# althonos/nafcodec

Hardware: NVIDIA B200
Metric: decoded_ascii_GBps (higher is better)
Workload: dtype u8

## Files before the change

nafcodec_b200/csrc/naf_kernels.cu:

```cuda
#include "naf_kernels.cuh"

#include <algorithm>

#include "zstd_core.cuh"

namespace nk {

#define FULL 0xFFFFFFFFu

__device__ __forceinline__ void flag_archive(NafCounts* counts, uint32_t* status, uint32_t bits) {
    atomicOr((unsigned long long*)&counts->status, (unsigned long long)bits);
    atomicOr(status, bits);
}

struct CS { uint32_t c; uint64_t s; };

__device__ __forceinline__ CS block_excl_scan(uint32_t c, uint64_t s, CS* total) {
    __shared__ uint32_t wc[33];
    __shared__ uint64_t ws[33];
    const int lane = threadIdx.x & 31, warp = threadIdx.x >> 5, nwarps = blockDim.x >> 5;
    uint32_t ic = c;
    uint64_t is = s;
    for (int d = 1; d < 32; d <<= 1) {
        uint32_t tc = __shfl_up_sync(FULL, ic, d);
        uint64_t ts = __shfl_up_sync(FULL, is, d);
        if (lane >= d) { ic += tc; is += ts; }
    }
    if (lane == 31) { wc[warp] = ic; ws[warp] = is; }
    __syncthreads();
    if (warp == 0) {
        uint32_t xc = lane < nwarps ? wc[lane] : 0, oc = xc;
        uint64_t xs = lane < nwarps ? ws[lane] : 0, os = xs;
        for (int d = 1; d < 32; d <<= 1) {
            uint32_t tc = __shfl_up_sync(FULL, xc, d);
            uint64_t ts = __shfl_up_sync(FULL, xs, d);
            if (lane >= d) { xc += tc; xs += ts; }
        }
        wc[lane] = xc - oc; ws[lane] = xs - os;
        if (lane == 31) { wc[32] = xc; ws[32] = xs; }
    }
    __syncthreads();
    CS r;
    r.c = ic - c + wc[warp];
    r.s = is - s + ws[warp];
    total->c = wc[32];
    total->s = ws[32];
    __syncthreads();
    return r;
}

__device__ __forceinline__ void toggle_bit(uint32_t* bits, uint32_t* chunk_par, uint64_t pos) {
    atomicXor(&bits[pos >> 5], 1u << (pos & 31));
    atomicXor(&chunk_par[pos / CHUNK_RESIDUES], 1u);
}

struct SliceView { const uint8_t* src; uint64_t size, begin, end; bool present, last; };

__device__ __forceinline__ SliceView slice_view(const uint8_t* arena, const NafDev& A, int task, uint32_t slice) {
    SliceView V;
    V.present = task == 0 ? (A.has & HAS_IDS) != 0 : task == 1 ? (A.has & HAS_COMMENTS) != 0 : task == 2 ? (A.has & HAS_LENGTHS) != 0
                                                                                                          : (A.has & HAS_MASK) && (A.has & HAS_SEQUENCE);
    V.src = arena + (task == 0 ? A.ids_off : task == 1 ? A.com_off : task == 2 ? A.len_off : A.mask_off);
    V.size = !V.present ? 0 : task == 0 ? A.ids_size : task == 1 ? A.com_size : task == 2 ? (A.len_size & ~3ull) : A.mask_size;
    V.begin = (uint64_t)slice * NAF_SLICE;
    V.end = V.begin + NAF_SLICE < V.size ? V.begin + NAF_SLICE : V.size;
    V.last = V.begin < V.size ? V.end == V.size : (slice == 0);
    return V;
}

__device__ __forceinline__ void pair_of16(int task, const uint4& v, uint32_t nvalid, uint32_t& c, uint64_t& s) {
    const uint32_t w[4] = {v.x, v.y, v.z, v.w};
    if (task == 2) { for (uint32_t j = 0; j < nvalid / 4; j++) { c += (w[j] != FULL); s += w[j]; } return; }
    const uint32_t term = task == 3 ? 0xFFu : 0u;
    for (uint32_t j = 0; j < nvalid; j++) {
        const uint32_t b = (w[j >> 2] >> (8 * (j & 3))) & 0xFF;
        c += task == 3 ? (b != term) : (b == term);
        if (task == 3) s += b;
    }
}

__global__ void __launch_bounds__(1024) k_naf_agg(const uint8_t* arena, const NafDev* archives, CS* agg, uint32_t n_slices) {
    const NafDev& A = archives[blockIdx.y];
    const int task = blockIdx.x / n_slices;
    const uint32_t slice = blockIdx.x % n_slices;
    const SliceView V = slice_view(arena, A, task, slice);
    uint32_t c = 0;
    uint64_t s = 0;
    for (uint64_t p0 = V.begin + (uint64_t)threadIdx.x * 16; p0 < V.end; p0 += 1024 * 16) {
        const uint4 v = *(const uint4*)(V.src + p0);
        pair_of16(task, v, V.end - p0 >= 16 ? 16u : (uint32_t)(V.end - p0), c, s);
    }
    CS tot;
    block_excl_scan(c, s, &tot);
    if (threadIdx.x == 0) agg[((size_t)blockIdx.y * 4 + task) * n_slices + slice] = tot;
}

__global__ void __launch_bounds__(1024) k_naf_scan(uint8_t* arena, const NafDev* archives, uint32_t* status, const CS* agg, uint32_t n_slices) {
    const NafDev& A = archives[blockIdx.y];
    const int task = blockIdx.x / n_slices;
    const uint32_t slice = blockIdx.x % n_slices;
    const int tid = threadIdx.x;
    NafCounts* counts = (NafCounts*)(arena + A.counts_off);
    const SliceView V = slice_view(arena, A, task, slice);
    if (V.begin >= V.size && slice != 0) return;
    uint64_t carry_c = 0, carry_s = 0;
    if (slice) {
        const CS* ag = agg + ((size_t)blockIdx.y * 4 + task) * n_slices;
        uint32_t c = 0;
        uint64_t s = 0;
        for (uint32_t j = tid; j < slice; j += 1024) { c += ag[j].c; s += ag[j].s; }
        CS tot;
        block_excl_scan(c, s, &tot);
        carry_c = tot.c; carry_s = tot.s;
    }
    if (task <= 1) {
        if (!V.present) { if (tid == 0) { if (task == 0) counts->n_ids = 0; else counts->n_comments = 0; } return; }
        uint64_t* offs = (uint64_t*)(arena + (task == 0 ? A.id_offsets_off : A.com_offsets_off));
        if (tid == 0 && slice == 0) offs[0] = 0;
        uint64_t carry = carry_c;
        uint32_t hi = 0;
        for (uint64_t base = V.begin; base < V.end; base += 1024 * 16) {
            uint64_t p0 = base + (uint64_t)tid * 16;
            uint4 v = make_uint4(0x01010101u, 0x01010101u, 0x01010101u, 0x01010101u);
            if (p0 < V.end) v = *(const uint4*)(V.src + p0);
            uint32_t w[4] = {v.x, v.y, v.z, v.w};
            uint32_t nvalid = p0 >= V.end ? 0 : (V.end - p0 >= 16 ? 16 : (uint32_t)(V.end - p0));
            uint32_t c = 0;
            for (uint32_t j = 0; j < nvalid; j++) {
                uint32_t b = (w[j >> 2] >> (8 * (j & 3))) & 0xFF;
                c += (b == 0);
                hi |= b;
            }
            CS tot;
            CS ex = block_excl_scan(c, 0, &tot);
            uint64_t k = carry + ex.c;
            if (c) {
                for (uint32_t j = 0; j < nvalid; j++) {
                    uint32_t b = (w[j >> 2] >> (8 * (j & 3))) & 0xFF;
                    if (b == 0) { k++; if (k <= A.n_records) offs[k] = p0 + j + 1; }
                }
            }
            carry += tot.c;
        }
        if (__any_sync(FULL, hi & 0x80)) { if ((tid & 31) == 0) atomicOr((unsigned long long*)&counts->nonascii, 1ull << task); }
        if (tid == 0 && V.last) {
            if (task == 0) counts->n_ids = carry; else counts->n_comments = carry;
            if (carry < A.n_records && V.size > 0 && V.src[V.size - 1] != 0) flag_archive(counts, status, zc::E_NUL);
        }
    } else if (task == 2) {
        uint64_t* rec = (uint64_t*)(arena + A.rec_offsets_off);
        uint64_t* lens = (uint64_t*)(arena + A.lengths_off);
        if (tid == 0 && slice == 0) rec[0] = 0;
        const uint64_t w_begin = V.begin / 4, w_end = V.end / 4;
        for (uint64_t base = w_begin; base < w_end; base += 1024 * 4) {
            uint64_t i0 = base + (uint64_t)tid * 4;
            uint4 v = make_uint4(FULL, FULL, FULL, FULL);
            if (i0 < w_end) v = *(const uint4*)(V.src + i0 * 4);
            uint32_t w[4] = {v.x, v.y, v.z, v.w};
            uint32_t nvalid = i0 >= w_end ? 0 : (w_end - i0 >= 4 ? 4 : (uint32_t)(w_end - i0));
            uint32_t c = 0;
            uint64_t s = 0;
            for (uint32_t j = 0; j < nvalid; j++) { c += (w[j] != FULL); s += w[j]; }
            CS tot;
            CS ex = block_excl_scan(c, s, &tot);
            uint64_t k = carry_c + ex.c, S = carry_s + ex.s;
            for (uint32_t j = 0; j < nvalid; j++) {
                S += w[j];
                if (w[j] != FULL) { k++; if (k <= A.n_records) rec[k] = S; }
            }
            carry_c += tot.c; carry_s += tot.s;
        }
        if (n_slices > 1) {
            if (tid == 0 && V.last) counts->n_lengths = carry_c;
            return;
        }
        __syncthreads();
        uint64_t n_len = carry_c < A.n_records ? carry_c : A.n_records;
        uint64_t total = rec[n_len];
        if (tid == 0) {
            counts->n_lengths = n_len;
            counts->total_residues = total;
            counts->first_bad_record = NO_RECORD;
            if ((A.has & HAS_SEQUENCE) && total > A.seq_residues) flag_archive(counts, status, zc::E_LENGTHS);
            if ((A.has & HAS_QUALITY) && total > A.qual_size) flag_archive(counts, status, zc::E_LENGTHS);
        }
        for (uint64_t k = tid; k < n_len; k += blockDim.x) lens[k] = rec[k + 1] - rec[k];
    } else {
        if (!V.present) { if (tid == 0 && slice == 0) { counts->n_mask_runs = 0; counts->mask_sum = 0; } return; }
        uint64_t* bounds = (uint64_t*)(arena + A.mask_bounds_off);
        uint32_t* bits = (uint32_t*)(arena + A.mask_bits_off);
        uint32_t* cpar = (uint32_t*)(arena + A.chunk_par_off);
        for (uint64_t base = V.begin; base < V.end; base += 1024 * 16) {
            uint64_t p0 = base + (uint64_t)tid * 16;
            uint4 v = make_uint4(0, 0, 0, 0);
            if (p0 < V.end) v = *(const uint4*)(V.src + p0);
            uint32_t w[4] = {v.x, v.y, v.z, v.w};
            uint32_t nvalid = p0 >= V.end ? 0 : (V.end - p0 >= 16 ? 16 : (uint32_t)(V.end - p0));
            uint32_t c = 0;
            uint64_t s = 0;
            for (uint32_t j = 0; j < nvalid; j++) {
                uint32_t b = (w[j >> 2] >> (8 * (j & 3))) & 0xFF;
                c += (b != 0xFF); s += b;
            }
            CS tot;
            CS ex = block_excl_scan(c, s, &tot);
            uint64_t k = carry_c + ex.c, S = carry_s + ex.s;
            for (uint32_t j = 0; j < nvalid; j++) {
                uint32_t b = (w[j >> 2] >> (8 * (j & 3))) & 0xFF;
                S += b;
                if (b != 0xFF) { bounds[k++] = S; if (S <= A.seq_residues) toggle_bit(bits, cpar, S); }
            }
            carry_c += tot.c; carry_s += tot.s;
        }
        if (tid == 0 && V.last) {
            if (V.size > 0 && V.src[V.size - 1] == 0xFF) {
                bounds[carry_c++] = carry_s;
                if (carry_s <= A.seq_residues) toggle_bit(bits, cpar, carry_s);
            }
            counts->n_mask_runs = carry_c;
            counts->mask_sum = carry_s;
        }
    }
}

__global__ void __launch_bounds__(256) k_naf_lengths(uint8_t* arena, const NafDev* archives, uint32_t* status) {
    const NafDev& A = archives[blockIdx.y];
    NafCounts* counts = (NafCounts*)(arena + A.counts_off);
    const uint64_t* rec = (const uint64_t*)(arena + A.rec_offsets_off);
    uint64_t* lens = (uint64_t*)(arena + A.lengths_off);
    const uint64_t raw = (A.has & HAS_LENGTHS) ? counts->n_lengths : 0;
    const uint64_t n_len = raw < A.n_records ? raw : A.n_records;
    const uint64_t r = (uint64_t)blockIdx.x * blockDim.x + threadIdx.x;
    if (r < n_len) lens[r] = rec[r + 1] - rec[r];
    if (r == 0) {
        const uint64_t total = rec[n_len];
        counts->n_lengths = n_len;
        counts->total_residues = total;
        counts->first_bad_record = NO_RECORD;
        if ((A.has & HAS_SEQUENCE) && total > A.seq_residues) flag_archive(counts, status, zc::E_LENGTHS);
        if ((A.has & HAS_QUALITY) && total > A.qual_size) flag_archive(counts, status, zc::E_LENGTHS);
    }
}

__global__ void __launch_bounds__(256) k_mask_fix(uint8_t* arena, const NafDev* archives, uint32_t* status) {
    const NafDev& A = archives[blockIdx.y];
    if (!(A.has & HAS_MASK) || !(A.has & HAS_SEQUENCE)) return;
    NafCounts* counts = (NafCounts*)(arena + A.counts_off);
    const uint64_t r = (uint64_t)blockIdx.x * blockDim.x + threadIdx.x;
    if (r >= counts->n_lengths) return;
    const uint64_t* rec = (const uint64_t*)(arena + A.rec_offsets_off);
    const uint64_t* bounds = (const uint64_t*)(arena + A.mask_bounds_off);
    uint32_t* bits = (uint32_t*)(arena + A.mask_bits_off);
    const uint64_t S = rec[r], E = rec[r + 1];
    if (E == S || E > A.seq_residues) return;
    const uint64_t pos = E - 1, n_runs = counts->n_mask_runs;
    uint64_t lo = 0, hi = n_runs;
    while (lo < hi) {
        uint64_t mid = (lo + hi) >> 1;
        if (bounds[mid] > pos) hi = mid; else lo = mid + 1;
    }
    if (lo == n_runs) { flag_archive(counts, status, zc::E_MASK); return; }
    if (lo & 1) {
        uint64_t a = lo ? bounds[lo - 1] : 0;
        uint32_t* cpar = (uint32_t*)(arena + A.chunk_par_off);
        toggle_bit(bits, cpar, a > S ? a : S);
        toggle_bit(bits, cpar, E);
    }
}

__device__ __forceinline__ uint32_t prmt(uint32_t a, uint32_t b, uint32_t s) {
#if defined(__CUDA_ARCH__)
    uint32_t d;
    asm("prmt.b32 %0, %1, %2, %3;" : "=r"(d) : "r"(a), "r"(b), "r"(s));
    return d;
#else
    return __byte_perm(a, b, s);
#endif
}

__device__ __forceinline__ uint32_t iupac4(uint32_t x16, uint32_t l0) {
    const uint32_t sel = x16 & 0x7777u;
    const uint32_t lo = prmt(l0, 0x42535943u, sel);
    const uint32_t hi = prmt(0x44525741u, 0x4E56484Du, sel);
    const uint32_t m = prmt(0x80808080u, 0u, x16 & 0x8888u);
    return (lo & ~m) | (hi & m);
}

__device__ __forceinline__ uint32_t spread4_x20(uint32_t q) {
    return ((q * 0x00204081u) & 0x01010101u) << 5;
}

__global__ void __launch_bounds__(UNPACK_T) k_unpack(uint8_t* arena, const NafDev* archives) {
    const NafDev& A = archives[blockIdx.y];
    if (!(A.has & HAS_SEQUENCE) || A.seq_type > 1 || blockIdx.x >= A.n_chunks) return;
    __shared__ uint32_t wp[32], wp2[32];
    __shared__ uint32_t wball, cball;
    const NafCounts* counts = (const NafCounts*)(arena + A.counts_off);
    const uint64_t total = counts->total_residues < A.seq_residues ? counts->total_residues : A.seq_residues;
    const uint64_t wi = (uint64_t)blockIdx.x * CHUNK_WORDS + UNPACK_W * threadIdx.x;
    const uint64_t r0 = wi * 32;
    uint32_t mask[UNPACK_W];
#pragma unroll
    for (uint32_t k = 0; k < UNPACK_W; k++) mask[k] = 0;
    if (A.has & HAS_MASK) {
        const uint32_t* bits = (const uint32_t*)(arena + A.mask_bits_off);
        const uint64_t n_words = (A.seq_residues + 32) / 32;
        uint32_t par = 0;
#pragma unroll
        for (uint32_t k = 0; k < UNPACK_W; k++) {
            const uint32_t w = wi + k < n_words ? bits[wi + k] : 0;
            uint32_t m = w;
            m ^= m << 1; m ^= m << 2; m ^= m << 4; m ^= m << 8; m ^= m << 16;
            mask[k] = par ? ~m : m;
            par ^= __popc(w) & 1;
        }
        const int lane = threadIdx.x & 31, warp = threadIdx.x >> 5;
        uint32_t b = __ballot_sync(FULL, par);
        if (lane == 0) wp[warp] = __popc(b) & 1;
        __syncthreads();
        if (warp == 0) { uint32_t bb = __ballot_sync(FULL, lane < (int)(UNPACK_T / 32) ? wp[lane] : 0u); if (lane == 0) wball = bb; }
        __syncthreads();
        const uint32_t* cpar = (const uint32_t*)(arena + A.chunk_par_off);
        uint32_t cp = 0;
        for (uint32_t c = threadIdx.x; c < blockIdx.x; c += blockDim.x) cp ^= cpar[c];
        const uint32_t cb = __ballot_sync(FULL, cp & 1);
        if (lane == 0) wp2[warp] = __popc(cb) & 1;
        __syncthreads();
        if (warp == 0) { uint32_t bb = __ballot_sync(FULL, lane < (int)(UNPACK_T / 32) ? wp2[lane] : 0u); if (lane == 0) cball = bb; }
        __syncthreads();
        const uint32_t carry = (__popc(cball) & 1) ^ (__popc(wball & ((1u << warp) - 1u)) & 1) ^ (__popc(b & ((1u << lane) - 1u)) & 1);
        if (carry) {
#pragma unroll
            for (uint32_t k = 0; k < UNPACK_W; k++) mask[k] = ~mask[k];
        }
    }
    if (r0 >= total) return;
    const uint32_t l0 = A.seq_type == 1 ? 0x4B47552Du : 0x4B47542Du;
    const uint4* src = (const uint4*)(arena + A.seq_off + r0 / 2);
    uint4 pk[UNPACK_W];
#pragma unroll
    for (uint32_t k = 0; k < UNPACK_W; k++) {
        pk[k] = make_uint4(0, 0, 0, 0);
        if (r0 + 32 * k < total) pk[k] = src[k];
    }
    uint4* dst = (uint4*)(arena + A.ascii_off + r0);
#pragma unroll
    for (uint32_t k = 0; k < UNPACK_W; k++) {
        if (r0 + 32 * k >= total) break;
        const uint32_t x[4] = {pk[k].x, pk[k].y, pk[k].z, pk[k].w};
        uint32_t o[8];
#pragma unroll
        for (int j = 0; j < 4; j++) {
            o[2 * j] = iupac4(x[j] & 0xFFFFu, l0) | spread4_x20((mask[k] >> (8 * j)) & 0xFu);
            o[2 * j + 1] = iupac4(x[j] >> 16, l0) | spread4_x20((mask[k] >> (8 * j + 4)) & 0xFu);
        }
        dst[2 * k] = make_uint4(o[0], o[1], o[2], o[3]);
        dst[2 * k + 1] = make_uint4(o[4], o[5], o[6], o[7]);
    }
}

__global__ void __launch_bounds__(CHUNK_WORDS) k_text_mask(uint8_t* arena, const NafDev* archives) {
    const NafDev& A = archives[blockIdx.y];
    if (!(A.has & HAS_SEQUENCE) || !(A.has & HAS_MASK) || A.seq_type <= 1 || blockIdx.x >= A.n_chunks) return;
    const NafCounts* counts = (const NafCounts*)(arena + A.counts_off);
    const uint64_t total = counts->total_residues < A.seq_residues ? counts->total_residues : A.seq_residues;
    const uint64_t wi = (uint64_t)blockIdx.x * CHUNK_WORDS + threadIdx.x;
    const uint32_t* bits = (const uint32_t*)(arena + A.mask_bits_off);
    const uint32_t* par = (const uint32_t*)(arena + A.chunk_par_off);
    const uint64_t n_words = (A.seq_residues + 32) / 32;
    if (wi >= n_words) return;
    uint32_t carry = 0;
    for (uint32_t c = 0; c < blockIdx.x; c++) carry ^= par[c] & 1;
    for (uint64_t j = (uint64_t)blockIdx.x * CHUNK_WORDS; j < wi; j++) carry ^= __popc(bits[j]) & 1;
    uint32_t m = bits[wi];
    m ^= m << 1; m ^= m << 2; m ^= m << 4; m ^= m << 8; m ^= m << 16;
    if (carry) m = ~m;
    uint8_t* s = arena + A.seq_off;
    for (int j = 0; j < 32; j++) {
        uint64_t i = wi * 32 + j;
        if (i >= total) break;
        uint8_t c = s[i];
        if (((m >> j) & 1) && c >= 'A' && c <= 'Z') s[i] = c | 0x20;
    }
}

__global__ void __launch_bounds__(256) k_ascii_check(uint8_t* arena, const NafDev* archives) {
    const NafDev& A = archives[blockIdx.y];
    const int field = blockIdx.z;
    const uint8_t* src;
    uint64_t size;
    if (field == 0) { if (!(A.has & HAS_SEQUENCE) || A.seq_type <= 1) return; src = arena + A.seq_off; size = A.seq_size; }
    else { if (!(A.has & HAS_QUALITY)) return; src = arena + A.qual_off; size = A.qual_size; }
    NafCounts* counts = (NafCounts*)(arena + A.counts_off);
    uint32_t acc = 0;
    const uint64_t n16 = (size + 15) / 16;
    for (uint64_t i = (uint64_t)blockIdx.x * blockDim.x + threadIdx.x; i < n16; i += (uint64_t)gridDim.x * blockDim.x) {
        uint4 v = *(const uint4*)(src + i * 16);
        if (i * 16 + 16 > size) {
            uint32_t w[4] = {v.x, v.y, v.z, v.w};
            for (int j = 0; j < 16; j++) if (i * 16 + j < size) acc |= (w[j >> 2] >> (8 * (j & 3))) & 0xFF;
        } else acc |= v.x | v.y | v.z | v.w;
    }
    if (__any_sync(FULL, acc & 0x80808080u)) { if ((threadIdx.x & 31) == 0) atomicOr((unsigned long long*)&counts->nonascii, 1ull << (2 + field)); }
}

__device__ __forceinline__ bool utf8_ok(const uint8_t* s, uint64_t n) {
    uint64_t i = 0;
    while (i < n) {
        uint32_t b = s[i];
        if (b < 0x80) { i++; continue; }
        uint32_t need, cp;
        if (b >= 0xC2 && b <= 0xDF) { need = 1; cp = b & 0x1F; }
        else if (b >= 0xE0 && b <= 0xEF) { need = 2; cp = b & 0x0F; }
        else if (b >= 0xF0 && b <= 0xF4) { need = 3; cp = b & 0x07; }
        else return false;
        if (n - i <= need) return false;
        for (uint32_t k = 1; k <= need; k++) {
            uint32_t c = s[i + k];
            if ((c & 0xC0) != 0x80) return false;
            cp = (cp << 6) | (c & 0x3F);
        }
        if (need == 2 && (cp < 0x800 || (cp >= 0xD800 && cp <= 0xDFFF))) return false;
        if (need == 3 && (cp < 0x10000 || cp > 0x10FFFF)) return false;
        i += need + 1;
    }
    return true;
}

__global__ void __launch_bounds__(256) k_utf8_validate(uint8_t* arena, const NafDev* archives, uint32_t* status) {
    const NafDev& A = archives[blockIdx.y];
    const int field = blockIdx.z;
    NafCounts* counts = (NafCounts*)(arena + A.counts_off);
    if (!((counts->nonascii >> field) & 1)) return;
    const uint64_t r = (uint64_t)blockIdx.x * blockDim.x + threadIdx.x;
    const uint8_t* s;
    uint64_t b, e;
    if (field <= 1) {
        uint64_t n = field == 0 ? counts->n_ids : counts->n_comments;
        if (n > A.n_records) n = A.n_records;
        if (r >= n) return;
        const uint64_t* offs = (const uint64_t*)(arena + (field == 0 ? A.id_offsets_off : A.com_offsets_off));
        s = arena + (field == 0 ? A.ids_off : A.com_off);
        b = offs[r]; e = offs[r + 1] - 1;
    } else {
        if (r >= counts->n_lengths) return;
        const uint64_t* rec = (const uint64_t*)(arena + A.rec_offsets_off);
        s = arena + (field == 2 ? A.seq_off : A.qual_off);
        b = rec[r]; e = rec[r + 1];
        if (e > (field == 2 ? A.seq_size : A.qual_size)) return;
    }
    if (!utf8_ok(s + b, e - b)) {
        flag_archive(counts, status, zc::E_UTF8);
        atomicMin((unsigned long long*)&counts->first_bad_record, (unsigned long long)r);
    }
}

int launch_naf_stage(uint8_t* arena, const NafDev* archives, uint32_t n_archives, uint64_t max_records, uint64_t max_scan_bytes, void* scan_agg,
                     uint32_t max_chunks, uint64_t max_text_bytes, bool any_mask, bool any_text_mask, uint32_t* status, cudaStream_t st,
                     StageEvents* ev) {
    StageEvents none;
    if (!ev) ev = &none;
    int launches = 0;
    if (n_archives == 0) { for (int i = 0; i < NAF_STAGES; i++) ev->mark(); return 0; }
    const uint32_t n_slices = (uint32_t)std::max<uint64_t>(1, (max_scan_bytes + NAF_SLICE - 1) / NAF_SLICE);
    uint32_t rec_grid = (uint32_t)((max_records + 255) / 256);
    if (n_slices > 1) { NAF_LAUNCH(k_naf_agg, dim3(4 * n_slices, n_archives), 1024, 0, st, arena, archives, (CS*)scan_agg, n_slices); launches++; }
    NAF_LAUNCH(k_naf_scan, dim3(4 * n_slices, n_archives), 1024, 0, st, arena, archives, status, (const CS*)scan_agg, n_slices); launches++;
    if (n_slices > 1) { NAF_LAUNCH(k_naf_lengths, dim3(rec_grid ? rec_grid : 1, n_archives), 256, 0, st, arena, archives, status); launches++; }
    ev->mark();
    if (max_chunks > 0 && any_mask) {
        if (rec_grid) { NAF_LAUNCH(k_mask_fix, dim3(rec_grid, n_archives), 256, 0, st, arena, archives, status); launches++; }
        ev->mark();
        ev->mark();
    } else { ev->mark(); ev->mark(); }
    if (max_chunks > 0) {
        NAF_LAUNCH(k_unpack, dim3(max_chunks, n_archives), UNPACK_T, 0, st, arena, archives); launches++;
        if (any_text_mask) { NAF_LAUNCH(k_text_mask, dim3(max_chunks, n_archives), CHUNK_WORDS, 0, st, arena, archives); launches++; }
    }
    ev->mark();
    if (max_text_bytes > 0) {
        uint32_t g = (uint32_t)((max_text_bytes / 16 + 255) / 256);
        if (g > 148 * 8) g = 148 * 8;
        if (g == 0) g = 1;
        NAF_LAUNCH(k_ascii_check, dim3(g, n_archives, 2), 256, 0, st, arena, archives); launches++;
    }
    if (rec_grid) { NAF_LAUNCH(k_utf8_validate, dim3(rec_grid, n_archives, 4), 256, 0, st, arena, archives, status); launches++; }
    ev->mark();
    return launches;
}

}
```

nafcodec_b200/csrc/naf_kernels.cuh:

```cuda
#pragma once
#include "cuda_compat.h"
#include <stdint.h>

namespace nk {

enum : uint32_t { HAS_IDS = 1, HAS_COMMENTS = 2, HAS_LENGTHS = 4, HAS_MASK = 8, HAS_SEQUENCE = 16, HAS_QUALITY = 32 };

constexpr uint32_t UNPACK_T = 256;
constexpr uint32_t UNPACK_W = 2;
constexpr uint32_t CHUNK_WORDS = UNPACK_W * UNPACK_T;
constexpr uint32_t CHUNK_RESIDUES = CHUNK_WORDS * 32;
constexpr uint64_t NO_RECORD = ~0ull;
constexpr uint32_t NAF_SLICE = 32768;
constexpr uint32_t NAF_AGG_BYTES = 16;

struct NafCounts {
    uint64_t n_ids;
    uint64_t n_comments;
    uint64_t n_lengths;
    uint64_t total_residues;
    uint64_t n_mask_runs;
    uint64_t mask_sum;
    uint64_t first_bad_record;
    uint64_t nonascii;
    uint64_t status;
    uint64_t _pad;
};

struct NafDev {
    uint64_t n_records;
    uint32_t seq_type;
    uint32_t has;
    uint64_t seq_residues;
    uint64_t ids_off, ids_size, com_off, com_size, len_off, len_size, mask_off, mask_size;
    uint64_t seq_off, seq_size, qual_off, qual_size;
    uint64_t counts_off, id_offsets_off, com_offsets_off, lengths_off, rec_offsets_off, ascii_off;
    uint64_t mask_bits_off, mask_bounds_off, chunk_par_off;
    uint32_t n_chunks;
    uint32_t _pad;
};

int launch_naf_stage(uint8_t* arena, const NafDev* archives_dev, uint32_t n_archives, uint64_t max_records, uint64_t max_scan_bytes, void* scan_agg,
                     uint32_t max_chunks, uint64_t max_text_bytes, bool any_mask, bool any_text_mask, uint32_t* status, cudaStream_t stream,
                     StageEvents* ev);
constexpr int NAF_STAGES = 5;

}
```

nafcodec_b200/csrc/naf_load.cuh:

```cuda
#pragma once
#include "cuda_compat.h"
#include <stdint.h>

namespace nk {

__device__ __forceinline__ uint4 load16u(const uint8_t* p) {
    const uint32_t s = (uint32_t)((uintptr_t)p & 15);
    const uint4* q = (const uint4*)(p - s);
    const uint4 lo = q[0];
    if (s == 0) return lo;
    const uint4 hi = q[1];
    const bool s2 = s & 8, s1 = s & 4;
    const uint32_t a0 = s2 ? lo.z : lo.x, a1 = s2 ? lo.w : lo.y, a2 = s2 ? hi.x : lo.z, a3 = s2 ? hi.y : lo.w, a4 = s2 ? hi.z : hi.x, a5 = s2 ? hi.w : hi.y;
    const uint32_t b0 = s1 ? a1 : a0, b1 = s1 ? a2 : a1, b2 = s1 ? a3 : a2, b3 = s1 ? a4 : a3, b4 = s1 ? a5 : a4;
    const uint32_t bs = (s & 3) * 8;
    const uint32_t o[4] = {__funnelshift_r(b0, b1, bs), __funnelshift_r(b1, b2, bs), __funnelshift_r(b2, b3, bs), __funnelshift_r(b3, b4, bs)};
    return make_uint4(o[0], o[1], o[2], o[3]);
}

}
```

nafcodec_b200/csrc/nafgpu_api.cu:

```cuda
#if defined(__SSE2__)
#include <emmintrin.h>
#endif
#include <stdio.h>
#include <stdlib.h>
#include <string.h>

#include <algorithm>
#include <atomic>
#include <chrono>
#include <memory>
#include <mutex>
#include <thread>
#include <string>
#include <vector>

#include "../../include/nafgpu.h"
#include "cuda_compat.h"
#include "frame_walk.h"
#include "naf_export.cuh"
#include "naf_kernels.cuh"
#include "naf_pack.cuh"
#include "naf_text.cuh"
#include "zstd_kernels.cuh"

namespace {

constexpr uint64_t ALIGN = 128;
inline uint64_t align_up(uint64_t v, uint64_t a = ALIGN) { return (v + a - 1) / a * a; }
constexpr int N_STAGES = zk::ZSTD_STAGES + nk::NAF_STAGES;
constexpr size_t FLUSH_BYTES = 256u << 20;

struct DevBuf {
    void* p = nullptr;
    size_t cap = 0;
    bool ensure(size_t n) {
        if (n <= cap) return true;
        if (p) cudaFree(p);
        p = nullptr; cap = 0;
        size_t want = n + n / 8 + 256;
        if (cudaMalloc(&p, want) != cudaSuccess) { p = nullptr; cudaGetLastError(); return false; }
        cap = want;
        return true;
    }
    void release() { if (p) cudaFree(p); p = nullptr; cap = 0; }
    ~DevBuf() { release(); }
};
struct PinBuf {
    void* p = nullptr;
    size_t cap = 0;
    bool ensure(size_t n) {
        if (n <= cap) return true;
        if (p) cudaFreeHost(p);
        p = nullptr; cap = 0;
        size_t want = n + n / 8 + 256;
        if (cudaHostAlloc(&p, want, cudaHostAllocDefault) != cudaSuccess) { p = nullptr; cudaGetLastError(); return false; }
        cap = want;
        return true;
    }
    void release() { if (p) cudaFreeHost(p); p = nullptr; cap = 0; }
    ~PinBuf() { release(); }
};

struct ArchPlan {
    uint64_t n_records = 0;
    bool dec[6] = {false, false, false, false, false, false};
    uint64_t blob_off[6] = {0, 0, 0, 0, 0, 0};
    uint64_t blob_size[6] = {0, 0, 0, 0, 0, 0};
    bool nucleotide = true;
    uint64_t line_length = 0;
    uint32_t sep = ' ';
    uint32_t first_frame = 0, n_frames = 0;
    int host_status = 0;
    std::string host_msg;
};

struct WalkTask {
    uint32_t arch = 0;
    int sec = 0;
    const uint8_t* data = nullptr;
    uint64_t comp_off = 0, comp_size = 0, dst_off = 0, dst_size = 0;
    fw::JobPlan plan;
    int rc = 0;
    std::string err;
    bool live = true;
    size_t bo = 0;
    uint32_t so = 0, slot_off = 0, ho = 0;
    uint64_t lo = 0;
    uint64_t p_begin = 0, p_end = 0;
    bool first = true, last = true, heavy = false;
    fw::RangeState st;
    int carry_huf_task = -1, carry_tbl_task[3] = {-1, -1, -1};
    uint32_t carry_huf_block = 0, carry_huf_slot = 0, carry_tbl_slot[3] = {0, 0, 0};
    uint32_t abs_huf_block = zf::NO_BLOCK, abs_huf_slot = 0, abs_tbl[3] = {zf::NO_SLOT, zf::NO_SLOT, zf::NO_SLOT};
};

struct PrepClock {
    bool on = getenv("NAFGPU_DEBUG_PREP") != nullptr;
    std::chrono::steady_clock::time_point t = std::chrono::steady_clock::now();
    void lap(const char* what) {
        if (!on) return;
        const auto n = std::chrono::steady_clock::now();
        fprintf(stderr, "[prepare] %-28s %8.3f ms\n", what, std::chrono::duration<double, std::milli>(n - t).count());
        t = n;
    }
};

static_assert(sizeof(zf::BlockDesc) % 16 == 0, "store_desc writes 16 bytes at a time");
#if defined(__SSE2__) && !defined(__CUDA_ARCH__)
inline void store_desc(zf::BlockDesc* dst, const zf::BlockDesc& b) {
    if (((uintptr_t)dst & 15) == 0) {
        const __m128i* s = (const __m128i*)&b;
        __m128i* d = (__m128i*)dst;
        for (size_t k = 0; k < sizeof(zf::BlockDesc) / 16; k++) _mm_stream_si128(d + k, _mm_loadu_si128(s + k));
    } else {
        *dst = b;
    }
}
inline void desc_fence() { _mm_sfence(); }
#else
inline void store_desc(zf::BlockDesc* dst, const zf::BlockDesc& b) { *dst = b; }
inline void desc_fence() {}
#endif

static std::atomic<int> g_helpers_busy{0};
struct HelperLease {
    unsigned n = 1;
    HelperLease() {
        const int hw = (int)std::max(1u, std::thread::hardware_concurrency());
        const int cap = std::min(12, std::max(1, hw * 3 / 4));
        const int got = std::max(1, std::min(cap, hw - g_helpers_busy.load(std::memory_order_relaxed)));
        g_helpers_busy.fetch_add(got, std::memory_order_relaxed);
        n = (unsigned)got;
    }
    ~HelperLease() { g_helpers_busy.fetch_sub((int)n, std::memory_order_relaxed); }
    HelperLease(const HelperLease&) = delete;
    HelperLease& operator=(const HelperLease&) = delete;
};

template <class F>
void parallel_for(size_t n, unsigned max_threads, F fn) {
    if (n <= 1 || max_threads <= 1) { for (size_t i = 0; i < n; i++) fn(i); return; }
    const unsigned w = (unsigned)std::min<size_t>(n, max_threads);
    std::atomic<size_t> next{0};
    auto body = [&] { for (;;) { const size_t i = next.fetch_add(1); if (i >= n) return; fn(i); } };
    std::vector<std::thread> th;
    for (unsigned t = 1; t < w; t++) th.emplace_back(body);
    body();
    for (std::thread& t : th) t.join();
}

}

struct nafgpu_ctx {
    int device = 0;
    cudaStream_t st = 0, st2 = 0, st3 = 0;
    cudaEvent_t ev_fork = nullptr, ev_join = nullptr, ev_fork3 = nullptr, ev_join3 = nullptr, ev_fork4 = nullptr, ev_join4 = nullptr, ev_block = nullptr, ev_d2h = nullptr;
    std::string err;
    DevBuf comp, arena, lit, desc, bstate, hufw, fsstate, lzidx, scanagg, debug, tables, table_al, seq32, seq64, misc, flush, text, fin_g, pack_in, pack_out;
    size_t o_frames = 0, o_naf = 0, o_huf = 0, o_chunks = 0, o_gbase = 0, o_tiles = 0, o_big = 0, o_bigseq = 0, o_biglit = 0;
    PinBuf stage, result, misc_host, text_host, text_stage, pack_host;
    fw::JobPlan plan;
    std::vector<WalkTask> tasks;
    size_t n_tasks = 0;
    std::vector<nk::NafDev> arch;
    std::vector<ArchPlan> aplan;
    zk::JobDev J;
    uint64_t z1_size = 0, z2_off = 0, z2_size = 0, arena_size = 0, counts_size = 0;
    uint64_t max_records = 0, max_text = 0, max_mask = 0, max_scan = 0;
    uint32_t max_chunks = 0;
    bool any_mask = false, any_text_mask = false;
    uint32_t coop_ctas = 1, fin_ctas = 1, fin2_ctas = 1;
    size_t misc_words = 0;
    nafgpu_job_stats stats;
    bool prepared = false, ran = false;
    bool win_counts = false;
    PinBuf win;
    uint32_t want = 0;
    bool exp_ready = false;
    std::vector<nafgpu_counts> counts;
    DevBuf exp_desc;
    PinBuf exp_stage;
    uint32_t n_exp_rec = 0, n_exp_span[4] = {0, 0, 0, 0};
    uint64_t o_exp_span[4] = {0, 0, 0, 0}, exp_bytes[4] = {0, 0, 0, 0}, exp_records = 0, exp_residues = 0;
    cudaEvent_t ev_exp_ready = nullptr, ev_exp_done = nullptr;
    cudaEvent_t ev[N_STAGES + 3];
    bool ev_ok = false;
#if !defined(NAFGPU_EMULATE)
    cudaGraphExec_t graph = nullptr;
#endif
};

namespace {

int fail(nafgpu_ctx* c, int code, const std::string& msg) {
    c->err = msg;
    return code;
}

#define CUDA_TRY(c, expr) do { cudaError_t _e = (expr); if (_e != cudaSuccess) { \
    char _b[256]; snprintf(_b, sizeof _b, "%s failed: %s", #expr, cudaGetErrorString(_e)); return fail((c), NAFGPU_ERR_CUDA, _b); } } while (0)

void drop_graph(nafgpu_ctx* c) {
#if !defined(NAFGPU_EMULATE)
    if (c->graph) { cudaGraphExecDestroy(c->graph); c->graph = nullptr; }
#else
    (void)c;
#endif
}

int enqueue_run(nafgpu_ctx* c, StageEvents* ev) {
    cudaStream_t st = c->st;
    CUDA_TRY(c, cudaMemsetAsync(c->misc.p, 0, c->misc_words * 4, st));
    if (c->J.n_seq && !c->J.lz_small) {
        CUDA_TRY(c, cudaMemsetAsync(c->J.seq_done, 0, c->J.n_seq * 4, st));
        CUDA_TRY(c, cudaMemsetAsync(c->J.lz_blocker, 0xFF, c->J.n_seq * 4, st));
    }
    CUDA_TRY(c, cudaMemsetAsync(c->arena.p, 0, c->counts_size, st));
    if (c->z2_size) CUDA_TRY(c, cudaMemsetAsync((uint8_t*)c->arena.p + c->z2_off, 0, c->z2_size, st));
    int launches = zk::launch_zstd_stage(c->J, st, ev ? (cudaStream_t)0 : c->st2, c->ev_fork, c->ev_join, ev, c->st3, c->ev_fork3, c->ev_join3, c->ev_fork4, c->ev_join4);
    launches += nk::launch_naf_stage((uint8_t*)c->arena.p, (const nk::NafDev*)((const uint8_t*)c->desc.p + c->o_naf), (uint32_t)c->arch.size(), c->max_records, c->max_scan, c->scanagg.p,
                                     c->max_chunks, c->max_text, c->any_mask, c->any_text_mask, c->J.status, st, ev);
    c->stats.kernel_launches = (uint32_t)launches;
    CUDA_TRY(c, cudaGetLastError());
    c->ran = true;
    c->win_counts = false;
    c->exp_ready = false;
    return NAFGPU_OK;
}

void read_lz_stats(nafgpu_ctx* c) {
    const uint32_t* m = (const uint32_t*)c->misc_host.p;
    c->stats.lz_handover = m[4]; c->stats.lz_rounds = m[5]; c->stats.lz_unresolved = m[6];
    c->stats.lz_flow = c->misc_words >= 32 ? (m[c->misc_words - 32] | ((c->J.lz_flow_early && m[c->misc_words - 32 + 4] == 0) ? 2u : 0u)) : 0;
    if (c->misc_words >= 24) memcpy(c->stats.lz_pending, m + c->misc_words - 24, 24 * 4);
}

int status_to_code(uint32_t s, std::string& msg) {
    using namespace zc;
    if (s == 0) return NAFGPU_OK;
    char b[96];
    snprintf(b, sizeof b, " (device status 0x%x)", s);
    if (s & (E_FSE_TABLE | E_HUF_TREE | E_HUF_STREAM | E_SEQ_STREAM | E_LITERALS | E_OFFSET | E_NO_TABLE | E_INTERNAL)) {
        msg = std::string("corrupt zstd stream") + b; return NAFGPU_ERR_INVALID_DATA;
    }
    if (s & E_CHECKSUM) { msg = std::string("zstd frame checksum mismatch") + b; return NAFGPU_ERR_INVALID_DATA; }
    if (s & E_SIZE) { msg = std::string("section does not regenerate the size its header states") + b; return NAFGPU_ERR_INVALID_DATA; }
    if (s & E_LENGTHS) { msg = std::string("record lengths exceed the sequence/quality stream") + b; return NAFGPU_ERR_UNEXPECTED_EOF; }
    if (s & E_MASK) { msg = std::string("failed to get mask unit") + b; return NAFGPU_ERR_UNEXPECTED_EOF; }
    if (s & E_NUL) { msg = std::string("id/comment stream is not NUL terminated") + b; return NAFGPU_ERR_INVALID_DATA; }
    if (s & E_UTF8) { msg = std::string("invalid utf-8") + b; return NAFGPU_ERR_UTF8; }
    msg = std::string("unknown device status") + b;
    return NAFGPU_ERR_INVALID_DATA;
}

static std::mutex g_d2h_turn[16];

static cudaError_t wait_stream(nafgpu_ctx* c) {
    if (c->z1_size < (8u << 20) || !c->ev_block) return cudaStreamSynchronize(c->st);
    cudaError_t e = cudaEventRecord(c->ev_block, c->st);
    return e != cudaSuccess ? e : cudaEventSynchronize(c->ev_block);
}

static cudaEvent_t g_last_d2h[16];

static int d2h_results(nafgpu_ctx* c) {
    if (!c->result.ensure(c->z1_size + 64)) return fail(c, NAFGPU_ERR_NOMEM, "pinned host allocation failed");
    c->win_counts = false;
    CUDA_TRY(c, wait_stream(c));
    {
        std::lock_guard<std::mutex> turn(g_d2h_turn[c->device & 15]);
        cudaEvent_t prev = g_last_d2h[c->device & 15];
        if (prev && prev != c->ev_d2h && c->ev_d2h) CUDA_TRY(c, cudaStreamWaitEvent(c->st, prev, 0));
        CUDA_TRY(c, cudaMemcpyAsync(c->misc_host.p, c->misc.p, c->misc_words * 4, cudaMemcpyDeviceToHost, c->st));
        CUDA_TRY(c, cudaMemcpyAsync(c->result.p, c->arena.p, c->z1_size, cudaMemcpyDeviceToHost, c->st));
        if (c->ev_d2h) { CUDA_TRY(c, cudaEventRecord(c->ev_d2h, c->st)); g_last_d2h[c->device & 15] = c->ev_d2h; }
        else { CUDA_TRY(c, wait_stream(c)); return NAFGPU_OK; }
    }
    CUDA_TRY(c, wait_stream(c));
    return NAFGPU_OK;
}

struct Copy { const uint8_t* src; uint64_t dst, size; };

int finish_prepare(nafgpu_ctx* c, const std::vector<Copy>& copies, uint64_t comp_off, uint32_t n, bool copies_enqueued = false) {
    PrepClock clk;
    size_t nb = 0;
    uint64_t walked_bytes = 0;
    for (size_t ti = 0; ti < c->n_tasks; ti++) {
        WalkTask& T = c->tasks[ti];
        if (!T.live) continue;
        fw::JobPlan& G = c->plan;
        const fw::JobPlan& L = T.plan;
        T.bo = nb; T.so = (uint32_t)G.seq_total; T.lo = G.lit_total - 16; T.slot_off = G.n_slots - 3; T.ho = G.n_huf_slots;
        if (G.seq_total + L.seq_total > 0xFFFFFFF0ull || nb + L.blocks.size() > 0xFFFFFFF0ull) return fail(c, NAFGPU_ERR_UNSUPPORTED, "job has too many blocks or sequences: split the batch");
        for (zf::FrameDesc F : L.frames) { F.first_block += (uint32_t)T.bo; F.first_seq += T.so; G.frames.push_back(F); }
        if (!T.first) {
            zf::FrameDesc& F = G.frames.back();
            F.n_blocks += T.st.n_blocks; F.n_seq += T.st.n_seq;
            if (T.last) { F.has_checksum = T.st.has_checksum; F.checksum = T.st.checksum; }
            if (T.carry_huf_task >= 0) { const WalkTask& S = c->tasks[T.carry_huf_task]; T.abs_huf_block = (uint32_t)S.bo + T.carry_huf_block; T.abs_huf_slot = S.ho + T.carry_huf_slot; }
            for (int k = 0; k < 3; k++) {
                if (T.carry_tbl_task[k] == -2) T.abs_tbl[k] = T.carry_tbl_slot[k];
                else if (T.carry_tbl_task[k] >= 0) T.abs_tbl[k] = c->tasks[T.carry_tbl_task[k]].slot_off + T.carry_tbl_slot[k];
            }
        }
        for (zf::HufItem it : L.huf_items) { it.block += (uint32_t)T.bo; G.huf_items.push_back(it); }
        for (uint32_t b : L.big_seq) G.big_seq.push_back(b + (uint32_t)T.bo);
        for (uint32_t b : L.big_lit) G.big_lit.push_back(b + (uint32_t)T.bo);
        G.seq_total += L.seq_total; G.lit_total += L.lit_total - 16; G.n_slots += L.n_slots - 3; G.n_huf_slots += L.n_huf_slots;
        G.n_huf_blocks += L.n_huf_blocks; G.n_seq_blocks += L.n_seq_blocks; G.n_checksums += L.n_checksums;
        G.max_seq_section = std::max(G.max_seq_section, L.max_seq_section);
        G.max_seq_section_big = std::max(G.max_seq_section_big, L.max_seq_section_big); G.n_tiny_seq_blocks += L.n_tiny_seq_blocks;
        nb += L.blocks.size();
        walked_bytes += T.comp_size;
    }
    c->plan.finalize(zk::HUF_SMALL_SYMBOLS);
    const fw::JobPlan& pl = c->plan;
    const size_t nf = pl.frames.size();
    const uint64_t nseq = pl.seq_total;

    c->misc_words = 0;
    const size_t nh = pl.huf_items.size();
    c->o_frames = align_up(nb * sizeof(zf::BlockDesc), 16);
    c->o_naf = c->o_frames + align_up(nf * sizeof(zf::FrameDesc), 16);
    c->o_huf = c->o_naf + align_up((size_t)n * sizeof(nk::NafDev), 16);
    c->o_chunks = c->o_huf + align_up(nh * sizeof(zf::HufItem), 16);
    std::vector<uint32_t> chunk_first(nf + 1, 0);
    for (size_t f = 0; f < nf; f++) {
        const uint64_t nchunks = (pl.frames[f].dst_size + 65535) >> 16;
        if ((uint64_t)chunk_first[f] + nchunks > 0x7FFFFFFFull) return fail(c, NAFGPU_ERR_UNSUPPORTED, "job too large for the chunk table");
        chunk_first[f + 1] = chunk_first[f] + (uint32_t)nchunks;
    }
    const uint32_t total_chunks = chunk_first[nf];
    std::vector<uint64_t> g_base(nf + 1, 0);
    for (size_t f = 0; f < nf; f++) g_base[f + 1] = g_base[f] + ((pl.frames[f].dst_size + 15) & ~(uint64_t)15);
    c->o_gbase = c->o_chunks + align_up((nf + 1) * 4, 16);
    std::vector<zf::FsTile> tiles;
    std::vector<zf::FsBigFrame> bigs;
    uint32_t fs_big = zf::FS_BIG_FRAME, fs_tile = zf::FS_TILE;
    if (const char* e = getenv("NAFGPU_FS_TILE")) { fs_tile = (uint32_t)std::max(1, atoi(e)); fs_big = 2 * fs_tile; }
    for (size_t f = 0; f < nf; f++) {
        const zf::FrameDesc& F = pl.frames[f];
        if (F.n_blocks <= fs_big) continue;
        bigs.push_back({(uint32_t)f, (uint32_t)tiles.size(), (F.n_blocks + fs_tile - 1) / fs_tile, 0u});
        for (uint32_t b = 0; b < F.n_blocks; b += fs_tile) tiles.push_back({(uint32_t)f, F.first_block + b, std::min(fs_tile, F.n_blocks - b), 0u});
    }
    c->o_tiles = c->o_gbase + align_up((nf + 1) * 8, 16);
    c->o_big = c->o_tiles + align_up(tiles.size() * sizeof(zf::FsTile), 16);
    c->o_bigseq = c->o_big + align_up(bigs.size() * sizeof(zf::FsBigFrame), 16);
    c->o_biglit = c->o_bigseq + align_up(pl.big_seq.size() * 4, 16);
    const size_t stage_bytes = c->o_biglit + align_up(pl.big_lit.size() * 4, 16);
    c->misc_words = 1 + 3 + 1 + 1 + 1 + 3 + nf + total_chunks + 8 + 24;
    bool ok = c->comp.ensure(comp_off + 64) && c->arena.ensure(c->arena_size) && c->lit.ensure(pl.lit_total + 64) &&
              c->desc.ensure(stage_bytes + 64) && c->fin_g.ensure((size_t)g_base[nf] * 4 + 256 + (size_t)total_chunks * 8192) &&
              c->bstate.ensure(nb * sizeof(zf::BlockState) + 64) && c->fsstate.ensure(tiles.size() * sizeof(zf::FsTileState) + 64) && c->lzidx.ensure(((size_t)total_chunks * 16 + nf + 16) * 4) &&
              c->scanagg.ensure((size_t)n * 4 * ((c->max_scan + nk::NAF_SLICE - 1) / nk::NAF_SLICE + 1) * nk::NAF_AGG_BYTES + 64) && c->hufw.ensure((size_t)pl.n_huf_slots * 258 + 64) &&
              c->tables.ensure((size_t)pl.n_slots * zf::FSE_SLOT_CELLS * sizeof(zc::SeqCell)) && c->table_al.ensure(pl.n_slots + 64) &&
              c->seq32.ensure(nseq * 5 * 4 + 64) && c->seq64.ensure(nseq * sizeof(zf::SeqRec) + 64) && c->misc.ensure(c->misc_words * 4);
    if (!ok) return fail(c, NAFGPU_ERR_NOMEM, "device allocation failed");
    clk.lap("merge + device buffers");
    if (!c->stage.ensure(stage_bytes + 64) || !c->result.ensure(c->counts_size + 64) || !c->misc_host.ensure(c->misc_words * 4 + 64))
        return fail(c, NAFGPU_ERR_NOMEM, "pinned host allocation failed");

    uint8_t* sp = (uint8_t*)c->stage.p;
    {
        std::vector<uint32_t> frame_off(c->n_tasks, 0);
        { uint32_t fo = 0; for (size_t t = 0; t < c->n_tasks; t++) { frame_off[t] = c->tasks[t].first ? fo : fo - 1; if (c->tasks[t].live) fo += (uint32_t)c->tasks[t].plan.frames.size(); } }
        (void)walked_bytes;
        unsigned threads = 1;
        std::unique_ptr<HelperLease> lease;
        if (nb > 200000) { lease.reset(new HelperLease); threads = lease->n; }
        struct Chunk { size_t task, begin, end; };
        std::vector<Chunk> chunks;
        for (size_t t = 0; t < c->n_tasks; t++) {
            if (!c->tasks[t].live) continue;
            const size_t cnt = c->tasks[t].plan.blocks.size();
            for (size_t b = 0; b < cnt; b += 65536) chunks.push_back({t, b, std::min(cnt, b + 65536)});
        }
        parallel_for(chunks.size(), threads, [&](size_t ci) {
            const Chunk& K = chunks[ci];
            const WalkTask& T = c->tasks[K.task];
            zf::BlockDesc* out = (zf::BlockDesc*)sp + T.bo;
            const zf::BlockDesc* in = T.plan.blocks.data();
            const uint32_t fo = frame_off[K.task];
            for (size_t i = K.begin; i < K.end; i++) {
                zf::BlockDesc b = in[i];
                b.frame += fo;
                if (b.n_seq) b.seq_base += T.so;
                if (b.huf_block == fw::PREV_BLOCK) { b.lit_base += T.lo; b.huf_block = T.abs_huf_block; b.huf_slot = T.abs_huf_slot; }
                else {
                    if (b.lit_type >= zf::LT_HUF && b.btype == zf::BT_COMPRESSED) { b.lit_base += T.lo; b.huf_slot += T.ho; }
                    if (b.huf_block != zf::NO_BLOCK) b.huf_block += (uint32_t)T.bo;
                }
                for (int k = 0; k < 3; k++) {
                    if (b.tbl[k] == fw::PREV_SLOT) b.tbl[k] = T.abs_tbl[k];
                    else if (b.tbl[k] != zf::NO_SLOT && b.tbl[k] >= 3) b.tbl[k] += T.slot_off;
                }
                store_desc(out + i, b);
            }
            desc_fence();
        });
    }
    clk.lap("pinned staging + block copy");
    if (nf) memcpy(sp + c->o_frames, pl.frames.data(), nf * sizeof(zf::FrameDesc));
    if (n) memcpy(sp + c->o_naf, c->arch.data(), (size_t)n * sizeof(nk::NafDev));
    if (nh) memcpy(sp + c->o_huf, pl.huf_items.data(), nh * sizeof(zf::HufItem));
    memcpy(sp + c->o_chunks, chunk_first.data(), (nf + 1) * 4);
    memcpy(sp + c->o_gbase, g_base.data(), (nf + 1) * 8);
    if (!pl.big_seq.empty()) memcpy(sp + c->o_bigseq, pl.big_seq.data(), pl.big_seq.size() * 4);
    if (!pl.big_lit.empty()) memcpy(sp + c->o_biglit, pl.big_lit.data(), pl.big_lit.size() * 4);
    if (!tiles.empty()) { memcpy(sp + c->o_tiles, tiles.data(), tiles.size() * sizeof(zf::FsTile)); memcpy(sp + c->o_big, bigs.data(), bigs.size() * sizeof(zf::FsBigFrame)); }
    if (stage_bytes) CUDA_TRY(c, cudaMemcpyAsync(c->desc.p, sp, stage_bytes, cudaMemcpyHostToDevice, c->st));
    uint64_t h2d = stage_bytes;
    for (const Copy& cp : copies) {
        if (!copies_enqueued) CUDA_TRY(c, cudaMemcpyAsync((uint8_t*)c->comp.p + cp.dst, cp.src, cp.size, cudaMemcpyHostToDevice, c->st));
        h2d += cp.size;
    }

    clk.lap("H2D enqueue");
    zk::JobDev& J = c->J;
    J.comp = (const uint8_t*)c->comp.p; J.out = (uint8_t*)c->arena.p; J.lit = (uint8_t*)c->lit.p;
    J.frames = (const zf::FrameDesc*)((const uint8_t*)c->desc.p + c->o_frames); J.blocks = (const zf::BlockDesc*)c->desc.p;
    J.bstate = (zf::BlockState*)c->bstate.p; J.tables = (zc::SeqCell*)c->tables.p; J.table_al = (uint8_t*)c->table_al.p;
    J.seq_done = (uint32_t*)c->seq32.p;
    J.lz_list[0] = J.seq_done + nseq; J.lz_list[1] = J.seq_done + 2 * nseq; J.lz_list[2] = J.seq_done + 3 * nseq; J.lz_blocker = J.seq_done + 4 * nseq;
    J.seq = (zf::SeqRec*)c->seq64.p;
    J.tiny_blocks = pl.n_tiny_seq_blocks >= 4096u ? 1u : 0u;
    if (const char* e = getenv("NAFGPU_TINY_BLOCKS")) J.tiny_blocks = (uint32_t)atoi(e);
    J.seq_big_list = (const uint32_t*)((const uint8_t*)c->desc.p + c->o_bigseq); J.n_seq_big = (uint32_t)pl.big_seq.size();
    J.lit_big_list = (const uint32_t*)((const uint8_t*)c->desc.p + c->o_biglit); J.n_lit_big = (uint32_t)pl.big_lit.size();
    {
        uint64_t small_max = 2048;
        if (const char* e = getenv("NAFGPU_LZ_SMALL")) small_max = (uint64_t)std::min(8192, std::max(0, atoi(e)));
        J.lz_small = (nseq <= small_max && nf <= 65535 && c->arena_size < (1ull << 32)) ? 1u : 0u;
    }
    J.seq_stage_bytes = std::min<uint32_t>((((J.tiny_blocks ? pl.max_seq_section_big : pl.max_seq_section) + 15u) & ~15u) + 64u, 16u * 1024u);
    uint32_t* misc = (uint32_t*)c->misc.p;
    J.status = misc; J.lz_count = misc + 1; J.lz_handover = misc + 4; J.lz_rounds = misc + 5; J.fin_unresolved = misc + 6; J.fin_count = misc + 7;
    J.frame_bad = misc + 10; J.fin_chunk_flag = misc + 10 + nf; J.lz_pending = misc + 10 + nf + total_chunks + 8;
    J.lz_flow = misc + 10 + nf + total_chunks;
    J.lz_flow_on = nseq > 8192 ? 1u : 0u;
    if (const char* e = getenv("NAFGPU_LZ_FLOW")) J.lz_flow_on = (uint32_t)atoi(e);
    J.flow_ctas = (uint32_t)std::min<uint64_t>((nseq + 255) / 256, 148u * 8u);
    J.lz_flow_early = (nseq > 2048 && nseq <= 65536 && !getenv("NAFGPU_LZ_SMALL")) ? 1u : 0u;
    if (const char* e = getenv("NAFGPU_LZ_FLOW_EARLY")) J.lz_flow_early = (uint32_t)atoi(e);
    J.fin_chunk_first = (const uint32_t*)((const uint8_t*)c->desc.p + c->o_chunks); J.fin_total_chunks = total_chunks;
    J.lz_idx = (uint32_t*)c->lzidx.p;
    J.fin_ctas = c->fin_ctas; J.fin2_ctas = c->fin2_ctas; J.fin_g = (uint32_t*)c->fin_g.p; J.fin_ext = (uint32_t*)c->fin_g.p + g_base[nf] + 64;
    J.fin_g_base = (const uint64_t*)((const uint8_t*)c->desc.p + c->o_gbase);
    J.coop_ctas = c->coop_ctas;
    {
        uint64_t biggest = 0;
        for (const auto& F : c->plan.frames) biggest = std::max<uint64_t>(biggest, F.dst_size);
        (void)biggest;
        const uint64_t waves = ((uint64_t)total_chunks + c->fin_ctas - 1) / std::max<uint32_t>(c->fin_ctas, 1u);
        J.fin_cost_us = (uint32_t)std::min<uint64_t>(300 + waves * 270, 0x7FFFFFFFu);
        if (const char* e = getenv("NAFGPU_FIN_COST_US")) J.fin_cost_us = (uint32_t)atoi(e);
    }
    J.huf_weights = (uint8_t*)c->hufw.p; J.huf_meta = (uint8_t*)c->hufw.p + (size_t)pl.n_huf_slots * 256;
    J.huf_items = (const zf::HufItem*)((const uint8_t*)c->desc.p + c->o_huf); J.n_huf_items = (uint32_t)nh; J.n_huf_big = pl.n_huf_big; J.max_huf_stream = pl.max_huf_stream; J.max_huf_small = pl.max_huf_small;
    J.huf_block_min = 0;
    if (const char* e = getenv("NAFGPU_HUF_BLOCK_MIN")) J.huf_block_min = (uint32_t)std::max(1, atoi(e));
    J.debug = nullptr; J.debug_seq = nullptr;
    if (getenv("NAFGPU_DEBUG_HUF") && nh) {
        if (!c->debug.ensure(nh * 64 + 64)) return fail(c, NAFGPU_ERR_NOMEM, "debug buffer");
        cudaMemsetAsync(c->debug.p, 0, nh * 64 + 64, c->st);
        J.debug = (unsigned long long*)c->debug.p;
        J.debug_seq = J.debug + nh * 8;
    }
    J.fs_tiles = (const zf::FsTile*)((const uint8_t*)c->desc.p + c->o_tiles); J.fs_big = (const zf::FsBigFrame*)((const uint8_t*)c->desc.p + c->o_big);
    J.fs_state = (zf::FsTileState*)c->fsstate.p; J.n_fs_tiles = (uint32_t)tiles.size(); J.n_fs_big = (uint32_t)bigs.size(); J.fs_big_frame = fs_big;
    J.n_frames = (uint32_t)nf; J.n_blocks = (uint32_t)nb; J.n_slots = pl.n_slots; J.n_seq = nseq; J.n_checksums = pl.n_checksums;

    c->stats.n_archives = n; c->stats.n_frames = nf; c->stats.n_blocks = nb; c->stats.n_sequences = nseq;
    c->stats.h2d_bytes = h2d; c->stats.d2h_bytes = c->z1_size + c->misc_words * 4;
    c->stats.n_stages = N_STAGES + 1;
    c->prepared = true;
    return NAFGPU_OK;
}

int archive_status(nafgpu_ctx* c, uint32_t a, std::string& msg) {
    const ArchPlan& P = c->aplan[a];
    if (P.host_status) { msg = P.host_msg; return P.host_status; }
    const uint32_t* frame_bad = (const uint32_t*)c->misc_host.p + 10;
    uint32_t s = 0;
    for (uint32_t f = P.first_frame; f < P.first_frame + P.n_frames; f++) s |= frame_bad[f];
    const nk::NafCounts* C = (const nk::NafCounts*)((const uint8_t*)c->result.p + c->arch[a].counts_off);
    s |= (uint32_t)C->status;
    return status_to_code(s & ~zc::E_UTF8, msg);
}

int read_counts(nafgpu_ctx* c) {
    if (c->win_counts) return NAFGPU_OK;
    CUDA_TRY(c, wait_stream(c));
    CUDA_TRY(c, cudaMemcpyAsync(c->misc_host.p, c->misc.p, c->misc_words * 4, cudaMemcpyDeviceToHost, c->st));
    CUDA_TRY(c, cudaMemcpyAsync(c->result.p, c->arena.p, c->counts_size, cudaMemcpyDeviceToHost, c->st));
    CUDA_TRY(c, cudaStreamSynchronize(c->st));
    read_lz_stats(c);
    c->win_counts = true;
    return NAFGPU_OK;
}

int export_tables(nafgpu_ctx* c) {
    if (c->exp_ready) return NAFGPU_OK;
    { int rc = read_counts(c); if (rc) return rc; }
    const uint32_t n = (uint32_t)c->arch.size();
    c->counts.assign(n, nafgpu_counts());
    std::vector<nk::ExpRec> recs;
    std::vector<nk::ExpSpan> spans[4];
    uint64_t records = 0, residues = 0, bytes[4] = {0, 0, 0, 0};
    for (uint32_t a = 0; a < n; a++) {
        const nk::NafDev& D = c->arch[a];
        const ArchPlan& P = c->aplan[a];
        const nk::NafCounts* C = (const nk::NafCounts*)((const uint8_t*)c->result.p + D.counts_off);
        nafgpu_counts& k = c->counts[a];
        memset(&k, 0, sizeof k);
        k.n_records = P.n_records;
        k.first_bad_record = nk::NO_RECORD;
        std::string msg;
        k.status = archive_status(c, a, msg);
        if (k.status) continue;
        k.n_ids = P.dec[0] ? std::min<uint64_t>(C->n_ids, P.n_records) : 0;
        k.n_comments = P.dec[1] ? std::min<uint64_t>(C->n_comments, P.n_records) : 0;
        k.n_lengths = P.dec[2] ? C->n_lengths : 0;
        k.total_residues = P.dec[2] ? C->total_residues : 0;
        k.id_bytes = P.dec[0] ? D.ids_size : 0;
        k.comment_bytes = P.dec[1] ? D.com_size : 0;
        k.first_bad_record = C->first_bad_record;
        k.record_status = (C->first_bad_record != nk::NO_RECORD) ? NAFGPU_ERR_UTF8 : 0;
        if (k.n_lengths)
            recs.push_back({records, residues, D.rec_offsets_off, {P.dec[4] ? D.ascii_off : nk::NO_FIELD, P.dec[5] ? D.qual_off : nk::NO_FIELD}, 0});
        const uint64_t field_bytes[4] = {k.id_bytes, k.comment_bytes, P.dec[4] ? k.total_residues : 0, P.dec[5] ? k.total_residues : 0};
        const uint64_t field_off[4] = {D.ids_off, D.com_off, D.ascii_off, D.qual_off};
        for (int f = 0; f < 4; f++) {
            if (!field_bytes[f]) continue;
            spans[f].push_back({bytes[f], field_off[f]});
            bytes[f] += field_bytes[f];
        }
        records += k.n_lengths;
        residues += k.total_residues;
    }
    uint64_t off = align_up(recs.size() * sizeof(nk::ExpRec), 16);
    for (int f = 0; f < 4; f++) { c->o_exp_span[f] = off; off += align_up(spans[f].size() * sizeof(nk::ExpSpan), 16); }
    if (!c->exp_desc.ensure(off + 64)) return fail(c, NAFGPU_ERR_NOMEM, "device allocation failed");
    if (!c->exp_stage.ensure(off + 64)) return fail(c, NAFGPU_ERR_NOMEM, "pinned host allocation failed");
    uint8_t* S = (uint8_t*)c->exp_stage.p;
    if (!recs.empty()) memcpy(S, recs.data(), recs.size() * sizeof(nk::ExpRec));
    for (int f = 0; f < 4; f++) if (!spans[f].empty()) memcpy(S + c->o_exp_span[f], spans[f].data(), spans[f].size() * sizeof(nk::ExpSpan));
    if (off) CUDA_TRY(c, cudaMemcpyAsync(c->exp_desc.p, S, off, cudaMemcpyHostToDevice, c->st));
    c->n_exp_rec = (uint32_t)recs.size();
    for (int f = 0; f < 4; f++) { c->n_exp_span[f] = (uint32_t)spans[f].size(); c->exp_bytes[f] = bytes[f]; }
    c->exp_records = records;
    c->exp_residues = residues;
    c->exp_ready = true;
    return NAFGPU_OK;
}

}

extern "C" {

int nafgpu_ctx_create(int device, nafgpu_ctx** out) {
    if (!out) return NAFGPU_ERR_ARGUMENT;
    *out = nullptr;
    int n = 0;
    if (cudaGetDeviceCount(&n) != cudaSuccess || n <= 0) { cudaGetLastError(); return NAFGPU_ERR_NO_DEVICE; }
    if (device < 0 || device >= n) return NAFGPU_ERR_ARGUMENT;
    if (cudaSetDevice(device) != cudaSuccess) return NAFGPU_ERR_CUDA;
    nafgpu_ctx* c = new nafgpu_ctx();
    c->device = device;
    memset(&c->stats, 0, sizeof c->stats);
    memset(&c->J, 0, sizeof c->J);
    if (cudaStreamCreateWithFlags(&c->st, cudaStreamNonBlocking) != cudaSuccess) { delete c; return NAFGPU_ERR_CUDA; }
    if (cudaStreamCreateWithFlags(&c->st2, cudaStreamNonBlocking) != cudaSuccess || cudaStreamCreateWithFlags(&c->st3, cudaStreamNonBlocking) != cudaSuccess) { delete c; return NAFGPU_ERR_CUDA; }
    if (cudaEventCreateWithFlags(&c->ev_fork3, cudaEventDisableTiming) != cudaSuccess || cudaEventCreateWithFlags(&c->ev_join3, cudaEventDisableTiming) != cudaSuccess) { delete c; return NAFGPU_ERR_CUDA; }
    if (cudaEventCreateWithFlags(&c->ev_fork4, cudaEventDisableTiming) != cudaSuccess || cudaEventCreateWithFlags(&c->ev_join4, cudaEventDisableTiming) != cudaSuccess) { delete c; return NAFGPU_ERR_CUDA; }
    if (cudaEventCreateWithFlags(&c->ev_fork, cudaEventDisableTiming) != cudaSuccess || cudaEventCreateWithFlags(&c->ev_join, cudaEventDisableTiming) != cudaSuccess) { delete c; return NAFGPU_ERR_CUDA; }
    if (cudaEventCreateWithFlags(&c->ev_block, cudaEventDisableTiming | cudaEventBlockingSync) != cudaSuccess) { c->ev_block = nullptr; cudaGetLastError(); }
    if (cudaEventCreateWithFlags(&c->ev_d2h, cudaEventDisableTiming) != cudaSuccess) { c->ev_d2h = nullptr; cudaGetLastError(); }
    if (cudaEventCreateWithFlags(&c->ev_exp_ready, cudaEventDisableTiming) != cudaSuccess || cudaEventCreateWithFlags(&c->ev_exp_done, cudaEventDisableTiming) != cudaSuccess) { delete c; return NAFGPU_ERR_CUDA; }
    for (int i = 0; i < N_STAGES + 3; i++) if (cudaEventCreate(&c->ev[i]) != cudaSuccess) { delete c; return NAFGPU_ERR_CUDA; }
    c->ev_ok = true;
    c->coop_ctas = zk::lz_resolve_max_ctas(device);
    zk::lz_finish_ctas(device, &c->fin_ctas, &c->fin2_ctas);
    *out = c;
    return NAFGPU_OK;
}

void nafgpu_ctx_destroy(nafgpu_ctx* c) {
    if (!c) return;
    cudaSetDevice(c->device);
    cudaStreamSynchronize(c->st);
    drop_graph(c);
    DevBuf* d[] = {&c->comp, &c->arena, &c->lit, &c->desc, &c->bstate, &c->hufw, &c->fsstate, &c->lzidx, &c->scanagg, &c->debug, &c->tables, &c->table_al, &c->seq32, &c->seq64, &c->misc, &c->flush, &c->text, &c->fin_g, &c->pack_in, &c->pack_out, &c->exp_desc};
    for (DevBuf* b : d) b->release();
    c->stage.release(); c->result.release(); c->misc_host.release(); c->text_host.release(); c->text_stage.release(); c->pack_host.release(); c->win.release();
    c->exp_stage.release();
    if (c->ev_exp_ready) cudaEventDestroy(c->ev_exp_ready);
// ... 820 lines not shown
```

nafcodec_b200/csrc/zstd_format.h:

```cpp
#pragma once
#include <stdint.h>

namespace zf {

constexpr uint32_t BLOCK_MAX = 128 * 1024;
constexpr uint32_t NO_BLOCK = 0xFFFFFFFFu;
constexpr uint32_t NO_SLOT = 0xFFFFFFFFu;
constexpr int COMP_PAD = 32;

enum BlockType : uint8_t { BT_RAW = 0, BT_RLE = 1, BT_COMPRESSED = 2 };
enum LitType : uint8_t { LT_RAW = 0, LT_RLE = 1, LT_HUF = 2, LT_TREELESS = 3 };
enum SeqMode : uint8_t { SM_PREDEF = 0, SM_RLE = 1, SM_FSE = 2, SM_REPEAT = 3 };

struct FrameDesc {
    uint64_t src_off;
    uint64_t src_size;
    uint64_t dst_off;
    uint64_t dst_size;
    uint32_t first_block;
    uint32_t n_blocks;
    uint32_t first_seq;
    uint32_t n_seq;
    uint64_t window;
    uint32_t has_checksum;
    uint32_t checksum;
};

struct BlockDesc {
    uint64_t src_off;
    uint64_t lit_base;
    uint32_t src_size;
    uint32_t frame;
    uint32_t lit_regen;
    uint32_t lit_csize;
    uint32_t lit_src;
    uint32_t seq_src;
    uint32_t n_seq;
    uint32_t seq_base;
    uint32_t huf_block;
    uint32_t tbl[3];
    uint8_t btype;
    uint8_t lit_type;
    uint8_t n_streams;
    uint8_t modes;
    uint8_t defines;
    uint8_t _pad[3];
    uint32_t known_regen;
    uint32_t huf_slot;
};

constexpr uint32_t TINY_SEQ_MAX = 32, TINY_LIT_MAX = 2048;
#if defined(__CUDACC__)
#define ZF_HD __host__ __device__
#else
#define ZF_HD
#endif
ZF_HD inline bool tiny_seq_block(const BlockDesc& B) { return B.btype == BT_COMPRESSED && B.n_seq != 0 && B.n_seq <= TINY_SEQ_MAX; }
ZF_HD inline bool needs_seq_kernel(const BlockDesc& B) { return B.btype == BT_COMPRESSED && B.n_seq > TINY_SEQ_MAX; }
ZF_HD inline bool tiny_lit_block(const BlockDesc& B) {
    if (B.btype != BT_COMPRESSED) return B.src_size <= TINY_LIT_MAX;
    return B.n_seq <= TINY_SEQ_MAX && B.lit_regen <= TINY_LIT_MAX;
}

struct HufItem {
    uint32_t block;
    uint32_t src_off;
    uint32_t src_size;
    uint32_t dst_off;
    uint32_t n_sym;
    uint32_t seg_symbols;
};

struct SeqRec {
    uint32_t ll, ml;
    uint32_t off;
    uint32_t litpos;
    uint32_t outpos;
    uint32_t block;
    uint64_t match_pos;
};

struct BlockState {
    uint64_t out_off;
    uint32_t regen;
    uint32_t seq_bits_off;
    int32_t rep_src[3];
    uint32_t rep_val[3];
    uint32_t rep_in[3];
    uint32_t _pad;
};

constexpr uint32_t FS_BIG_FRAME = 16384, FS_TILE = 8192;
struct FsTile { uint32_t frame, first_block, n_blocks, _pad; };
struct FsBigFrame { uint32_t frame, first_tile, n_tiles, _pad; };
struct FsTileState {
    uint64_t off_in;
    uint64_t regen;
    uint32_t rep_in[3];
    int32_t ms[3];
    uint32_t mv[3];
    uint32_t bad;
};

constexpr uint32_t OFF_SYMBOLIC = 0x80000000u;

constexpr int FSE_SLOT_CELLS = 512;

}
```

nafcodec_b200/csrc/zstd_kernels.cu:

```cuda
#include "zstd_kernels.cuh"

#include <algorithm>

namespace zk {

using namespace zf;
using zc::BackBits;
using zc::SeqCell;

__device__ __forceinline__ void flag_error(const JobDev& J, uint32_t frame, uint32_t bits) {
    atomicOr(J.status, bits);
    atomicOr(&J.frame_bad[frame], bits);
}

struct SmemBits {
    const uint32_t* sw;
    uint64_t w;
    int qi, rr;
    int x_zero;
    __device__ __forceinline__ void init(const uint32_t* words, int x, int xz) {
        sw = words; x_zero = xz;
        qi = (x >> 5) - 1;
        rr = x - (qi << 5);
        w = ((uint64_t)sw[qi + 1] << 32) | sw[qi];
    }
    __device__ __forceinline__ uint32_t read(int k) {
        if (rr < k) { w = (w << 32) | sw[--qi]; rr += 32; }
        rr -= k;
        return k ? (uint32_t)(w >> rr) & (k >= 32 ? 0xFFFFFFFFu : ((1u << k) - 1u)) : 0u;
    }
    __device__ __forceinline__ int remaining() const { return (qi << 5) + rr - x_zero; }
};

#if defined(__CUDA_ARCH__)
typedef uint32_t saddr_t;
__device__ __forceinline__ saddr_t to_saddr(const void* p) { return (saddr_t)__cvta_generic_to_shared(p); }
__device__ __forceinline__ uint32_t lds32(saddr_t a) { uint32_t v; asm volatile("ld.shared.u32 %0, [%1];" : "=r"(v) : "r"(a)); return v; }
__device__ __forceinline__ uint2 lds64(saddr_t a) { uint2 v; asm volatile("ld.shared.v2.u32 {%0, %1}, [%2];" : "=r"(v.x), "=r"(v.y) : "r"(a)); return v; }
__device__ __forceinline__ uint32_t lds16(saddr_t a) { uint16_t v; asm volatile("ld.shared.u16 %0, [%1];" : "=h"(v) : "r"(a)); return v; }
__device__ __forceinline__ void sts8(saddr_t a, uint32_t v) { asm volatile("st.shared.u8 [%0], %1;" :: "r"(a), "r"(v)); }
__device__ __forceinline__ void sts32(saddr_t a, uint32_t v) { asm volatile("st.shared.u32 [%0], %1;" :: "r"(a), "r"(v)); }
#else
typedef uintptr_t saddr_t;
static inline saddr_t to_saddr(const void* p) { return (saddr_t)p; }
static inline uint32_t lds32(saddr_t a) { return *(const uint32_t*)a; }
static inline uint2 lds64(saddr_t a) { return *(const uint2*)a; }
static inline uint32_t lds16(saddr_t a) { return *(const uint16_t*)a; }
static inline void sts8(saddr_t a, uint32_t v) { *(uint8_t*)a = (uint8_t)v; }
static inline void sts32(saddr_t a, uint32_t v) { *(uint32_t*)a = v; }
#endif

__device__ __forceinline__ uint32_t smem_bits(const uint32_t* sw, int o, uint32_t k) {
    const uint32_t lo = sw[o >> 5], hi = sw[(o >> 5) + 1];
    const uint32_t v = __funnelshift_r(lo, hi, (uint32_t)o);
    return k >= 32 ? v : (v & ((1u << k) - 1u));
}

template <class Emit>
__device__ __forceinline__ bool fse_build_warp(const int16_t* norm, int max_symbol, int al, uint8_t* cell_sym, uint16_t* cnt, uint16_t* cum,
                                               int lane, Emit emit) {
    const int size = 1 << al, mask = size - 1, step = (size >> 1) + (size >> 3) + 3;
    const uint32_t lt = (1u << lane) - 1u;
    int n_low = 0, reg_total = 0;
    for (int s0 = 0; s0 <= max_symbol; s0 += 32) {
        const int s = s0 + lane;
        const int nv = s <= max_symbol ? (int)norm[s] : 0;
        const bool low = nv == -1;
        const uint32_t lb = __ballot_sync(0xFFFFFFFFu, low);
        if (low) cell_sym[size - 1 - (n_low + __popc(lb & lt))] = (uint8_t)s;
        const int c = nv > 0 ? nv : 0;
        int inc = c;
#pragma unroll
        for (int d = 1; d < 32; d <<= 1) { const int t = __shfl_up_sync(0xFFFFFFFFu, inc, d); if (lane >= d) inc += t; }
        if (s <= max_symbol) { cnt[s] = (uint16_t)(low ? 1 : c); cum[s] = (uint16_t)(reg_total + inc - c); }
        reg_total += __shfl_sync(0xFFFFFFFFu, inc, 31);
        n_low += __popc(lb);
    }
    if (lane == 0) cum[max_symbol + 1] = (uint16_t)reg_total;
    __syncwarp();
    if (reg_total + n_low != size) return false;
    const int high = size - n_low;
    int placed = 0;
    for (int j0 = 0; j0 < size; j0 += 32) {
        const int p = ((j0 + lane) * step) & mask;
        const bool valid = p < high;
        const uint32_t vb = __ballot_sync(0xFFFFFFFFu, valid);
        if (valid) {
            const int t = placed + __popc(vb & lt);
            int lo = 0, hi = max_symbol + 1;
            while (hi - lo > 1) { const int mid = (lo + hi) >> 1; if ((int)cum[mid] <= t) lo = mid; else hi = mid; }
            cell_sym[p] = (uint8_t)lo;
        }
        placed += __popc(vb);
    }
    __syncwarp();
    for (int i0 = 0; i0 < size; i0 += 32) {
        const int i = i0 + lane;
        const int s = cell_sym[i];
        const uint32_t same = __match_any_sync(0xFFFFFFFFu, s);
        const int r = __popc(same & lt);
        const uint32_t nx = (uint32_t)cnt[s] + (uint32_t)r;
        __syncwarp();
        if (r == 0) cnt[s] = (uint16_t)(cnt[s] + __popc(same));
        __syncwarp();
        const int nb = al - zc::highbit32(nx);
        emit(i, s, nb, (int)((nx << nb) - (uint32_t)size));
    }
    return true;
}

__device__ __forceinline__ uint32_t fse_read_ncount_staged(const uint32_t* dw, uint32_t byte0, uint32_t src_len, int max_symbol, int max_al,
                                                           int16_t* norm, int* al_out) {
    uint32_t pos = byte0 * 8u;
    const uint32_t limit = pos + src_len * 8u;
    auto peek = [&](uint32_t k) { const uint32_t i = pos >> 5; return __funnelshift_r(dw[i], dw[i + 1], pos) & ((1u << k) - 1u); };
    const int al = (int)peek(4) + 5;
    pos += 4;
    if (al > max_al) return 0;
    int rem = 1 << al, sym = 0;
    while (rem > 0 && sym <= max_symbol) {
        const uint32_t bits = 32u - (uint32_t)__clz(rem + 1);
        uint32_t v = peek(bits);
        const uint32_t low = (1u << (bits - 1)) - 1u, thr = (1u << bits) - 1u - (uint32_t)(rem + 1);
        const bool small = (v & low) < thr;
        pos += bits - (small ? 1u : 0u);
        v = small ? (v & low) : (v > low ? v - thr : v);
        const int pr = (int)v - 1;
        rem -= pr < 0 ? -pr : pr;
        norm[sym++] = (int16_t)pr;
        if (pr == 0) {
            for (;;) {
                const uint32_t r = peek(2);
                pos += 2;
                sym += (int)r;
                if (r != 3) break;
                if (pos > limit) return 0;
            }
            if (sym > max_symbol + 1) return 0;
        }
        if (pos > limit) return 0;
    }
    if (rem != 0 || sym > max_symbol + 1) return 0;
    *al_out = al;
    return ((pos + 7u) >> 3) - byte0;
}

template <int PART>
__global__ void __launch_bounds__(PART == 0 ? 96 : 32) k_build_tables(JobDev J) {
    if (PART == 1) {
        if (blockIdx.x >= J.n_blocks) return;
        const BlockDesc& B = J.blocks[blockIdx.x];
        if (B.btype != BT_COMPRESSED || B.lit_type != LT_HUF) return;
        __shared__ __align__(16) uint8_t tree[192];
        __shared__ __align__(16) uint32_t sb[48];
        __shared__ uint32_t cells[64];
        __shared__ uint8_t cell_sym[64];
        __shared__ __align__(4) uint8_t w[256];
        __shared__ int s_n, s_mode, s_start, s_nbytes, s_al;
        __shared__ int16_t hnorm[16];
        __shared__ uint16_t hcnt[16], hcum[16];
        const int l1 = threadIdx.x;
        const uint32_t tsize = B.lit_csize < 130u ? B.lit_csize : 130u;
        for (uint32_t i = l1; i < 192; i += 32) tree[i] = i < tsize ? J.comp[B.src_off + B.lit_src + i] : 0;
        for (uint32_t i = l1; i < 64; i += 32) ((uint32_t*)w)[i] = 0;
        for (uint32_t i = l1; i < 48; i += 32) sb[i] = 0;
        if (l1 == 0) { s_n = 0; s_mode = -1; }
        __syncwarp();
        const uint32_t h = tsize ? tree[0] : 0u;
        if (l1 == 0 && tsize) {
            if (h >= 128) { if (1u + (h - 127u + 1u) / 2u <= tsize) { s_mode = 0; s_n = (int)h - 127; } }
            else if (h >= 2 && 1u + h <= tsize) {
                int al = 0;
                const uint32_t used = zc::fse_read_ncount(tree + 1, h, 12, zc::MAX_AL_HUF, hnorm, &al);
                if (used != 0 && used < h) { s_mode = 2; s_start = 1 + (int)used; s_nbytes = (int)(h - used); s_al = al; }
            }
        }
        __syncwarp();
        if (s_mode == 2) {
            const bool good = fse_build_warp(hnorm, 12, s_al, cell_sym, hcnt, hcum, l1,
                                             [&](int i, int sy, int nb, int base) { cells[i] = (uint32_t)sy | ((uint32_t)nb << 8) | ((uint32_t)base << 16); });
            __syncwarp();
            if (l1 == 0) s_mode = good ? 1 : -1;
            __syncwarp();
        }
        int n = 0;
        bool good = s_mode >= 0;
        if (s_mode == 0) {
            n = s_n;
            for (int i = l1; i < n; i += 32) { const uint8_t b = tree[1 + (i >> 1)]; w[i] = (i & 1) ? (b & 15) : (b >> 4); }
        } else if (s_mode == 1) {
            for (int i = l1; i < s_nbytes; i += 32) ((uint8_t*)sb)[16 + i] = tree[s_start + i];
            __syncwarp();
            if (l1 == 0) {
                const uint8_t last = ((const uint8_t*)sb)[16 + s_nbytes - 1];
                bool ok = last != 0;
                if (ok) {
                    const int al = s_al;
                    int pos = 8 * (s_nbytes - 1) + zc::highbit32(last);
                    pos -= al; uint32_t s1 = smem_bits(sb, 128 + pos, (uint32_t)al);
                    pos -= al; uint32_t s2 = smem_bits(sb, 128 + pos, (uint32_t)al);
                    ok = pos >= 0;
                    int k = 0;
                    bool ended = false;
                    if (ok) for (int it = 0; it < 127; it++) {
                        const uint32_t c1 = cells[s1], c2 = cells[s2];
                        const int n1 = (int)((c1 >> 8) & 0xFF), n2 = (int)((c2 >> 8) & 0xFF);
                        const int p1 = pos - n1, p2 = p1 - n2;
                        const uint32_t b1 = smem_bits(sb, 128 + p1, (uint32_t)n1);
                        const uint32_t b2 = smem_bits(sb, 128 + (p2 < -96 ? -96 : p2), (uint32_t)n2);
                        w[k] = (uint8_t)c1; w[k + 1] = (uint8_t)c2;
                        s1 = (c1 >> 16) + b1;
                        s2 = (c2 >> 16) + b2;
                        if (p2 < 0) {
                            if (p1 < 0) k += 2;
                            else { w[k + 2] = (uint8_t)cells[s1]; k += 3; }
                            ended = true;
                            break;
                        }
                        k += 2; pos = p2;
                    }
                    ok = ok && ended;
                    s_n = ok ? k : 0;
                }
                if (!ok) s_n = 0;
            }
            __syncwarp();
            n = s_n;
            good = n > 0;
        }
        __syncwarp();
        uint32_t tot = 0, bad = 0;
        for (int i = l1; i < n; i += 32) { const uint32_t x = w[i]; if (x > (uint32_t)zc::HUF_MAX_BITS) bad = 1; else if (x) tot += 1u << (x - 1); }
#pragma unroll
        for (int d = 16; d > 0; d >>= 1) { tot += __shfl_xor_sync(0xFFFFFFFFu, tot, d); bad |= __shfl_xor_sync(0xFFFFFFFFu, bad, d); }
        int ns = 0, mb = 0;
        if (good && !bad && tot != 0) {
            mb = zc::highbit32(tot) + 1;
            const uint32_t left = (1u << mb) - tot;
            if (mb <= zc::HUF_MAX_BITS && (left & (left - 1)) == 0) {
                if (l1 == 0) w[n] = (uint8_t)(zc::highbit32(left) + 1);
                ns = n + 1;
            }
        }
        __syncwarp();
        uint32_t* gw = (uint32_t*)(J.huf_weights + (size_t)B.huf_slot * 256);
        for (int i = l1; i < 64; i += 32) gw[i] = ((const uint32_t*)w)[i];
        if (l1 != 0) return;
        J.huf_meta[(size_t)B.huf_slot * 2] = (uint8_t)(ns ? ns - 1 : 0);
        J.huf_meta[(size_t)B.huf_slot * 2 + 1] = (uint8_t)(ns ? mb : 0);
        if (ns == 0) flag_error(J, B.frame, zc::E_HUF_TREE);
        return;
    }
    __shared__ int16_t norm[3][56];
    __shared__ uint8_t cell_sym[3][512];
    __shared__ uint16_t cnt[3][56];
    __shared__ int al[3];
    __shared__ int mode[3];
    __shared__ int rle_sym[3];
    __shared__ int ok;
    const int lane = threadIdx.x & 31, warp = threadIdx.x >> 5;
    const uint32_t bi = blockIdx.x;
    uint32_t slot[3];
    uint32_t frame = 0;
    if (bi == J.n_blocks) {
        if (threadIdx.x < 3) {
            int k = (int)threadIdx.x;
            for (int s = 0; s <= zc::kind_max_symbol(k); s++) norm[k][s] = zc::predef_norm(k, s);
            al[k] = zc::predef_al(k);
            mode[k] = SM_FSE;
        }
        if (threadIdx.x == 0) ok = 1;
        slot[0] = 0; slot[1] = 1; slot[2] = 2;
    } else {
        const BlockDesc& B = J.blocks[bi];
        if (B.btype != BT_COMPRESSED || B.n_seq == 0) return;
        frame = B.frame;
        slot[0] = B.tbl[0]; slot[1] = B.tbl[1]; slot[2] = B.tbl[2];
        __shared__ __align__(16) uint8_t desc[272];
        const uint32_t dsize = (B.src_size - B.seq_src) < 240u ? (B.src_size - B.seq_src) : 240u;
        for (uint32_t i = threadIdx.x; i < 272; i += blockDim.x) desc[i] = i < dsize ? J.comp[B.src_off + B.seq_src + i] : 0;
        for (uint32_t i = threadIdx.x; i < 3 * 56; i += blockDim.x) (&norm[0][0])[i] = 0;
        __syncthreads();
        if (threadIdx.x == 0) {
            ok = 1;
            const uint8_t* src = desc - B.seq_src;
            uint32_t p = B.seq_src;
            for (int k = 0; k < 3; k++) {
                int m = (B.modes >> (6 - 2 * k)) & 3;
                mode[k] = (B.defines >> k) & 1 ? m : -1;
                if (p - B.seq_src + 80 > 256 && (m == SM_RLE || m == SM_FSE)) src = J.comp + B.src_off;
                if (m == SM_RLE) {
                    if (p >= B.src_size) { ok = 0; break; }
                    rle_sym[k] = src[p++];
                    if (rle_sym[k] > zc::kind_max_symbol(k)) { ok = 0; break; }
                } else if (m == SM_FSE) {
                    int a = 0;
                    const bool in_stage = src != J.comp + B.src_off;
                    uint32_t used = in_stage ? fse_read_ncount_staged((const uint32_t*)desc, p - B.seq_src, B.src_size - p, zc::kind_max_symbol(k), zc::kind_max_al(k), norm[k], &a)
                                             : zc::fse_read_ncount(src + p, B.src_size - p, zc::kind_max_symbol(k), zc::kind_max_al(k), norm[k], &a);
                    if (used == 0 || p + used > B.src_size) { ok = 0; break; }
                    al[k] = a;
                    p += used;
                }
            }
            if (p >= B.src_size) ok = 0;
// ... 1235 lines not shown
__global__ void __launch_bounds__(HB_T, 3) k_huf_decode_block(JobDev J) {
    NAF_DYN_SMEM(unsigned char, smem);
    uint16_t* t1 = (uint16_t*)smem;
    uint8_t* weights = smem + 4096;
    uint16_t* wcnt = (uint16_t*)(smem + 4096 + 256);
    uint32_t* misc = (uint32_t*)(smem + 4096 + 512);
    uint64_t* wmap = (uint64_t*)(smem + 4096 + 256);
    uint32_t* t3 = (uint32_t*)(smem + 4864);
    uint8_t* sout = smem + 4864 + 16384;
    uint16_t* legtab = (uint16_t*)sout;
    uint16_t* qitems = (uint16_t*)(sout + HB_LEG_BYTES);
    uint32_t* scomp = (uint32_t*)(smem + HB_FIXED);
    const int tid = threadIdx.x, lane = tid & 31, warp = tid >> 5;

    const uint32_t item0 = blockIdx.x * 4u;
    const BlockDesc& B = J.blocks[J.huf_items[item0].block];
#if defined(__CUDA_ARCH__)
    const uint32_t mbar = (uint32_t)__cvta_generic_to_shared(&misc[56]);
#endif
    auto stage = [&](uint32_t sidx) {
        const HufItem si = J.huf_items[item0 + sidx];
        const uint8_t* sg = J.comp + B.src_off + si.src_off;
        const uint32_t sa = (uint32_t)((uintptr_t)sg & 15);
        const uint32_t bytes = ((sa + si.src_size + 15u) >> 4) << 4;
#if defined(__CUDA_ARCH__)
        if (tid == 0) {
            asm volatile("mbarrier.arrive.expect_tx.shared::cta.b64 _, [%0], %1;" :: "r"(mbar), "r"(bytes) : "memory");
            asm volatile("cp.async.bulk.shared::cluster.global.mbarrier::complete_tx::bytes [%0], [%1], %2, [%3];"
                         :: "r"((uint32_t)__cvta_generic_to_shared(scomp + 4)), "l"(sg - sa), "r"(bytes), "r"(mbar) : "memory");
        }
#else
        for (uint32_t c = tid; c < (bytes >> 4); c += HB_T) ((uint4*)scomp)[1 + c] = ((const uint4*)(sg - sa))[c];
#endif
    };
#if defined(__CUDA_ARCH__)
    if (tid == 0) {
        asm volatile("mbarrier.init.shared::cta.b64 [%0], %1;" :: "r"(mbar), "r"(1));
        asm volatile("fence.mbarrier_init.release.cluster;" ::: "memory");
    }
    __syncthreads();
#endif
    stage(0);
    for (int i = tid; i < 64; i += HB_T) ((uint32_t*)weights)[i] = ((const uint32_t*)(J.huf_weights + (size_t)B.huf_slot * 256))[i];
    const int nsym = (int)J.huf_meta[(size_t)B.huf_slot * 2] + 1, maxbits = (int)J.huf_meta[(size_t)B.huf_slot * 2 + 1];
    __syncthreads();
    if (maxbits != 0) {
        huf_build_t1<HB_T>(weights, nsym, maxbits, t1, wcnt);
        huf_build_wide<HB_T, true>(t1, maxbits, nullptr, t3, 0u, 1u << HUF_W);
    }
    const bool fixed_len = !__syncthreads_or(tid < 128 && (tid & 15) >= 2 && (tid & 15) <= zc::HUF_MAX_BITS && wcnt[tid] != 0);
    const bool skip = __syncthreads_or(maxbits == 0 || (tid == 0 && J.frame_bad[B.frame] != 0));
    for (uint32_t sidx = 0; sidx < 4u; sidx++) {
    const HufItem it = J.huf_items[item0 + sidx];
    const uint8_t* g = J.comp + B.src_off + it.src_off;
    const uint32_t a = (uint32_t)((uintptr_t)g & 15);
#if defined(__CUDA_ARCH__)
    {
        uint32_t done;
        do {
            asm volatile("{\n\t.reg .pred p;\n\tmbarrier.try_wait.parity.shared::cta.b64 p, [%1], %2;\n\tselp.u32 %0, 1, 0, p;\n\t}"
                         : "=r"(done) : "r"(mbar), "r"(sidx & 1u) : "memory");
        } while (!done);
    }
#endif
    if (skip) break;
    if ((uint32_t)tid < 16 + a) ((uint8_t*)scomp)[tid] = 0;
    __syncthreads();

    const int Z = (int)(16 + a) * 8;
    const uint8_t last = ((const uint8_t*)scomp)[16 + a + it.src_size - 1];
    if (last == 0) { if (tid == 0) flag_error(J, B.frame, zc::E_HUF_STREAM); break; }
    const int P0 = 8 * (int)(it.src_size - 1) + zc::highbit32(last);
    const int XTOP = Z + P0;
    int S = (P0 + HB_T - 1) / HB_T;
    if (S < 2 * MAXC) S = 2 * MAXC;
    const int ck[HB_NLEG + 1] = {S < HB_CK0 ? S : HB_CK0, S < HB_CK1 ? S : HB_CK1, S < HB_CK2 ? S : HB_CK2, S};
    const int q0 = tid * S;
    const int qe = (q0 + S < P0) ? q0 + S : P0;
    const bool active = q0 < P0;
    const saddr_t s_comp = to_saddr(scomp), s_t3 = to_saddr(t3), s_t1 = to_saddr(t1);
    auto cp_at = [&](int rq0, int rqe, int j) { const int x = rq0 + ck[j]; return x < rqe ? x : rqe; };

    uint64_t first = ~0ull, fcnt = 0;
    uint32_t live = 0;
    if (active) {
        const int l0 = cp_at(q0, qe, 0);
        first = 0;
        if (fixed_len) {
            int q = q0 + (maxbits - q0 % maxbits) % maxbits, c = 0;
            track_advance3(s_comp, s_t3, s_t1, maxbits, XTOP, q, c, l0);
            first = (uint64_t)(uint32_t)(q - l0) * 0x1111111111111111ull;
            fcnt = (uint64_t)(uint32_t)c * 0x1111111111111111ull;
            live = 1u << (q - l0);
        } else {
            for (int k = 0; k < maxbits; k++) {
                int q = q0 + k, c = 0;
                track_advance3(s_comp, s_t3, s_t1, maxbits, XTOP, q, c, l0);
                const uint32_t o = (uint32_t)(q - l0);
                first |= (uint64_t)o << (4 * k);
                fcnt |= (uint64_t)c << (4 * k);
                live |= 1u << o;
            }
        }
        if (maxbits < 16) first |= ~0ull << (4 * maxbits);
    }
    uint32_t leg_done = 0;
    for (int leg = 0; leg < HB_NLEG; leg++) {
        if (ck[leg + 1] == ck[leg]) continue;
        leg_done |= 1u << leg;
        const uint32_t n_mine = (uint32_t)__popc(live);
        uint32_t qtotal;
        uint32_t idx = hb_scan(n_mine, misc + 8 * (leg & 1), &qtotal);
        for (uint32_t m = live; m; m &= m - 1) qitems[idx++] = (uint16_t)((uint32_t)tid | ((uint32_t)(__ffs((int)m) - 1) << 8));
        __syncthreads();
        for (uint32_t i = tid; i < qtotal; i += HB_T) {
            const uint32_t item = qitems[i];
            const int owner = (int)(item & 0xFFu), o = (int)(item >> 8);
            const int oq0 = owner * S, oqe = (oq0 + S < P0) ? oq0 + S : P0;
            const int lim = cp_at(oq0, oqe, leg + 1);
            int q = cp_at(oq0, oqe, leg) + o, c = 0;
            track_advance3(s_comp, s_t3, s_t1, maxbits, XTOP, q, c, lim);
            legtab[(leg * HB_T + owner) * MAXC + o] = (uint16_t)((uint32_t)(q - lim) | ((uint32_t)c << 4));
        }
        __syncthreads();
        uint32_t nl = 0;
        for (uint32_t m = live; m; m &= m - 1) nl |= 1u << (legtab[(leg * HB_T + tid) * MAXC + (__ffs((int)m) - 1)] & 15u);
        live = nl;
    }
    uint64_t fmap = MAP_IDENTITY;
    if (active) {
        uint64_t exit_of = 0;
        uint32_t starts = 0;
        for (int k = 0; k < maxbits; k++) starts |= 1u << ((uint32_t)(first >> (4 * k)) & 15u);
        for (uint32_t m = starts; m; m &= m - 1) {
            const int o0 = __ffs((int)m) - 1;
            uint32_t o = (uint32_t)o0;
#pragma unroll
            for (int leg = 0; leg < HB_NLEG; leg++) if (leg_done & (1u << leg)) o = legtab[(leg * HB_T + tid) * MAXC + o] & 15u;
            exit_of |= (uint64_t)o << (4 * o0);
        }
        fmap = 0;
        for (int k = 0; k < maxbits; k++) fmap |= ((exit_of >> (4 * ((uint32_t)(first >> (4 * k)) & 15u))) & 15ull) << (4 * k);
        if (maxbits < 16) fmap |= ~0ull << (4 * maxbits);
    }
    uint64_t inc_map = fmap;
#pragma unroll
    for (int d = 1; d < 32; d <<= 1) {
        const uint64_t o = __shfl_up_sync(0xFFFFFFFFu, inc_map, d);
        const bool need = lane >= d && !map_is_const(inc_map, maxbits);
        if (__any_sync(0xFFFFFFFFu, need)) { if (need) inc_map = map_compose(inc_map, o); }
    }
    uint64_t exc_map = __shfl_up_sync(0xFFFFFFFFu, inc_map, 1);
    if (lane == 0) exc_map = MAP_IDENTITY;
    if (lane == 31) wmap[warp] = inc_map;
    __syncthreads();
    if (tid == 0) {
        uint32_t k = 0;
        for (int w = 0; w < HB_NW; w++) { misc[16 + w] = k; k = (uint32_t)(wmap[w] >> (4 * k)) & 15u; }
    }
    __syncthreads();
    const uint32_t kw = misc[16 + warp];
    const uint32_t ktrue = (uint32_t)(exc_map >> (4 * kw)) & 15u;
    uint32_t mycnt = 0;
    int myland = -1;
    if (active && ktrue < (uint32_t)maxbits) {
        uint32_t o = (uint32_t)(first >> (4 * ktrue)) & 15u;
        mycnt = (uint32_t)(fcnt >> (4 * ktrue)) & 15u;
#pragma unroll
        for (int leg = 0; leg < HB_NLEG; leg++) {
            if (leg_done & (1u << leg)) { const uint32_t e = legtab[(leg * HB_T + tid) * MAXC + o]; o = e & 15u; mycnt += e >> 4; }
        }
        myland = qe + (int)o;
    }
    const bool bad_end = active && qe == P0 && myland != P0;
    const int any_bad = __syncthreads_or(bad_end);
    uint32_t total;
    const uint32_t off = hb_scan(mycnt, misc, &total);
    if (any_bad || total != it.n_sym) { if (tid == 0) flag_error(J, B.frame, zc::E_HUF_STREAM); break; }
    uint8_t* dst = J.lit + B.lit_base + it.dst_off;
    const uint32_t a2 = (uint32_t)((uintptr_t)dst & 15);
    if (mycnt) {
        saddr_t out = to_saddr(sout) + a2 + off;
        int q = q0 + (int)ktrue;
        int rem = qe - q;
        Win w;
        win_init(w, s_comp, XTOP - q);
        const int sh1 = HUF_W - maxbits;
        while ((out & 3u) && rem > 0) {
            const uint32_t e = lds16(s_t1 + 2 * (win_peek(w) >> sh1));
            sts8(out, e >> 8); out++;
            rem -= (int)(e & 0xFFu);
            win_consume(w, (int)(e & 0xFFu));
        }
        uint32_t acc_lo = 0, acc_hi = 0;
        int pc = 0;
        while (rem > HUF_W) {
            const uint32_t e = lds32(s_t3 + win_peek_x4(w));
            const int n = (int)(e >> 28), len = (int)(e >> 24) & 15;
            const uint32_t sy = e & 0xFFFFFFu;
            acc_lo |= sy << (8 * pc);
            acc_hi |= __funnelshift_l(sy, 0u, 8 * pc);
            pc += n;
            if (pc >= 4) { sts32(out, acc_lo); out += 4; acc_lo = acc_hi; acc_hi = 0; pc -= 4; }
            rem -= len;
            win_consume(w, len);
        }
        while (rem > 0) {
            const uint32_t e = lds16(s_t1 + 2 * (win_peek(w) >> sh1));
            acc_lo |= (e >> 8) << (8 * pc);
            pc++;
            if (pc == 4) { sts32(out, acc_lo); out += 4; acc_lo = 0; pc = 0; }
            rem -= (int)(e & 0xFFu);
            win_consume(w, (int)(e & 0xFFu));
        }
        for (int k = 0; k < pc; k++) sts8(out + k, acc_lo >> (8 * k));
    }
    __syncthreads();
    if (sidx + 1 < 4u) stage(sidx + 1);
    {
        const uint32_t n = it.n_sym, endb = a2 + n;
        uint8_t* dal = dst - a2;
        const uint32_t first_full = a2 ? 1u : 0u, last_full = endb >> 4;
        for (uint32_t c = first_full + tid; c < last_full; c += HB_T) ((uint4*)dal)[c] = ((const uint4*)sout)[c];
        if (a2) { uint32_t hend = endb < 16 ? endb : 16; for (uint32_t k = a2 + tid; k < hend; k += HB_T) dal[k] = sout[k]; }
        if (last_full >= first_full && (last_full << 4) < endb && !(a2 && last_full == 0))
            for (uint32_t k = (last_full << 4) + tid; k < endb; k += HB_T) dal[k] = sout[k];
    }
    __syncthreads();
    }
}

__device__ __forceinline__ void copy_g2g_plain(uint8_t* __restrict__ dst, const uint8_t* __restrict__ src, uint32_t n, int lane, int nlanes) {
    if (n < 64) { for (uint32_t k = lane; k < n; k += nlanes) dst[k] = src[k]; return; }
    const uint32_t h = (uint32_t)(-(intptr_t)dst) & 15u;
    for (uint32_t k = lane; k < h; k += nlanes) dst[k] = src[k];
    const uint32_t body = (n - h) >> 4;
    const uintptr_t sa = (uintptr_t)(src + h);
    const uint4* sw = (const uint4*)(sa & ~(uintptr_t)15);
    const uint32_t mis = (uint32_t)(sa & 15), q = mis >> 2, sh = (mis & 3) * 8;
    uint4* d4 = (uint4*)(dst + h);
    for (uint32_t c = lane; c < body; c += nlanes) {
        const uint4 A = sw[c], B = sw[c + 1];
        uint32_t w0, w1, w2, w3, w4;
        if (q == 0) { w0 = A.x; w1 = A.y; w2 = A.z; w3 = A.w; w4 = B.x; }
        else if (q == 1) { w0 = A.y; w1 = A.z; w2 = A.w; w3 = B.x; w4 = B.y; }
        else if (q == 2) { w0 = A.z; w1 = A.w; w2 = B.x; w3 = B.y; w4 = B.z; }
        else { w0 = A.w; w1 = B.x; w2 = B.y; w3 = B.z; w4 = B.w; }
        d4[c] = make_uint4(__funnelshift_r(w0, w1, sh), __funnelshift_r(w1, w2, sh), __funnelshift_r(w2, w3, sh), __funnelshift_r(w3, w4, sh));
    }
    const uint32_t done = h + (body << 4);
    for (uint32_t k = done + lane; k < n; k += nlanes) dst[k] = src[k];
}

template <int U>
__device__ __forceinline__ void copy_g2g_1rt(uint8_t* __restrict__ dst, const uint8_t* __restrict__ src, uint32_t n, int lane, int nlanes);
template <int U = 1>
__device__ __forceinline__ void copy_g2g(uint8_t* __restrict__ dst, const uint8_t* __restrict__ src, uint32_t n, int lane, int nlanes) {
    if (U == 1) copy_g2g_plain(dst, src, n, lane, nlanes);
    else copy_g2g_1rt<U>(dst, src, n, lane, nlanes);
}
template <int U>
__device__ __forceinline__ void copy_g2g_1rt(uint8_t* __restrict__ dst, const uint8_t* __restrict__ src, uint32_t n, int lane, int nlanes) {
    if (n < 64) {
        const uint32_t k0 = lane, k1 = lane + nlanes;
        uint8_t v0 = 0, v1 = 0;
        if (k0 < n) v0 = src[k0];
        if (k1 < n) v1 = src[k1];
        if (k0 < n) dst[k0] = v0;
        if (k1 < n) dst[k1] = v1;
        return;
    }
    const uint32_t h = (uint32_t)(-(intptr_t)dst) & 15u;
    const uint32_t body = (n - h) >> 4;
    const uintptr_t sa = (uintptr_t)(src + h);
    const uint4* sw = (const uint4*)(sa & ~(uintptr_t)15);
    const uint32_t mis = (uint32_t)(sa & 15), q = mis >> 2, sh = (mis & 3) * 8;
    uint4* d4 = (uint4*)(dst + h);
    const uint32_t tk = h + (body << 4) + (uint32_t)lane;
    uint8_t hb = 0, tb = 0;
    if ((uint32_t)lane < h) hb = src[lane];
    if (tk < n) tb = src[tk];
    for (uint32_t c = lane; c < body; c += (uint32_t)U * (uint32_t)nlanes) {
        uint4 A[U], B[U];
#pragma unroll
        for (int u = 0; u < U; u++) { const uint32_t x = c + (uint32_t)u * nlanes; if (x < body) { A[u] = sw[x]; B[u] = sw[x + 1]; } }
#pragma unroll
        for (int u = 0; u < U; u++) {
            const uint32_t x = c + (uint32_t)u * nlanes;
            if (x < body) {
                const uint4 a = A[u], b = B[u];
                uint32_t w0, w1, w2, w3, w4;
                if (q == 0) { w0 = a.x; w1 = a.y; w2 = a.z; w3 = a.w; w4 = b.x; }
                else if (q == 1) { w0 = a.y; w1 = a.z; w2 = a.w; w3 = b.x; w4 = b.y; }
                else if (q == 2) { w0 = a.z; w1 = a.w; w2 = b.x; w3 = b.y; w4 = b.z; }
                else { w0 = a.w; w1 = b.x; w2 = b.y; w3 = b.z; w4 = b.w; }
                d4[x] = make_uint4(__funnelshift_r(w0, w1, sh), __funnelshift_r(w1, w2, sh), __funnelshift_r(w2, w3, sh), __funnelshift_r(w3, w4, sh));
            }
        }
    }
    if ((uint32_t)lane < h) dst[lane] = hb;
    if (tk < n) dst[tk] = tb;
}

constexpr int LZLIT_G = 32;
constexpr int LZLIT_SPLIT = 4;
constexpr uint32_t LZLIT_LONG = 4096;

template <int U>
__global__ void __launch_bounds__(256, U == 1 ? 6 : 1) k_lz_literals(JobDev J) {
    __shared__ uint32_t lq_n, lq_lp[40], lq_op[40], lq_ll[40];
    const uint32_t bi = J.tiny_blocks ? J.lit_big_list[blockIdx.x] : blockIdx.x;
    const BlockDesc& B = J.blocks[bi];
    if (J.frame_bad[B.frame]) return;
    const BlockState& S = J.bstate[bi];
    uint8_t* out = J.out + S.out_off;
    const int tid = threadIdx.x + blockIdx.y * blockDim.x, nt = blockDim.x * gridDim.y;
    if (B.btype == BT_RAW) { copy_g2g(out, J.comp + B.src_off, B.src_size, tid, nt); return; }
    if (B.btype == BT_RLE) {
        uint8_t v = J.comp[B.src_off];
        for (uint32_t i = tid; i < B.src_size; i += nt) out[i] = v;
        return;
    }
    const uint8_t* lsrc = nullptr;
    uint8_t rle = 0;
    if (B.lit_type == LT_RAW) lsrc = J.comp + B.src_off + B.lit_src;
    else if (B.lit_type == LT_RLE) rle = J.comp[B.src_off + B.lit_src];
    else lsrc = J.lit + B.lit_base;
    if (B.n_seq == 0) {
        if (B.lit_type == LT_RLE) for (uint32_t i = tid; i < B.lit_regen; i += nt) out[i] = rle;
        else copy_g2g(out, lsrc, B.lit_regen, tid, nt);
        return;
    }
    const int lane = tid % LZLIT_G, ng = nt / LZLIT_G, grp = U > 1 ? (int)(threadIdx.x / LZLIT_G) * (int)gridDim.y + (int)blockIdx.y : tid / LZLIT_G;
    const uint32_t n = B.n_seq, base = B.seq_base;
    if (threadIdx.x == 0) lq_n = 0;
    __syncthreads();
    auto fetch = [&](uint32_t i, uint32_t& lp, uint32_t& op, uint32_t& ll, uint32_t& ml) {
        if (i > n) return;
        const uint32_t j = i < n ? i : n - 1;
        const uint4 r = *(const uint4*)&J.seq[base + j];
        ll = r.x; ml = r.y; lp = r.w; op = J.seq[base + j].outpos;
    };
    uint32_t lp = 0, op = 0, ll = 0, ml = 0;
    fetch((uint32_t)grp, lp, op, ll, ml);
    for (uint32_t i = grp; i <= n; i += ng) {
        uint32_t nlp = 0, nop = 0, nll = 0, nml = 0;
        fetch(i + ng, nlp, nop, nll, nml);
        if (i < n) {
            if (lane == 0) J.seq[base + i].match_pos = S.out_off + op + ll;
        } else {
            lp += ll; op += ll + ml; ll = B.lit_regen - lp;
        }
        if (ll > LZLIT_LONG && B.lit_type != LT_RLE) {
            if (lane == 0) { const uint32_t q = atomicAdd(&lq_n, 1u); lq_lp[q] = lp; lq_op[q] = op; lq_ll[q] = ll; }
        } else if (B.lit_type == LT_RLE) for (uint32_t k = lane; k < ll; k += LZLIT_G) out[op + k] = rle;
        else copy_g2g(out + op, lsrc + lp, ll, lane, LZLIT_G);
        lp = nlp; op = nop; ll = nll; ml = nml;
    }
    __syncthreads();
    for (uint32_t q = 0; q < lq_n; q++) copy_g2g<U>(out + lq_op[q], lsrc + lq_lp[q], lq_ll[q], (int)threadIdx.x, (int)blockDim.x);
}

__global__ void __launch_bounds__(256) k_lz_literals_tiny(JobDev J) {
    const int lane = threadIdx.x & 31;
    const uint32_t bi = blockIdx.x * 8 + (threadIdx.x >> 5);
    if (bi >= J.n_blocks) return;
    const BlockDesc& B = J.blocks[bi];
    if (!tiny_lit_block(B)) return;
    if (J.frame_bad[B.frame]) return;
    const BlockState& S = J.bstate[bi];
    uint8_t* out = J.out + S.out_off;
    if (B.btype == BT_RAW) { copy_g2g(out, J.comp + B.src_off, B.src_size, lane, 32); return; }
    if (B.btype == BT_RLE) {
        const uint8_t v = J.comp[B.src_off];
        for (uint32_t i = lane; i < B.src_size; i += 32) out[i] = v;
        return;
    }
    const uint8_t* lsrc = nullptr;
    uint8_t rle = 0;
    if (B.lit_type == LT_RAW) lsrc = J.comp + B.src_off + B.lit_src;
    else if (B.lit_type == LT_RLE) rle = J.comp[B.src_off + B.lit_src];
    else lsrc = J.lit + B.lit_base;
    const uint32_t n = B.n_seq, base = B.seq_base;
    uint32_t lp = 0, op = 0, ll = 0, ml = 0;
    if ((uint32_t)lane < n) {
        const uint4 r = *(const uint4*)&J.seq[base + lane];
        ll = r.x; ml = r.y; lp = r.w; op = J.seq[base + lane].outpos;
        J.seq[base + lane].match_pos = S.out_off + op + ll;
    }
    uint32_t t_lp = 0, t_op = 0;
    if (n) {
        const uint32_t e_lp = __shfl_sync(0xFFFFFFFFu, lp + ll, (int)n - 1), e_op = __shfl_sync(0xFFFFFFFFu, op + ll + ml, (int)n - 1);
        t_lp = e_lp; t_op = e_op;
    }
    for (uint32_t i = 0; i <= n; i++) {
        uint32_t rl, rp, ro;
        if (i < n) { rl = __shfl_sync(0xFFFFFFFFu, ll, (int)i); rp = __shfl_sync(0xFFFFFFFFu, lp, (int)i); ro = __shfl_sync(0xFFFFFFFFu, op, (int)i); }
        else { rp = t_lp; ro = t_op; rl = B.lit_regen > t_lp ? B.lit_regen - t_lp : 0u; }
        if (rl == 0) continue;
        if (rp + rl > B.lit_regen) break;
        if (B.lit_type == LT_RLE) for (uint32_t k = lane; k < rl; k += 32) out[ro + k] = rle;
        else copy_g2g(out + ro, lsrc + rp, rl, lane, 32);
    }
}

__device__ __forceinline__ uint32_t resolve_offset(const JobDev& J, uint32_t v, uint32_t block) {
    if (!(v & OFF_SYMBOLIC)) return v;
    uint32_t in = J.bstate[block].rep_in[(v >> 29) & 3];
    uint32_t d = v & 0x1FFFFFFFu;
    return in > d ? in - d : 0;
}

__device__ __forceinline__ void copy_match(uint8_t* out, uint64_t d, uint32_t off, uint32_t ml, int lane, int nlanes) {
    const uint8_t* s = out + d - off;
    uint8_t* o = out + d;
    const bool periodic = off < ml;
    for (uint32_t k0 = 0; k0 < ml; k0 += 8u * (uint32_t)nlanes) {
        uint8_t t[8];
#pragma unroll
        for (uint32_t j = 0; j < 8; j++) {
            const uint32_t k = k0 + j * (uint32_t)nlanes + (uint32_t)lane;
            if (k < ml) t[j] = s[periodic ? k % off : k];
        }
#pragma unroll
        for (uint32_t j = 0; j < 8; j++) {
            const uint32_t k = k0 + j * (uint32_t)nlanes + (uint32_t)lane;
            if (k < ml) o[k] = t[j];
        }
    }
}

__device__ __forceinline__ void fill_run(uint8_t* dst, uint32_t v, uint32_t n, int lane, int nlanes) {
    const uint32_t h = (uint32_t)(-(intptr_t)dst) & 15u;
    if (n < 32u + h) { for (uint32_t k = lane; k < n; k += nlanes) dst[k] = (uint8_t)v; return; }
    if ((uint32_t)lane < h) dst[lane] = (uint8_t)v;
    const uint32_t body = (n - h) >> 4, w = v * 0x01010101u;
    uint4* d4 = (uint4*)(dst + h);
    for (uint32_t c = lane; c < body; c += nlanes) d4[c] = make_uint4(w, w, w, w);
    for (uint32_t k = h + (body << 4) + lane; k < n; k += nlanes) dst[k] = (uint8_t)v;
}

__device__ __forceinline__ void copy_long_match(uint8_t* out, uint64_t d, uint32_t off, uint32_t ml, int lane, int nlanes) {
    if (off >= ml) copy_g2g(out + d, out + d - off, ml, lane, nlanes);
    else if (off == 1) fill_run(out + d, out[d - 1], ml, lane, nlanes);
    else copy_match(out, d, off, ml, lane, nlanes);
}

constexpr uint32_t LZ_IDX_SHIFT = 12, LZ_IDX_PER_CHUNK = 65536u >> LZ_IDX_SHIFT;

__global__ void __launch_bounds__(256) k_lz_index(JobDev J) {
    const uint64_t i = (uint64_t)blockIdx.x * blockDim.x + threadIdx.x;
    if (i >= J.n_seq) return;
    const SeqRec& R = J.seq[i];
    const BlockDesc& B = J.blocks[R.block];
    const FrameDesc& F = J.frames[B.frame];
    if (J.frame_bad[B.frame]) return;
    uint32_t* ix = J.lz_idx + (size_t)J.fin_chunk_first[B.frame] * LZ_IDX_PER_CHUNK + B.frame;
    const uint64_t n_cells = (uint64_t)(J.fin_chunk_first[B.frame + 1] - J.fin_chunk_first[B.frame]) * LZ_IDX_PER_CHUNK + 1;
    const uint64_t e_prev = i == F.first_seq ? 0 : (J.seq[i - 1].match_pos + J.seq[i - 1].ml - F.dst_off);
    const uint64_t e = R.match_pos + R.ml - F.dst_off;
    uint64_t k0 = i == F.first_seq ? 0 : (e_prev + (1u << LZ_IDX_SHIFT) - 1) >> LZ_IDX_SHIFT;
    uint64_t k1 = (e + (1u << LZ_IDX_SHIFT) - 1) >> LZ_IDX_SHIFT;
    if (k1 > n_cells) k1 = n_cells;
    for (uint64_t k = k0; k < k1; k++) ix[k] = (uint32_t)i;
    if (i + 1 == (uint64_t)F.first_seq + F.n_seq) for (uint64_t k = k1; k < n_cells; k++) ix[k] = (uint32_t)(i + 1);
}

constexpr uint32_t LZ_SHORT = 64;
constexpr uint32_t LZ_WARP_MAX = 4096;
constexpr int LZ_CTA = 256;
constexpr int LZ_HOPS = 8;
constexpr uint32_t LZ_MIN_ROUNDS = 3, LZ_MIN_PENDING = 192;

__device__ __forceinline__ int lz_try(const JobDev& J, uint32_t i, uint32_t round, uint64_t& d, uint32_t& off, uint32_t& ml) {
    SeqRec& R = J.seq[i];
    const uint32_t bi = R.block;
    const BlockDesc& B = J.blocks[bi];
    if (J.frame_bad[B.frame]) { J.seq_done[i] = round; return 2; }
    const FrameDesc& F = J.frames[B.frame];
    ml = R.ml;
    const uint32_t off0 = resolve_offset(J, R.off, bi);
    off = off0;
    d = R.match_pos;
    int verdict = 0;
    for (int hop = 0; hop <= LZ_HOPS; hop++) {
        if (off == 0 || (uint64_t)off > d - F.dst_off) {
            flag_error(J, B.frame, zc::E_OFFSET);
            J.seq_done[i] = round;
            return 2;
        }
        const uint64_t s = d - off;
        const uint64_t e = (off < ml) ? d : s + ml;
        uint32_t lo = F.first_seq, hi = i;
        {
            const uint32_t* ix = J.lz_idx + (size_t)J.fin_chunk_first[B.frame] * LZ_IDX_PER_CHUNK + B.frame + ((s - F.dst_off) >> LZ_IDX_SHIFT);
            const uint32_t a = ix[0], b = ix[1];
            if (a > lo) lo = a;
            if (b < hi) hi = b;
            if (lo > hi) lo = hi;
        }
        while (lo < hi) {
            const uint32_t mid = (lo + hi) >> 1;
            if (J.seq[mid].match_pos + J.seq[mid].ml > s) hi = mid; else lo = mid + 1;
        }
        uint32_t blocker = 0xFFFFFFFFu;
        for (uint32_t j = lo; j < i && J.seq[j].match_pos < e; j++) {
            const uint32_t dn = J.seq_done[j];
            if (dn == 0 || dn >= round) { blocker = j; break; }
        }
        if (blocker == 0xFFFFFFFFu) { verdict = 1; break; }
        const SeqRec& Q = J.seq[blocker];
        if (hop == LZ_HOPS || off < ml || Q.match_pos > s || e > Q.match_pos + Q.ml) { J.lz_blocker[i] = blocker; break; }
        off += resolve_offset(J, Q.off, Q.block);
    }
    if (off != off0) R.off = off;
    return verdict;
}

constexpr int LZ_U = 4;

__device__ __forceinline__ void lz_round(const JobDev& J, const uint32_t* list, uint32_t n, uint32_t round, uint32_t* next, uint32_t* next_n,
                                         uint32_t first, uint32_t stride,
                                         uint32_t* q_n, uint64_t* q_d, uint32_t* q_off, uint32_t* q_ml, uint32_t* q_i) {
    const int tid = threadIdx.x, lane = tid & 31;
    for (uint32_t base = first; base < n; base += stride * LZ_U) {
        if (tid == 0) *q_n = 0;
        __syncthreads();
        uint32_t idx[LZ_U];
        bool look[LZ_U], pend[LZ_U];
#pragma unroll
        for (int u = 0; u < LZ_U; u++) {
            const uint32_t k = base + (uint32_t)u * stride + (uint32_t)tid;
            look[u] = false; pend[u] = false; idx[u] = 0;
            if (k < n) {
                const uint32_t i = list ? list[k] : k;
                idx[u] = i;
                if (J.seq_done[i] == 0) {
                    look[u] = true;
                    if (round > 1u + J.lz_flow_early) {
                        const uint32_t b = J.lz_blocker[i];
                        if (b != 0xFFFFFFFFu) { const uint32_t dn = J.seq_done[b]; if (dn == 0 || dn >= round) { look[u] = false; pend[u] = true; } }
                    }
                }
            }
        }
#pragma unroll
        for (int u = 0; u < LZ_U; u++) {
            if (look[u]) {
                uint64_t d; uint32_t off, ml;
                const int v = lz_try(J, idx[u], round, d, off, ml);
                if (v == 0) pend[u] = true;
                else if (v == 1) {
                    if (ml <= LZ_SHORT) { copy_match(J.out, d, off, ml, 0, 1); J.seq_done[idx[u]] = round; }
                    else {
                        const uint32_t slot = atomicAdd(q_n, 1u);
                        if (slot < (uint32_t)LZ_CTA) { q_d[slot] = d; q_off[slot] = off; q_ml[slot] = ml; q_i[slot] = idx[u]; }
                        else pend[u] = true;
                    }
                }
            }
        }
#pragma unroll
        for (int u = 0; u < LZ_U; u++) {
            const uint32_t pb = __ballot_sync(0xFFFFFFFFu, pend[u]);
            uint32_t wbase = 0;
            if (lane == 0 && pb) wbase = atomicAdd(next_n, (uint32_t)__popc(pb));
            wbase = __shfl_sync(0xFFFFFFFFu, wbase, 0);
            if (pend[u]) next[wbase + __popc(pb & ((1u << lane) - 1u))] = idx[u];
        }
        __syncthreads();
        uint32_t nq = *q_n;
        if (nq > (uint32_t)LZ_CTA) nq = LZ_CTA;
        for (uint32_t t = (uint32_t)tid >> 5; t < nq; t += LZ_CTA / 32)
            if (q_ml[t] <= LZ_WARP_MAX) copy_long_match(J.out, q_d[t], q_off[t], q_ml[t], lane, 32);
        for (uint32_t t = 0; t < nq; t++)
            if (q_ml[t] > LZ_WARP_MAX) copy_long_match(J.out, q_d[t], q_off[t], q_ml[t], tid, LZ_CTA);
        if ((uint32_t)tid < nq) J.seq_done[q_i[tid]] = round;
        __syncthreads();
    }
}

#define LZ_SHARED_QUEUE \
    __shared__ uint32_t q_n; __shared__ uint64_t q_d[LZ_CTA]; __shared__ uint32_t q_off[LZ_CTA], q_ml[LZ_CTA], q_i[LZ_CTA]

__global__ void __launch_bounds__(LZ_CTA, 4) k_lz_first(JobDev J) {
    LZ_SHARED_QUEUE;
    lz_round(J, nullptr, (uint32_t)J.n_seq, 1u + J.lz_flow_early, J.lz_list[0], &J.lz_count[0], blockIdx.x * LZ_CTA, gridDim.x * LZ_CTA,
             &q_n, q_d, q_off, q_ml, q_i);
}

__global__ void __launch_bounds__(LZ_CTA) k_lz_resolve(JobDev J) {
    LZ_SHARED_QUEUE;
    uint32_t cur = 0;
    const uint32_t r0 = J.lz_flow_early;
    for (uint32_t round = 2 + r0;; round++) {
        const uint32_t nxt = cur == 2 ? 0 : cur + 1, clr = nxt == 2 ? 0 : nxt + 1;
        const uint32_t n = J.lz_count[cur];
        if (blockIdx.x == 0 && threadIdx.x == 0) { *J.lz_rounds = round - 1 - r0; if (round - 2 - r0 < 24) J.lz_pending[round - 2 - r0] = n; }
        if (n == 0) break;
        if (blockIdx.x == 0 && threadIdx.x == 0) J.lz_count[clr] = 0;
        lz_round(J, J.lz_list[cur], n, round, J.lz_list[nxt], &J.lz_count[nxt], blockIdx.x * LZ_CTA, gridDim.x * LZ_CTA,
                 &q_n, q_d, q_off, q_ml, q_i);
        NAF_GRID_SYNC();
        const uint32_t n_next = J.lz_count[nxt];
        cur = nxt;
        const uint32_t progress = n - n_next;
        const uint64_t round_ns = 5000 + n_next / 25;
        if (round >= LZ_MIN_ROUNDS + r0 && n_next > LZ_MIN_PENDING && J.lz_flow_on) {
            const uint64_t est = (uint64_t)n_next / (progress ? progress : 1u);
            if ((est >= 8 && est <= 256) || J.lz_flow_on == 2u) {
                if (blockIdx.x == 0 && threadIdx.x == 0) *J.lz_flow = 1;
                break;
            }
        }
        if (round >= LZ_MIN_ROUNDS + r0 && n_next > LZ_MIN_PENDING &&
            (uint64_t)n_next * round_ns > (uint64_t)(progress ? progress : 1u) * J.fin_cost_us * 1000u) {
            if (blockIdx.x == 0 && threadIdx.x == 0) *J.lz_handover = round - r0;
            break;
        }
    }
}

__device__ __forceinline__ unsigned long long flow_now_ns() {
#if defined(__CUDA_ARCH__)
    unsigned long long t; asm volatile("mov.u64 %0, %%globaltimer;" : "=l"(t)); return t;
#else
    return 0ull;
#endif
}

constexpr int LZF_T = 256;

constexpr unsigned long long LZF_EARLY_NS = 60000ull;

__global__ void __launch_bounds__(LZF_T) k_lz_flow(JobDev J, int early) {
    if (!early && *J.lz_flow == 0) return;
    volatile uint32_t* done = J.seq_done;
    volatile uint32_t* abort_flag = J.lz_flow + (early ? 4 : 2);
    uint32_t* const ticket = J.lz_flow + (early ? 3 : 1);
    const int lane = threadIdx.x & 31;
    const uint32_t n = (uint32_t)J.n_seq;
    const uint32_t stamp = early ? 1u : 0x7FFFFFFFu;
    const unsigned long long deadline = flow_now_ns() + (early ? LZF_EARLY_NS : (unsigned long long)J.fin_cost_us * 1000ull);
    for (;;) {
        uint32_t base = 0;
        if (lane == 0) base = atomicAdd(ticket, 32u);
        base = __shfl_sync(0xFFFFFFFFu, base, 0);
        if (base >= n) return;
        const uint32_t i = base + (uint32_t)lane;
        bool active = i < n && done[i] == 0;
        uint64_t d = 0, e = 0;
        uint32_t off = 0, ml = 0, j = 0, frame = 0;
        if (active) {
            const SeqRec& R = J.seq[i];
            const BlockDesc& B = J.blocks[R.block];
            frame = B.frame;
            const FrameDesc& F = J.frames[frame];
            if (J.frame_bad[frame]) { done[i] = stamp; active = false; }
            else {
                ml = R.ml; d = R.match_pos; off = resolve_offset(J, R.off, R.block);
                if (off == 0 || (uint64_t)off > d - F.dst_off) { flag_error(J, frame, zc::E_OFFSET); done[i] = stamp; active = false; }
                else {
                    const uint64_t sp = d - off;
                    e = off < ml ? d : sp + ml;
                    uint32_t lo = F.first_seq, hi = i;
                    const uint32_t* ix = J.lz_idx + (size_t)J.fin_chunk_first[frame] * LZ_IDX_PER_CHUNK + frame + ((sp - F.dst_off) >> LZ_IDX_SHIFT);
                    const uint32_t a = ix[0], b = ix[1];
                    if (a > lo) lo = a;
                    if (b < hi) hi = b;
                    if (lo > hi) lo = hi;
                    while (lo < hi) { const uint32_t mid = (lo + hi) >> 1; if (J.seq[mid].match_pos + J.seq[mid].ml > sp) hi = mid; else lo = mid + 1; }
                    j = lo;
                }
            }
        }
        uint32_t idle = 0;
        while (__any_sync(0xFFFFFFFFu, active)) {
            bool ready = false;
            if (active) {
                while (j < i && J.seq[j].match_pos < e && done[j] != 0) j++;
                ready = !(j < i && J.seq[j].match_pos < e);
            }
            const uint32_t rb = __ballot_sync(0xFFFFFFFFu, ready);
            if (rb) {
                __threadfence();
                for (uint32_t m = rb; m; m &= m - 1) {
                    const int src = __ffs((int)m) - 1;
                    const uint64_t dd = ((uint64_t)__shfl_sync(0xFFFFFFFFu, (uint32_t)(d >> 32), src) << 32) | __shfl_sync(0xFFFFFFFFu, (uint32_t)d, src);
                    const uint32_t oo = __shfl_sync(0xFFFFFFFFu, off, src), mm = __shfl_sync(0xFFFFFFFFu, ml, src);
                    if (oo >= mm) copy_g2g_1rt<4>(J.out + dd, J.out + dd - oo, mm, lane, 32);
                    else copy_long_match(J.out, dd, oo, mm, lane, 32);
                }
                __threadfence();
                if (ready) { done[i] = stamp; active = false; }
                idle = 0;
                continue;
            }
            if ((++idle & 63u) == 0) {
                uint32_t stop = 0;
                if (lane == 0) { stop = *abort_flag; if (!stop && flow_now_ns() > deadline) { *abort_flag = 1; stop = 1; } }
                if (__shfl_sync(0xFFFFFFFFu, stop, 0)) {
                    if (lane == 0 && !early) atomicMax(J.lz_handover, *J.lz_rounds + 1u);
                    return;
                }
            }
#if defined(__CUDA_ARCH__)
            __nanosleep(100);
#endif
        }
        uint32_t stop = 0;
        if (lane == 0) stop = *abort_flag;
        if (__shfl_sync(0xFFFFFFFFu, stop, 0)) { if (lane == 0 && !early) atomicMax(J.lz_handover, *J.lz_rounds + 1u); return; }
    }
}

constexpr uint32_t LZS_MAX = 8192;
constexpr int LZS_T = 1024;
__host__ __device__ constexpr uint32_t lzs_smem_bytes(uint32_t n) { return ((n + 3u) & ~3u) * 24u; }

__global__ void __launch_bounds__(LZS_T) k_lz_small(JobDev J) {
    NAF_DYN_SMEM(uint32_t, lzs);
    const uint32_t n = (uint32_t)J.n_seq, np = (n + 3u) & ~3u;
    uint32_t* pos = lzs;
    uint32_t* mlen = pos + np;
    uint32_t* moff = mlen + np;
    uint16_t* done = (uint16_t*)(moff + np);
    uint16_t* frm = done + np;
    uint32_t* q_i = (uint32_t*)(frm + np);
    uint32_t* q_off = q_i + np;
    __shared__ uint32_t q_n, q_big, s_pending[3];
    const int tid = threadIdx.x, lane = tid & 31;
    for (uint32_t i = tid; i < n; i += LZS_T) {
        const SeqRec& R = J.seq[i];
        const BlockDesc& B = J.blocks[R.block];
        pos[i] = (uint32_t)R.match_pos; mlen[i] = R.ml; frm[i] = (uint16_t)B.frame;
        moff[i] = resolve_offset(J, R.off, R.block);
        done[i] = J.frame_bad[B.frame] ? 1 : 0;
    }
    if (tid == 0) { s_pending[0] = s_pending[1] = s_pending[2] = 0; }
    __shared__ uint32_t fr_first[64], fr_off[64];
    const bool fr_cached = J.n_frames <= 64u;
    if (fr_cached && (uint32_t)tid < J.n_frames) { fr_first[tid] = J.frames[tid].first_seq; fr_off[tid] = (uint32_t)J.frames[tid].dst_off; }
    __syncthreads();
    long long t_probe = 0, t_copy = 0, t0 = 0, t_begin = 0;
    SEQ_CLK(t_begin);
    uint32_t prev_pending = n, handover = 0, round = 1;
    for (;; round++) {
        if (tid == 0) { q_n = 0; q_big = 0; s_pending[(round + 1) % 3] = 0; }
        __syncthreads();
        SEQ_CLK(t0);
        uint32_t mine = 0;
        for (uint32_t i = tid; i < n; i += LZS_T) {
            if (done[i]) continue;
            const uint32_t f = frm[i];
            const uint32_t f_first = fr_cached ? fr_first[f] : J.frames[f].first_seq, f_off = fr_cached ? fr_off[f] : (uint32_t)J.frames[f].dst_off;
            const uint32_t d = pos[i], ml = mlen[i];
            uint32_t off = moff[i];
            int verdict = 0;
            for (int hop = 0; hop <= LZ_HOPS; hop++) {
                if (off == 0 || off > d - f_off) { flag_error(J, f, zc::E_OFFSET); verdict = 2; break; }
                const uint32_t sp = d - off, e = off < ml ? d : sp + ml;
                uint32_t lo = f_first, hi = i;
                while (lo < hi) { const uint32_t mid = (lo + hi) >> 1; if (pos[mid] + mlen[mid] > sp) hi = mid; else lo = mid + 1; }
                uint32_t blocker = 0xFFFFFFFFu;
                for (uint32_t j = lo; j < i && pos[j] < e; j++) {
                    const uint32_t dn = done[j];
                    if (dn == 0 || dn >= round) { blocker = j; break; }
                }
                if (blocker == 0xFFFFFFFFu) { verdict = 1; break; }
                if (hop == LZ_HOPS || off < ml || pos[blocker] > sp || e > pos[blocker] + mlen[blocker]) break;
                off += moff[blocker];
            }
            moff[i] = off;
            if (verdict == 2) done[i] = (uint16_t)round;
            else if (verdict == 1) {
                const bool big = ml > 2048u && off >= ml;
                const uint32_t slot = big ? np - 1u - atomicAdd(&q_big, 1u) : atomicAdd(&q_n, 1u);
                q_i[slot] = i; q_off[slot] = off;
            }
            else mine++;
        }
        if (mine) atomicAdd(&s_pending[round % 3], mine);
        __syncthreads();
        SEQ_LAP(t_probe, t0);
        const uint32_t nq = q_n, nbig = q_big;
        {
            const uint32_t warp = (uint32_t)tid >> 5, NW = LZS_T / 32;
            for (uint32_t t = warp; t < nq; t += NW) {
                const uint32_t i = q_i[t], ml = mlen[i], off = q_off[t];
                if (off >= ml) copy_g2g<4>(J.out + pos[i], J.out + pos[i] - off, ml, lane, 32);
                else copy_long_match(J.out, pos[i], off, ml, lane, 32);
            }
            for (uint32_t t = 0; t < nbig; t++) {
                const uint32_t i = q_i[np - 1u - t], ml = mlen[i], off = q_off[np - 1u - t], d = pos[i];
                for (uint32_t pc = (warp + NW - (t & (NW - 1))) & (NW - 1); pc * 2048u < ml; pc += NW) {
                    const uint32_t b = pc * 2048u, len = ml - b < 2048u ? ml - b : 2048u;
                    copy_g2g<4>(J.out + d + b, J.out + d - off + b, len, lane, 32);
                }
            }
        }
        __syncthreads();
        SEQ_LAP(t_copy, t0);
        for (uint32_t t = tid; t < nq; t += LZS_T) done[q_i[t]] = (uint16_t)round;
        for (uint32_t t = tid; t < nbig; t += LZS_T) done[q_i[np - 1u - t]] = (uint16_t)round;
        __syncthreads();
        const uint32_t pending = s_pending[round % 3];
        if (tid == 0 && round - 1 < 24) J.lz_pending[round - 1] = pending;
        if (pending == 0) break;
        const uint32_t progress = prev_pending - pending;
        if (round >= LZ_MIN_ROUNDS && pending > LZ_MIN_PENDING && round < 60000u &&
            (uint64_t)pending * (1500u + pending / 2u) > (uint64_t)(progress ? progress : 1u) * J.fin_cost_us * 1000u) { handover = round; break; }
        if (round >= 60000u) { handover = round; break; }
        prev_pending = pending;
    }
    for (uint32_t i = tid; i < n; i += LZS_T) J.seq_done[i] = done[i];
    if (tid == 0) { *J.lz_rounds = round; if (handover) *J.lz_handover = handover; }
    long long t_end = 0;
    SEQ_CLK(t_end);
    if (J.debug_seq && tid == 0) { J.debug_seq[5] = (unsigned long long)t_probe; J.debug_seq[6] = (unsigned long long)t_copy; J.debug_seq[7] = (unsigned long long)(t_end - t_begin); }
}

constexpr uint32_t FIN_C = 65536;
constexpr uint32_t FIN_T = 1024;
constexpr uint32_t FIN_U = 4;
constexpr uint32_t FIN_INLINE = 64;
constexpr uint32_t FIN_SMEM = FIN_C + FIN_C * 2 + FIN_C / 8 + FIN_T * 20;
constexpr int FIN2_T = 256;

__device__ __forceinline__ void fin_byte(uint16_t* ptr, uint32_t* extbit, uint32_t* g, uint32_t e, int32_t s) {
    if (s >= 0) ptr[e] = (uint16_t)s;
    else { g[e] = (uint32_t)((int32_t)e - s); atomicOr(&extbit[e >> 5], 1u << (e & 31)); }
}

__device__ __forceinline__ uint32_t fin_frame_of(const JobDev& J, uint32_t c) {
    uint32_t lo = 0, hi = J.n_frames;
    while (hi - lo > 1) { const uint32_t mid = (lo + hi) >> 1; if (J.fin_chunk_first[mid] <= c) lo = mid; else hi = mid; }
    return lo;
}

__global__ void __launch_bounds__(FIN_T) k_lz_finish(JobDev J) {
    if (*J.lz_handover == 0) return;
    NAF_DYN_SMEM(unsigned char, fin_smem);
    uint8_t* val = fin_smem;
    uint16_t* ptr = (uint16_t*)(fin_smem + FIN_C);
    uint32_t* extbit = (uint32_t*)(fin_smem + FIN_C * 3);
    uint32_t* q_rel = extbit + FIN_C / 32;
    uint32_t* q_len = q_rel + FIN_T;
    uint32_t* q_off = q_len + FIN_T;
    uint32_t* q_m0 = q_off + FIN_T;
    uint32_t* q_ml = q_m0 + FIN_T;
    __shared__ uint32_t s_f, s_mi, s_q, s_bad, s_unres;
    const uint32_t tid = threadIdx.x;

    for (uint32_t c = blockIdx.x; c < J.fin_total_chunks; c += gridDim.x) {
        __syncthreads();
        if (tid == 0) {
            const uint32_t f = fin_frame_of(J, c);
            s_f = f; s_bad = 0; s_unres = 0;
            if (!J.lz_small) s_mi = J.frames[f].n_seq ? J.lz_idx[(size_t)c * LZ_IDX_PER_CHUNK + f] : J.frames[f].first_seq;
            else {
                const uint64_t cs = J.frames[f].dst_off + (uint64_t)(c - J.fin_chunk_first[f]) * FIN_C;
                uint32_t lo = J.frames[f].first_seq, hi = lo + J.frames[f].n_seq;
                while (lo < hi) { const uint32_t mid = (lo + hi) >> 1; if (J.seq[mid].match_pos + J.seq[mid].ml > cs) hi = mid; else lo = mid + 1; }
                s_mi = lo;
            }
        }
        __syncthreads();
        const uint32_t f = s_f, mi = s_mi;
        if (J.frame_bad[f]) continue;
        const uint64_t f0 = J.frames[f].dst_off, fend = f0 + J.frames[f].dst_size;
        const uint32_t end = J.frames[f].first_seq + J.frames[f].n_seq;
        const uint64_t c0 = f0 + (uint64_t)(c - J.fin_chunk_first[f]) * FIN_C;
        const uint64_t c1 = (c0 + FIN_C < fend) ? c0 + FIN_C : fend;
        const uint32_t cn = (uint32_t)(c1 - c0);
        uint8_t* out_c0 = J.out + c0;
        uint32_t* g = J.fin_g + J.fin_g_base[f] + (size_t)(c - J.fin_chunk_first[f]) * FIN_C;
        bool mine = false;
        for (uint32_t base = mi;; base += FIN_T) {
            const uint32_t i = base + tid;
            bool stop = i >= end;
            if (!stop) {
                const SeqRec& R = J.seq[i];
                if (R.match_pos >= c1) stop = true;
                else if (J.seq_done[i] == 0) mine = true;
            }
            if (__syncthreads_or(stop || mine)) break;
        }
        if (!__syncthreads_or(mine)) continue;
        for (uint32_t e = tid * 16; e < FIN_C; e += FIN_T * 16) {
            uint32_t* p2 = (uint32_t*)(ptr + e);
#pragma unroll
            for (uint32_t k = 0; k < 8; k++) p2[k] = (e + 2 * k) | ((e + 2 * k + 1) << 16);
            if (e < cn) {
                *(uint4*)(val + e) = __ldcg((const uint4*)(out_c0 + e));
#pragma unroll
                for (uint32_t k = 0; k < 4; k++) ((uint4*)(g + e))[k] = make_uint4(0, 0, 0, 0);
            }
        }
        for (uint32_t e = tid; e < FIN_C / 32; e += FIN_T) extbit[e] = 0;
        __syncthreads();
        for (uint32_t base = mi;; base += FIN_T * FIN_U) {
            if (tid == 0) s_q = 0;
            __syncthreads();
            uint64_t pos[FIN_U];
            uint32_t ml[FIN_U], ov[FIN_U], blk[FIN_U];
            bool pend[FIN_U];
#pragma unroll
            for (uint32_t j = 0; j < FIN_U; j++) {
                const uint32_t i = base + j * FIN_T + tid;
                pos[j] = ~0ull; ml[j] = 0; ov[j] = 0; blk[j] = 0; pend[j] = false;
                if (i < end) {
                    const SeqRec& R = J.seq[i];
                    pos[j] = R.match_pos; ml[j] = R.ml; ov[j] = R.off; blk[j] = R.block; pend[j] = J.seq_done[i] == 0;
                }
            }
            bool stop = false;
#pragma unroll
            for (uint32_t j = 0; j < FIN_U; j++) {
                const uint32_t i = base + j * FIN_T + tid;
                if (i >= end || pos[j] >= c1) stop = true;
                else if (pend[j] && pos[j] + ml[j] > c0) {
                    const uint32_t off = resolve_offset(J, ov[j], blk[j]);
                    if (off == 0 || (uint64_t)off > pos[j] - f0 || off > 0x7F000000u) { flag_error(J, f, zc::E_OFFSET); s_bad = 1; }
                    else {
                        const uint64_t b0 = pos[j] > c0 ? pos[j] : c0, b1 = pos[j] + ml[j] < c1 ? pos[j] + ml[j] : c1;
                        const uint32_t rel = (uint32_t)(b0 - c0), len = (uint32_t)(b1 - b0), m0 = (uint32_t)(b0 - pos[j]);
                        const int32_t srel = (int32_t)((int64_t)(pos[j] - off) - (int64_t)c0);
                        if (len > FIN_INLINE) {
                            const uint32_t slot = atomicAdd(&s_q, 1u);
                            q_rel[slot] = rel; q_len[slot] = len; q_off[slot] = off; q_m0[slot] = m0; q_ml[slot] = ml[j];
                        } else if (off >= ml[j]) {
                            int32_t sp = srel + (int32_t)m0;
                            for (uint32_t k = 0; k < len; k++, sp++) fin_byte(ptr, extbit, g, rel + k, sp);
                        } else {
                            uint32_t r = m0 % off;
                            for (uint32_t k = 0; k < len; k++) { fin_byte(ptr, extbit, g, rel + k, srel + (int32_t)r); if (++r == off) r = 0; }
                        }
                    }
                }
            }
            const int all_stop = __syncthreads_or(stop);
            const uint32_t nq = s_q;
            for (uint32_t t = 0; t < nq; t++) {
                const uint32_t rel = q_rel[t], len = q_len[t], off = q_off[t], m0 = q_m0[t], mlen = q_ml[t];
                const int32_t srel = (int32_t)rel - (int32_t)m0 - (int32_t)off;
                for (uint32_t k = tid; k < len; k += FIN_T)
                    fin_byte(ptr, extbit, g, rel + k, srel + (int32_t)(off < mlen ? (m0 + k) % off : m0 + k));
            }
            if (all_stop) break;
            __syncthreads();
        }
        __syncthreads();
        if (s_bad) continue;
        for (;;) {
            bool changed = false;
            for (uint32_t e = tid; e < cn; e += FIN_T) {
                const uint32_t p = ptr[e];
                if (p != e) { const uint32_t pp = ptr[p]; if (pp != p) { ptr[e] = (uint16_t)pp; changed = true; } }
            }
            if (!__syncthreads_or(changed)) break;
        }
        uint32_t unres = 0;
        for (uint32_t e = tid; e < cn; e += FIN_T) {
            const uint32_t p = ptr[e];
            const bool ext = (extbit[p >> 5] >> (p & 31)) & 1u;
            if (p != e) {
                if (ext) { g[e] = e - p; unres++; }
                else out_c0[e] = val[p];
            } else if (ext) unres++;
        }
        if (unres) atomicAdd(&s_unres, unres);
        __syncthreads();
        if (s_unres) {
            uint32_t* xb = J.fin_ext + (size_t)c * (FIN_C / 32);
            for (uint32_t e = tid; e < FIN_C / 32; e += FIN_T) xb[e] = extbit[e];
        }
        if (tid == 0 && s_unres) { J.fin_chunk_flag[c] = 1; atomicAdd(J.fin_unresolved, s_unres); }
    }
}

constexpr uint32_t FIN2_U = 8;
constexpr uint32_t FIN2_TILE = FIN2_T * 32;

__global__ void __launch_bounds__(FIN2_T) k_lz_finish2(JobDev J) {
    if (*J.lz_handover == 0 || *J.fin_unresolved == 0) return;
    __shared__ uint32_t s_left, s_wsum[FIN2_T / 32];
    __shared__ uint16_t s_root[FIN2_TILE];
    const uint32_t tid = threadIdx.x, lane = tid & 31, warp = tid >> 5;
    volatile uint32_t* G = J.fin_g;
    volatile uint32_t* flag = J.fin_chunk_flag;
    for (uint32_t round = 0;; round++) {
        const uint32_t cur = round % 3, clr = (round + 1) % 3;
        if (blockIdx.x == 0 && tid == 0) J.fin_count[clr] = 0;
        uint32_t left_total = 0;
        for (uint32_t c = blockIdx.x; c < J.fin_total_chunks; c += gridDim.x) {
            if (flag[c] != 1) continue;
            __syncthreads();
            if (tid == 0) s_left = 0;
            const uint32_t f = fin_frame_of(J, c);
            const uint32_t cf = J.fin_chunk_first[f];
            const size_t gb = (size_t)J.fin_g_base[f];
            const uint64_t f0 = J.frames[f].dst_off;
            const uint64_t crel = (uint64_t)(c - cf) * FIN_C;
            const uint32_t* xb = J.fin_ext + (size_t)c * (FIN_C / 32);
            uint32_t left = 0;
            for (uint32_t t0 = 0; t0 < FIN_C; t0 += FIN2_TILE) {
                const uint32_t word = xb[(t0 >> 5) + tid];
                if (!__syncthreads_or(word != 0)) continue;
                const uint32_t cnt = __popc(word);
                uint32_t inc = cnt;
#pragma unroll
                for (int d = 1; d < 32; d <<= 1) { const uint32_t v = __shfl_up_sync(0xFFFFFFFFu, inc, d); if ((int)lane >= d) inc += v; }
                if (lane == 31) s_wsum[warp] = inc;
                __syncthreads();
                uint32_t before = inc - cnt, total = 0;
                for (uint32_t w = 0; w < FIN2_T / 32; w++) { const uint32_t v = s_wsum[w]; if (w < warp) before += v; total += v; }
                for (uint32_t m = word, k = before; m; m &= m - 1, k++) s_root[k] = (uint16_t)(t0 + tid * 32 + (uint32_t)(__ffs(m) - 1));
                __syncthreads();
                for (uint32_t k0 = tid; k0 < total; k0 += FIN2_T * FIN2_U) {
                    uint32_t re[FIN2_U], rd[FIN2_U], rs[FIN2_U];
                    uint8_t rv[FIN2_U];
#pragma unroll
                    for (uint32_t u = 0; u < FIN2_U; u++) {
                        const uint32_t k = k0 + u * FIN2_T;
                        rs[u] = 0; re[u] = 0; rd[u] = 0; rv[u] = 0;
                        if (k >= total) continue;
                        const uint32_t e = s_root[k];
                        const uint32_t dist = G[gb + crel + e];
                        if (dist == 0) continue;
                        const uint64_t prel = crel + e;
                        if (dist > prel) { flag_error(J, f, zc::E_OFFSET); G[gb + crel + e] = 0; continue; }
                        const uint64_t srel = prel - dist;
                        const uint32_t sc = cf + (uint32_t)(srel >> 16);
                        uint32_t gs = 0;
                        if (flag[sc] != 0) gs = G[gb + srel];
                        re[u] = e;
                        if (gs == 0) { rs[u] = 1; rd[u] = dist; }
                        else {
                            const uint64_t nd = (uint64_t)dist + gs;
                            if (nd > 0xFFFFFFFFull) { flag_error(J, f, zc::E_SIZE); G[gb + crel + e] = 0; continue; }
                            rs[u] = 2; rd[u] = (uint32_t)nd;
                        }
                    }
                    __threadfence();
#pragma unroll
                    for (uint32_t u = 0; u < FIN2_U; u++)
                        if (rs[u] == 1) rv[u] = *(volatile const uint8_t*)(J.out + f0 + crel + re[u] - rd[u]);
#pragma unroll
                    for (uint32_t u = 0; u < FIN2_U; u++)
                        if (rs[u] == 1) J.out[f0 + crel + re[u]] = rv[u];
                    __threadfence();
#pragma unroll
                    for (uint32_t u = 0; u < FIN2_U; u++) {
                        if (rs[u] == 1) G[gb + crel + re[u]] = 0;
                        else if (rs[u] == 2) { G[gb + crel + re[u]] = rd[u]; left++; }
                    }
                }
                __syncthreads();
            }
            if (left) atomicAdd(&s_left, left);
            __syncthreads();
            if (tid == 0) {
                if (s_left == 0) { __threadfence(); flag[c] = 2; }
                left_total += s_left;
            }
        }
        if (tid == 0 && left_total) atomicAdd(&J.fin_count[cur], left_total);
        NAF_GRID_SYNC();
        if (J.fin_count[cur] == 0) break;
    }
    for (uint32_t c = blockIdx.x; c < J.fin_total_chunks; c += gridDim.x) {
        if (flag[c] == 0) continue;
        const uint32_t f = fin_frame_of(J, c);
        const uint64_t f0 = J.frames[f].dst_off, fend = f0 + J.frames[f].dst_size;
        const uint64_t crel = (uint64_t)(c - J.fin_chunk_first[f]) * FIN_C;
        const uint32_t cn = (uint32_t)((crel + FIN_C < fend - f0) ? FIN_C : fend - f0 - crel);
        const uint32_t* g = J.fin_g + J.fin_g_base[f] + crel;
        uint8_t* o = J.out + f0 + crel;
        for (uint32_t e0 = tid * 4; e0 < cn; e0 += FIN2_T * 4) {
            const uint4 d = __ldcg((const uint4*)(g + e0));
            const uint32_t dd[4] = {d.x, d.y, d.z, d.w};
#pragma unroll
            for (uint32_t k = 0; k < 4; k++)
                if (dd[k] != 0 && e0 + k < cn && dd[k] <= e0 + k) o[e0 + k] = __ldcg(o + e0 + k - dd[k]);
        }
    }
}

__device__ __forceinline__ uint64_t xxh_rotl(uint64_t x, int r) { return (x << r) | (x >> (64 - r)); }
constexpr uint64_t XXP1 = 0x9E3779B185EBCA87ull, XXP2 = 0xC2B2AE3D27D4EB4Full, XXP3 = 0x165667B19E3779F9ull, XXP4 = 0x85EBCA77C2B2AE63ull,
                   XXP5 = 0x27D4EB2F165667C5ull;
__device__ __forceinline__ uint64_t xxh_round(uint64_t acc, uint64_t in) { return xxh_rotl(acc + in * XXP2, 31) * XXP1; }
__device__ __forceinline__ uint64_t xxh_merge(uint64_t h, uint64_t v) { return (h ^ xxh_round(0, v)) * XXP1 + XXP4; }

__global__ void __launch_bounds__(32) k_frame_checksum(JobDev J) {
    const uint32_t f = blockIdx.x;
    const FrameDesc& F = J.frames[f];
    if (!F.has_checksum || J.frame_bad[f]) return;
    const int lane = threadIdx.x;
    const uint8_t* p = J.out + F.dst_off;
    const uint64_t len = F.dst_size, stripes = len >> 5;
    uint64_t h;
    if (stripes) {
        uint64_t v = lane == 0 ? XXP1 + XXP2 : (lane == 1 ? XXP2 : (lane == 2 ? 0ull : 0ull - XXP1));
        if (lane < 4) {
            const uint64_t* q = (const uint64_t*)p + lane;
            uint64_t s = 0;
            for (; s + 8 <= stripes; s += 8) {
                uint64_t in[8];
#pragma unroll
                for (int k = 0; k < 8; k++) in[k] = q[4 * (s + k)];
#pragma unroll
                for (int k = 0; k < 8; k++) v = xxh_round(v, in[k]);
            }
            for (; s < stripes; s++) v = xxh_round(v, q[4 * s]);
        }
        const uint64_t v1 = __shfl_sync(0xFFFFFFFFu, v, 0), v2 = __shfl_sync(0xFFFFFFFFu, v, 1), v3 = __shfl_sync(0xFFFFFFFFu, v, 2),
                       v4 = __shfl_sync(0xFFFFFFFFu, v, 3);
        h = xxh_rotl(v1, 1) + xxh_rotl(v2, 7) + xxh_rotl(v3, 12) + xxh_rotl(v4, 18);
        h = xxh_merge(h, v1); h = xxh_merge(h, v2); h = xxh_merge(h, v3); h = xxh_merge(h, v4);
    } else h = XXP5;
    if (lane != 0) return;
    h += len;
    uint64_t i = stripes << 5;
    for (; i + 8 <= len; i += 8) { h ^= xxh_round(0, *(const uint64_t*)(p + i)); h = xxh_rotl(h, 27) * XXP1 + XXP4; }
    if (i + 4 <= len) { h ^= (uint64_t)(*(const uint32_t*)(p + i)) * XXP1; h = xxh_rotl(h, 23) * XXP2 + XXP3; i += 4; }
    for (; i < len; i++) { h ^= (uint64_t)p[i] * XXP5; h = xxh_rotl(h, 11) * XXP1; }
    h ^= h >> 33; h *= XXP2; h ^= h >> 29; h *= XXP3; h ^= h >> 32;
    if ((uint32_t)h != F.checksum) flag_error(J, f, zc::E_CHECKSUM);
}

uint32_t lz_resolve_max_ctas(int device) {
#if defined(NAFGPU_EMULATE)
    (void)device;
    return 1;
#else
    int sms = 0, per_sm = 0;
    cudaDeviceGetAttribute(&sms, cudaDevAttrMultiProcessorCount, device);
    cudaOccupancyMaxActiveBlocksPerMultiprocessor(&per_sm, k_lz_resolve, LZ_CTA, 0);
    if (per_sm > 4) per_sm = 4;
    return (uint32_t)(sms > 0 && per_sm > 0 ? sms * per_sm : 1);
#endif
}

void lz_finish_ctas(int device, uint32_t* level1, uint32_t* level2) {
#if defined(NAFGPU_EMULATE)
    (void)device;
    *level1 = 2; *level2 = 1;
#else
    int sms = 0, per_sm = 0;
    cudaDeviceGetAttribute(&sms, cudaDevAttrMultiProcessorCount, device);
    cudaOccupancyMaxActiveBlocksPerMultiprocessor(&per_sm, k_lz_finish2, FIN2_T, 0);
    if (per_sm > 4) per_sm = 4;
    *level1 = (uint32_t)(sms > 0 ? sms : 1);
    *level2 = (uint32_t)(sms > 0 && per_sm > 0 ? sms * per_sm : 1);
#endif
}

int launch_zstd_stage(const JobDev& J, cudaStream_t st, cudaStream_t st2, cudaEvent_t fork, cudaEvent_t join, StageEvents* ev,
                      cudaStream_t st3, cudaEvent_t fork3, cudaEvent_t join3, cudaEvent_t fork4, cudaEvent_t join4) {
    StageEvents none;
    if (!ev) ev = &none;
    int launches = 0;
    if (J.n_blocks == 0) { for (int i = 0; i < ZSTD_STAGES; i++) ev->mark(); return 0; }
    cudaStream_t sb = st2 ? st2 : st;
    (void)sb;
    if (st2) { cudaEventRecord(fork, st); cudaStreamWaitEvent(st2, fork, 0); }
    if (J.n_huf_items) {
        NAF_LAUNCH(k_build_tables<1>, J.n_blocks, 32, 0, sb, J); launches++;
        const bool side = st2 && st3 && J.n_huf_big && J.n_huf_items > J.n_huf_big;
        (void)side;
        if (side) {
            cudaEventRecord(fork3, sb); cudaStreamWaitEvent(st3, fork3, 0);
            const uint32_t smem = huf_fixed_smem(HUF_T_SMALL) + ((J.max_huf_small + 15 + 16 + 16 + 15) & ~15u);
            NAF_LAUNCH((k_huf_decode<HUF_T_SMALL>), J.n_huf_items - J.n_huf_big, HUF_T_SMALL, smem, st3, J, J.huf_items + J.n_huf_big); launches++;
            cudaEventRecord(join3, st3);
        }
        if (J.n_huf_big) {
            const uint32_t smem = hb_smem_bytes(J.max_huf_stream);
            if (!st2) ev->kernel_begin();
            const bool per_block = J.n_huf_big / 4 >= (J.huf_block_min ? J.huf_block_min : 296u);
            if (per_block) {
                NAF_SET_MAX_SMEM(k_huf_decode_block, smem);
                NAF_LAUNCH(k_huf_decode_block, J.n_huf_big / 4, HB_T, smem, sb, J); launches++;
            } else {
                NAF_SET_MAX_SMEM(k_huf_decode_big, smem);
                NAF_LAUNCH(k_huf_decode_big, J.n_huf_big, HB_T, smem, sb, J); launches++;
            }
            if (!st2) ev->kernel_end();
        }
        if (side) cudaStreamWaitEvent(sb, join3, 0);
        else if (J.n_huf_items > J.n_huf_big) {
            const uint32_t smem = huf_fixed_smem(HUF_T_SMALL) + ((J.max_huf_small + 15 + 16 + 16 + 15) & ~15u);
            NAF_LAUNCH((k_huf_decode<HUF_T_SMALL>), J.n_huf_items - J.n_huf_big, HUF_T_SMALL, smem, sb, J, J.huf_items + J.n_huf_big); launches++;
        }
    }
    if (st2) cudaEventRecord(join, st2);
    else ev->mark();
    NAF_LAUNCH(k_build_tables<0>, J.n_blocks + 1, 96, 0, st, J); launches++; ev->mark();
    const bool seq_side = st2 && st3 && J.tiny_blocks && J.n_seq_big;
    (void)seq_side;
    if (seq_side) {
        cudaEventRecord(fork4, st); cudaStreamWaitEvent(st3, fork4, 0);
        NAF_LAUNCH(k_decode_sequences, J.n_seq_big, 64, J.seq_stage_bytes, st3, J); launches++;
        cudaEventRecord(join4, st3);
    }
    if (J.tiny_blocks) { NAF_LAUNCH(k_decode_sequences_tiny, (J.n_blocks + SEQ_TINY_WARPS - 1) / SEQ_TINY_WARPS, SEQ_TINY_WARPS * 32, 0, st, J); launches++; }
    if (seq_side) cudaStreamWaitEvent(st, join4, 0);
    else if (!J.tiny_blocks || J.n_seq_big) { NAF_LAUNCH(k_decode_sequences, J.tiny_blocks ? J.n_seq_big : J.n_blocks, 64, J.seq_stage_bytes, st, J); launches++; }
    ev->mark();
    NAF_LAUNCH(k_frame_scan, J.n_frames, FSCAN_T, 0, st, J); launches++;
    if (J.n_fs_tiles) {
        NAF_LAUNCH(k_fs_reduce, J.n_fs_tiles, FSCAN_T, 0, st, J);
        NAF_LAUNCH(k_fs_prefix, J.n_fs_big, 32, 0, st, J);
        NAF_LAUNCH(k_fs_apply, J.n_fs_tiles, FSCAN_T, 0, st, J);
        launches += 3;
    }
    ev->mark();
    if (st2) { cudaStreamWaitEvent(st, join, 0); ev->mark(); }
    if (J.tiny_blocks) { NAF_LAUNCH(k_lz_literals_tiny, (J.n_blocks + 7) / 8, 256, 0, st, J); launches++; }
    const uint32_t lit_blocks = J.tiny_blocks ? J.n_lit_big : J.n_blocks;
    if (lit_blocks == 0) {}
    else if (lit_blocks <= 64u) { NAF_LAUNCH(k_lz_literals<4>, dim3(lit_blocks, 4 * LZLIT_SPLIT), 256, 0, st, J); launches++; }
    else { NAF_LAUNCH(k_lz_literals<1>, dim3(lit_blocks, lit_blocks > 16384u ? 1 : LZLIT_SPLIT), 256, 0, st, J); launches++; }
    ev->mark();
    if (J.n_seq > 0) {
        if (J.lz_small) {
            const uint32_t smem = lzs_smem_bytes((uint32_t)J.n_seq);
            NAF_SET_MAX_SMEM(k_lz_small, smem);
            NAF_LAUNCH(k_lz_small, 1, LZS_T, smem, st, J); launches++;
            ev->mark(); ev->mark();
        } else {
        uint32_t grid = (uint32_t)((J.n_seq + LZ_CTA - 1) / LZ_CTA);
        if (grid > 148u * 8u) grid = std::max<uint32_t>(148u * 8u, (uint32_t)((J.n_seq + LZ_CTA * LZ_U - 1) / (LZ_CTA * LZ_U)));
        if (grid > 148u * 64u) grid = 148u * 64u;
        NAF_LAUNCH(k_lz_index, (uint32_t)((J.n_seq + 255) / 256), 256, 0, st, J); launches++;
        if (J.lz_flow_early) { NAF_LAUNCH(k_lz_flow, J.flow_ctas ? J.flow_ctas : 1u, LZF_T, 0, st, J, 1); launches++; }
        NAF_LAUNCH(k_lz_first, grid, LZ_CTA, 0, st, J); launches++;
        ev->mark();
        uint32_t cg = J.coop_ctas ? J.coop_ctas : 1u;
        { const uint64_t want = (J.n_seq + LZ_CTA * 2 - 1) / (LZ_CTA * 2); if (want < cg) cg = want < 8 ? 8u : (uint32_t)want; if (cg > (J.coop_ctas ? J.coop_ctas : 1u)) cg = J.coop_ctas ? J.coop_ctas : 1u; }
        (void)cg;
        JobDev Jc = J;
        NAF_LAUNCH_COOP(k_lz_resolve, cg, LZ_CTA, st, Jc); launches++;
        if (J.lz_flow_on) { NAF_LAUNCH(k_lz_flow, J.flow_ctas ? J.flow_ctas : 1u, LZF_T, 0, st, J, 0); launches++; }
        ev->mark();
        }
        JobDev Jc = J;
        const uint32_t fin_grid = J.fin_total_chunks < J.fin_ctas ? J.fin_total_chunks : J.fin_ctas;
        if (fin_grid && J.n_seq > LZ_MIN_PENDING) {
            NAF_SET_MAX_SMEM(k_lz_finish, FIN_SMEM);
            NAF_LAUNCH(k_lz_finish, fin_grid, FIN_T, FIN_SMEM, st, J); launches++;
            uint32_t cg2 = J.fin2_ctas ? J.fin2_ctas : 1u;
            if (J.fin_total_chunks * 2u < cg2) cg2 = J.fin_total_chunks * 2u < 8u ? 8u : J.fin_total_chunks * 2u;
            if (cg2 > (J.fin2_ctas ? J.fin2_ctas : 1u)) cg2 = J.fin2_ctas ? J.fin2_ctas : 1u;
            (void)cg2;
            NAF_LAUNCH_COOP(k_lz_finish2, cg2, FIN2_T, st, Jc); launches++;
        }
        ev->mark();
    } else { ev->mark(); ev->mark(); ev->mark(); }
    if (J.n_checksums) { NAF_LAUNCH(k_frame_checksum, J.n_frames, 32, 0, st, J); launches++; }
    return launches;
}

}
```

Before: 441.0.

## Decode nucleotide 4-bit data directly to ASCII inside zstd literal and match stages

Nucleotide sequence frames now carry an ASCII output offset and IUPAC lookup word. Literals are expanded to letter pairs as they are written, and matches are copied in the letter domain. The finish and checksum stages repack the letters to nibbles when needed. The standalone unpack kernel now runs only when a mask is present, and only ORs lowercase bits into the ASCII output. This removes a full pass that reread the packed data and rewrote the ASCII buffer, but it adds pack/expand work in the finish kernels, doubles match-copy byte volume, and complicates the checksum path.

```diff
diff --git a/nafcodec_b200/csrc/naf_kernels.cu b/nafcodec_b200/csrc/naf_kernels.cu
--- a/nafcodec_b200/csrc/naf_kernels.cu
+++ b/nafcodec_b200/csrc/naf_kernels.cu
@@ -1,4 +1,5 @@
 #include "naf_kernels.cuh"
+#include "naf_load.cuh"
 
 #include <algorithm>
 
@@ -268,119 +269,95 @@
     }
 }
 
-__device__ __forceinline__ uint32_t prmt(uint32_t a, uint32_t b, uint32_t s) {
-#if defined(__CUDA_ARCH__)
-    uint32_t d;
-    asm("prmt.b32 %0, %1, %2, %3;" : "=r"(d) : "r"(a), "r"(b), "r"(s));
-    return d;
-#else
-    return __byte_perm(a, b, s);
-#endif
-}
-
-__device__ __forceinline__ uint32_t iupac4(uint32_t x16, uint32_t l0) {
-    const uint32_t sel = x16 & 0x7777u;
-    const uint32_t lo = prmt(l0, 0x42535943u, sel);
-    const uint32_t hi = prmt(0x44525741u, 0x4E56484Du, sel);
-    const uint32_t m = prmt(0x80808080u, 0u, x16 & 0x8888u);
-    return (lo & ~m) | (hi & m);
-}
-
 __device__ __forceinline__ uint32_t spread4_x20(uint32_t q) {
     return ((q * 0x00204081u) & 0x01010101u) << 5;
 }
 
 __global__ void __launch_bounds__(UNPACK_T) k_unpack(uint8_t* arena, const NafDev* archives) {
     const NafDev& A = archives[blockIdx.y];
-    if (!(A.has & HAS_SEQUENCE) || A.seq_type > 1 || blockIdx.x >= A.n_chunks) return;
-    __shared__ uint32_t wp[32], wp2[32];
-    __shared__ uint32_t wball, cball;
+    if (!(A.has & HAS_SEQUENCE) || !(A.has & HAS_MASK) || A.seq_type > 1 || blockIdx.x >= A.n_chunks) return;
+    __shared__ uint32_t wpar[UNPACK_T / 32], wcar[UNPACK_T / 32];
     const NafCounts* counts = (const NafCounts*)(arena + A.counts_off);
     const uint64_t total = counts->total_residues < A.seq_residues ? counts->total_residues : A.seq_residues;
     const uint64_t wi = (uint64_t)blockIdx.x * CHUNK_WORDS + UNPACK_W * threadIdx.x;
     const uint64_t r0 = wi * 32;
     uint32_t mask[UNPACK_W];
-#pragma unroll
-    for (uint32_t k = 0; k < UNPACK_W; k++) mask[k] = 0;
-    if (A.has & HAS_MASK) {
+    {
         const uint32_t* bits = (const uint32_t*)(arena + A.mask_bits_off);
+        const uint32_t* cpar = (const uint32_t*)(arena + A.chunk_par_off);
         const uint64_t n_words = (A.seq_residues + 32) / 32;
+        uint32_t w[UNPACK_W];
+#pragma unroll
+        for (uint32_t k = 0; k < UNPACK_W; k++) w[k] = wi + k < n_words ? bits[wi + k] : 0;
+        uint32_t cp = 0;
+        for (uint32_t c = threadIdx.x; c < blockIdx.x; c += blockDim.x) cp ^= cpar[c];
         uint32_t par = 0;
 #pragma unroll
         for (uint32_t k = 0; k < UNPACK_W; k++) {
-            const uint32_t w = wi + k < n_words ? bits[wi + k] : 0;
-            uint32_t m = w;
+            uint32_t m = w[k];
             m ^= m << 1; m ^= m << 2; m ^= m << 4; m ^= m << 8; m ^= m << 16;
             mask[k] = par ? ~m : m;
-            par ^= __popc(w) & 1;
+            par ^= __popc(w[k]) & 1;
         }
         const int lane = threadIdx.x & 31, warp = threadIdx.x >> 5;
-        uint32_t b = __ballot_sync(FULL, par);
-        if (lane == 0) wp[warp] = __popc(b) & 1;
+        const uint32_t b = __ballot_sync(FULL, par), cb = __ballot_sync(FULL, cp & 1);
+        if (lane == 0) { wpar[warp] = __popc(b) & 1; wcar[warp] = __popc(cb) & 1; }
         __syncthreads();
-        if (warp == 0) { uint32_t bb = __ballot_sync(FULL, lane < (int)(UNPACK_T / 32) ? wp[lane] : 0u); if (lane == 0) wball = bb; }
-        __syncthreads();
-        const uint32_t* cpar = (const uint32_t*)(arena + A.chunk_par_off);
-        uint32_t cp = 0;
-        for (uint32_t c = threadIdx.x; c < blockIdx.x; c += blockDim.x) cp ^= cpar[c];
-        const uint32_t cb = __ballot_sync(FULL, cp & 1);
-        if (lane == 0) wp2[warp] = __popc(cb) & 1;
-        __syncthreads();
-        if (warp == 0) { uint32_t bb = __ballot_sync(FULL, lane < (int)(UNPACK_T / 32) ? wp2[lane] : 0u); if (lane == 0) cball = bb; }
-        __syncthreads();
-        const uint32_t carry = (__popc(cball) & 1) ^ (__popc(wball & ((1u << warp) - 1u)) & 1) ^ (__popc(b & ((1u << lane) - 1u)) & 1);
+        uint32_t carry = __popc(b & ((1u << lane) - 1u)) & 1;
+#pragma unroll
+        for (int v = 0; v < (int)(UNPACK_T / 32); v++) carry ^= wcar[v] ^ (v < warp ? wpar[v] : 0u);
         if (carry) {
 #pragma unroll
             for (uint32_t k = 0; k < UNPACK_W; k++) mask[k] = ~mask[k];
         }
     }
     if (r0 >= total) return;
-    const uint32_t l0 = A.seq_type == 1 ? 0x4B47552Du : 0x4B47542Du;
-    const uint4* src = (const uint4*)(arena + A.seq_off + r0 / 2);
-    uint4 pk[UNPACK_W];
-#pragma unroll
-    for (uint32_t k = 0; k < UNPACK_W; k++) {
-        pk[k] = make_uint4(0, 0, 0, 0);
-        if (r0 + 32 * k < total) pk[k] = src[k];
-    }
     uint4* dst = (uint4*)(arena + A.ascii_off + r0);
 #pragma unroll
-    for (uint32_t k = 0; k < UNPACK_W; k++) {
-        if (r0 + 32 * k >= total) break;
-        const uint32_t x[4] = {pk[k].x, pk[k].y, pk[k].z, pk[k].w};
-        uint32_t o[8];
-#pragma unroll
-        for (int j = 0; j < 4; j++) {
-            o[2 * j] = iupac4(x[j] & 0xFFFFu, l0) | spread4_x20((mask[k] >> (8 * j)) & 0xFu);
-            o[2 * j + 1] = iupac4(x[j] >> 16, l0) | spread4_x20((mask[k] >> (8 * j + 4)) & 0xFu);
-        }
-        dst[2 * k] = make_uint4(o[0], o[1], o[2], o[3]);
-        dst[2 * k + 1] = make_uint4(o[4], o[5], o[6], o[7]);
-    }
-}
-
-__global__ void __launch_bounds__(CHUNK_WORDS) k_text_mask(uint8_t* arena, const NafDev* archives) {
+    for (uint32_t k = 0; k < UNPACK_W; k++)
+        if (r0 + 32 * k >= total) mask[k] = 0;
+#pragma unroll
+    for (uint32_t k0 = 0; k0 < UNPACK_W; k0 += 4) {
+        uint4 v[8];
+#pragma unroll
+        for (uint32_t k = 0; k < 4; k++)
+            if (mask[k0 + k]) { v[2 * k] = dst[2 * (k0 + k)]; v[2 * k + 1] = dst[2 * (k0 + k) + 1]; }
+#pragma unroll
+        for (uint32_t k = 0; k < 4; k++) {
+            const uint32_t m = mask[k0 + k];
+            if (!m) continue;
+            uint4 a = v[2 * k], b = v[2 * k + 1];
+            a.x |= spread4_x20(m & 0xFu); a.y |= spread4_x20((m >> 4) & 0xFu); a.z |= spread4_x20((m >> 8) & 0xFu); a.w |= spread4_x20((m >> 12) & 0xFu);
+            b.x |= spread4_x20((m >> 16) & 0xFu); b.y |= spread4_x20((m >> 20) & 0xFu); b.z |= spread4_x20((m >> 24) & 0xFu); b.w |= spread4_x20(m >> 28);
+            dst[2 * (k0 + k)] = a;
+            dst[2 * (k0 + k) + 1] = b;
+        }
+    }
+}
+
+constexpr uint32_t TEXT_MASK_T = 256;
+__global__ void __launch_bounds__(TEXT_MASK_T) k_text_mask(uint8_t* arena, const NafDev* archives) {
     const NafDev& A = archives[blockIdx.y];
     if (!(A.has & HAS_SEQUENCE) || !(A.has & HAS_MASK) || A.seq_type <= 1 || blockIdx.x >= A.n_chunks) return;
     const NafCounts* counts = (const NafCounts*)(arena + A.counts_off);
     const uint64_t total = counts->total_residues < A.seq_residues ? counts->total_residues : A.seq_residues;
-    const uint64_t wi = (uint64_t)blockIdx.x * CHUNK_WORDS + threadIdx.x;
     const uint32_t* bits = (const uint32_t*)(arena + A.mask_bits_off);
     const uint32_t* par = (const uint32_t*)(arena + A.chunk_par_off);
     const uint64_t n_words = (A.seq_residues + 32) / 32;
-    if (wi >= n_words) return;
-    uint32_t carry = 0;
-    for (uint32_t c = 0; c < blockIdx.x; c++) carry ^= par[c] & 1;
-    for (uint64_t j = (uint64_t)blockIdx.x * CHUNK_WORDS; j < wi; j++) carry ^= __popc(bits[j]) & 1;
-    uint32_t m = bits[wi];
-    m ^= m << 1; m ^= m << 2; m ^= m << 4; m ^= m << 8; m ^= m << 16;
-    if (carry) m = ~m;
-    uint8_t* s = arena + A.seq_off;
-    for (int j = 0; j < 32; j++) {
-        uint64_t i = wi * 32 + j;
-        if (i >= total) break;
-        uint8_t c = s[i];
-        if (((m >> j) & 1) && c >= 'A' && c <= 'Z') s[i] = c | 0x20;
+    for (uint64_t wi = (uint64_t)blockIdx.x * CHUNK_WORDS + threadIdx.x; wi < (uint64_t)(blockIdx.x + 1) * CHUNK_WORDS && wi < n_words; wi += TEXT_MASK_T) {
+        uint32_t carry = 0;
+        for (uint32_t c = 0; c < blockIdx.x; c++) carry ^= par[c] & 1;
+        for (uint64_t j = (uint64_t)blockIdx.x * CHUNK_WORDS; j < wi; j++) carry ^= __popc(bits[j]) & 1;
+        uint32_t m = bits[wi];
+        m ^= m << 1; m ^= m << 2; m ^= m << 4; m ^= m << 8; m ^= m << 16;
+        if (carry) m = ~m;
+        uint8_t* s = arena + A.seq_off;
+        for (int j = 0; j < 32; j++) {
+            uint64_t i = wi * 32 + j;
+            if (i >= total) break;
+            uint8_t c = s[i];
+            if (((m >> j) & 1) && c >= 'A' && c <= 'Z') s[i] = c | 0x20;
+        }
     }
 }
 
@@ -473,9 +450,9 @@
         ev->mark();
         ev->mark();
     } else { ev->mark(); ev->mark(); }
-    if (max_chunks > 0) {
+    if (max_chunks > 0 && any_mask) {
         NAF_LAUNCH(k_unpack, dim3(max_chunks, n_archives), UNPACK_T, 0, st, arena, archives); launches++;
-        if (any_text_mask) { NAF_LAUNCH(k_text_mask, dim3(max_chunks, n_archives), CHUNK_WORDS, 0, st, arena, archives); launches++; }
+        if (any_text_mask) { NAF_LAUNCH(k_text_mask, dim3(max_chunks, n_archives), TEXT_MASK_T, 0, st, arena, archives); launches++; }
     }
     ev->mark();
     if (max_text_bytes > 0) {
diff --git a/nafcodec_b200/csrc/naf_kernels.cuh b/nafcodec_b200/csrc/naf_kernels.cuh
--- a/nafcodec_b200/csrc/naf_kernels.cuh
+++ b/nafcodec_b200/csrc/naf_kernels.cuh
@@ -7,7 +7,7 @@
 enum : uint32_t { HAS_IDS = 1, HAS_COMMENTS = 2, HAS_LENGTHS = 4, HAS_MASK = 8, HAS_SEQUENCE = 16, HAS_QUALITY = 32 };
 
 constexpr uint32_t UNPACK_T = 256;
-constexpr uint32_t UNPACK_W = 2;
+constexpr uint32_t UNPACK_W = 8;
 constexpr uint32_t CHUNK_WORDS = UNPACK_W * UNPACK_T;
 constexpr uint32_t CHUNK_RESIDUES = CHUNK_WORDS * 32;
 constexpr uint64_t NO_RECORD = ~0ull;
diff --git a/nafcodec_b200/csrc/naf_load.cuh b/nafcodec_b200/csrc/naf_load.cuh
--- a/nafcodec_b200/csrc/naf_load.cuh
+++ b/nafcodec_b200/csrc/naf_load.cuh
@@ -18,4 +18,37 @@
     return make_uint4(o[0], o[1], o[2], o[3]);
 }
 
+__device__ __forceinline__ uint32_t prmt(uint32_t a, uint32_t b, uint32_t s) {
+#if defined(__CUDA_ARCH__)
+    uint32_t d;
+    asm("prmt.b32 %0, %1, %2, %3;" : "=r"(d) : "r"(a), "r"(b), "r"(s));
+    return d;
+#else
+    return __byte_perm(a, b, s);
+#endif
 }
+
+constexpr uint32_t IUPAC_LO_DNA = 0x4B47542Du, IUPAC_LO_RNA = 0x4B47552Du;
+
+__device__ __forceinline__ uint32_t iupac4(uint32_t x16, uint32_t l0) {
+    const uint32_t sel = x16 & 0x7777u;
+    const uint32_t lo = prmt(l0, 0x42535943u, sel);
+    const uint32_t hi = prmt(0x44525741u, 0x4E56484Du, sel);
+    const uint32_t m = prmt(0x80808080u, 0u, x16 & 0x8888u);
+    return (lo & ~m) | (hi & m);
+}
+
+__device__ __forceinline__ uint32_t iupac_code(uint32_t c) {
+    const uint32_t i = c & 31u, w = i < 16u ? (i < 8u ? 0x200B4780u : 0x0FC0300Du) : (i < 24u ? 0x9E116A00u : 0x00000050u);
+    return c < 0x40u ? 0u : (w >> ((i & 7u) * 4u)) & 15u;
+}
+
+__device__ __forceinline__ uint64_t iupac_pack16(uint4 v) {
+    const uint32_t w[4] = {v.x, v.y, v.z, v.w};
+    uint64_t r = 0;
+#pragma unroll
+    for (int j = 0; j < 16; j++) r |= (uint64_t)iupac_code((w[j >> 2] >> (8 * (j & 3))) & 0xFFu) << (4 * j);
+    return r;
+}
+
+}
diff --git a/nafcodec_b200/csrc/nafgpu_api.cu b/nafcodec_b200/csrc/nafgpu_api.cu
--- a/nafcodec_b200/csrc/nafgpu_api.cu
+++ b/nafcodec_b200/csrc/nafgpu_api.cu
@@ -293,7 +293,14 @@
         const fw::JobPlan& L = T.plan;
         T.bo = nb; T.so = (uint32_t)G.seq_total; T.lo = G.lit_total - 16; T.slot_off = G.n_slots - 3; T.ho = G.n_huf_slots;
         if (G.seq_total + L.seq_total > 0xFFFFFFF0ull || nb + L.blocks.size() > 0xFFFFFFF0ull) return fail(c, NAFGPU_ERR_UNSUPPORTED, "job has too many blocks or sequences: split the batch");
-        for (zf::FrameDesc F : L.frames) { F.first_block += (uint32_t)T.bo; F.first_seq += T.so; G.frames.push_back(F); }
+        for (zf::FrameDesc F : L.frames) {
+            F.first_block += (uint32_t)T.bo; F.first_seq += T.so;
+            if (T.sec == NAFGPU_SEC_SEQUENCE && c->aplan[T.arch].nucleotide) {
+                F.ascii_off = c->arch[T.arch].ascii_off;
+                F.direct_lut = c->arch[T.arch].seq_type == 1 ? nk::IUPAC_LO_RNA : nk::IUPAC_LO_DNA;
+            }
+            G.frames.push_back(F);
+        }
         if (!T.first) {
             zf::FrameDesc& F = G.frames.back();
             F.n_blocks += T.st.n_blocks; F.n_seq += T.st.n_seq;
diff --git a/nafcodec_b200/csrc/zstd_format.h b/nafcodec_b200/csrc/zstd_format.h
--- a/nafcodec_b200/csrc/zstd_format.h
+++ b/nafcodec_b200/csrc/zstd_format.h
@@ -24,6 +24,9 @@
     uint64_t window;
     uint32_t has_checksum;
     uint32_t checksum;
+    uint64_t ascii_off;
+    uint32_t direct_lut;
+    uint32_t _pad;
 };
 
 struct BlockDesc {
diff --git a/nafcodec_b200/csrc/zstd_kernels.cu b/nafcodec_b200/csrc/zstd_kernels.cu
--- a/nafcodec_b200/csrc/zstd_kernels.cu
+++ b/nafcodec_b200/csrc/zstd_kernels.cu
@@ -1,6 +1,8 @@
 #include "zstd_kernels.cuh"
 
 #include <algorithm>
+
+#include "naf_load.cuh"
 
 namespace zk {
 
@@ -1842,33 +1844,73 @@
     if (tk < n) dst[tk] = tb;
 }
 
+__device__ __forceinline__ uint32_t iupac_pair(uint32_t b, uint32_t l0) { return nk::iupac4(b, l0) & 0xFFFFu; }
+
+__device__ __forceinline__ void expand_g2g(uint8_t* __restrict__ dst, const uint8_t* __restrict__ src, uint32_t n, int lane, int nlanes, uint32_t l0) {
+    const uint32_t h = ((uint32_t)(-(intptr_t)dst) & 15u) >> 1;
+    if (n < h + 16u) { for (uint32_t k = lane; k < n; k += nlanes) *(uint16_t*)(dst + 2 * k) = (uint16_t)iupac_pair(src[k], l0); return; }
+    const uint32_t body = (n - h) >> 4;
+    const uintptr_t sa = (uintptr_t)(src + h);
+    const uint4* sw = (const uint4*)(sa & ~(uintptr_t)15);
+    const uint32_t mis = (uint32_t)(sa & 15), q = mis >> 2, sh = (mis & 3) * 8;
+    uint4* d4 = (uint4*)(dst + 2 * h);
+    for (uint32_t c = lane; c < body; c += nlanes) {
+        const uint4 A = sw[c], B = sw[c + 1];
+        uint32_t w0, w1, w2, w3, w4;
+        if (q == 0) { w0 = A.x; w1 = A.y; w2 = A.z; w3 = A.w; w4 = B.x; }
+        else if (q == 1) { w0 = A.y; w1 = A.z; w2 = A.w; w3 = B.x; w4 = B.y; }
+        else if (q == 2) { w0 = A.z; w1 = A.w; w2 = B.x; w3 = B.y; w4 = B.z; }
+        else { w0 = A.w; w1 = B.x; w2 = B.y; w3 = B.z; w4 = B.w; }
+        const uint32_t p0 = __funnelshift_r(w0, w1, sh), p1 = __funnelshift_r(w1, w2, sh), p2 = __funnelshift_r(w2, w3, sh), p3 = __funnelshift_r(w3, w4, sh);
+        d4[2 * c] = make_uint4(nk::iupac4(p0 & 0xFFFFu, l0), nk::iupac4(p0 >> 16, l0), nk::iupac4(p1 & 0xFFFFu, l0), nk::iupac4(p1 >> 16, l0));
+        d4[2 * c + 1] = make_uint4(nk::iupac4(p2 & 0xFFFFu, l0), nk::iupac4(p2 >> 16, l0), nk::iupac4(p3 & 0xFFFFu, l0), nk::iupac4(p3 >> 16, l0));
+    }
+    if ((uint32_t)lane < h) *(uint16_t*)(dst + 2 * lane) = (uint16_t)iupac_pair(src[lane], l0);
+    for (uint32_t k = h + (body << 4) + lane; k < n; k += nlanes) *(uint16_t*)(dst + 2 * k) = (uint16_t)iupac_pair(src[k], l0);
+}
+
+__device__ __forceinline__ void fill_run(uint8_t* dst, uint32_t w, uint32_t n, int lane, int nlanes) {
+    const uint32_t h = (uint32_t)(-(intptr_t)dst) & 15u;
+    if (n < 32u + h) { for (uint32_t k = lane; k < n; k += nlanes) dst[k] = (uint8_t)(w >> (8 * ((uintptr_t)(dst + k) & 3))); return; }
+    if ((uint32_t)lane < h) dst[lane] = (uint8_t)(w >> (8 * ((uintptr_t)(dst + lane) & 3)));
+    const uint32_t body = (n - h) >> 4;
+    uint4* d4 = (uint4*)(dst + h);
+    for (uint32_t c = lane; c < body; c += nlanes) d4[c] = make_uint4(w, w, w, w);
+    for (uint32_t k = h + (body << 4) + lane; k < n; k += nlanes) dst[k] = (uint8_t)(w >> (8 * ((uintptr_t)(dst + k) & 3)));
+}
+
 constexpr int LZLIT_G = 32;
 constexpr int LZLIT_SPLIT = 4;
 constexpr uint32_t LZLIT_LONG = 4096;
 
-template <int U>
-__global__ void __launch_bounds__(256, U == 1 ? 6 : 1) k_lz_literals(JobDev J) {
+template <int U, bool D>
+__device__ __forceinline__ void put_run(uint8_t* out, uint32_t p, const uint8_t* src, uint32_t n, int lane, int nlanes, uint32_t l0) {
+    if (D) expand_g2g(out + 2 * p, src, n, lane, nlanes, l0);
+    else copy_g2g<U>(out + p, src, n, lane, nlanes);
+}
+template <bool D>
+__device__ __forceinline__ uint32_t rle_word(uint32_t v, uint32_t l0) { return D ? iupac_pair(v, l0) * 0x00010001u : v * 0x01010101u; }
+template <bool D>
+__device__ __forceinline__ void rle_run(uint8_t* out, uint32_t p, uint32_t w, uint32_t n, int lane, int nlanes) {
+    if (D) for (uint32_t k = lane; k < n; k += nlanes) *(uint16_t*)(out + 2 * (p + k)) = (uint16_t)w;
+    else for (uint32_t k = lane; k < n; k += nlanes) out[p + k] = (uint8_t)w;
+}
+
+template <int U, bool D>
+__device__ __forceinline__ void lz_literals_block(const JobDev& J, const BlockDesc& B, const BlockState& S, uint8_t* out, uint32_t l0) {
     __shared__ uint32_t lq_n, lq_lp[40], lq_op[40], lq_ll[40];
-    const uint32_t bi = J.tiny_blocks ? J.lit_big_list[blockIdx.x] : blockIdx.x;
-    const BlockDesc& B = J.blocks[bi];
-    if (J.frame_bad[B.frame]) return;
-    const BlockState& S = J.bstate[bi];
-    uint8_t* out = J.out + S.out_off;
+    constexpr uint32_t sc = D ? 1 : 0;
     const int tid = threadIdx.x + blockIdx.y * blockDim.x, nt = blockDim.x * gridDim.y;
-    if (B.btype == BT_RAW) { copy_g2g(out, J.comp + B.src_off, B.src_size, tid, nt); return; }
-    if (B.btype == BT_RLE) {
-        uint8_t v = J.comp[B.src_off];
-        for (uint32_t i = tid; i < B.src_size; i += nt) out[i] = v;
-        return;
-    }
+    if (B.btype == BT_RAW) { put_run<1, D>(out, 0, J.comp + B.src_off, B.src_size, tid, nt, l0); return; }
+    if (B.btype == BT_RLE) { fill_run(out, rle_word<D>(J.comp[B.src_off], l0), B.src_size << sc, tid, nt); return; }
     const uint8_t* lsrc = nullptr;
-    uint8_t rle = 0;
+    uint32_t rle = 0;
     if (B.lit_type == LT_RAW) lsrc = J.comp + B.src_off + B.lit_src;
-    else if (B.lit_type == LT_RLE) rle = J.comp[B.src_off + B.lit_src];
+    else if (B.lit_type == LT_RLE) rle = rle_word<D>(J.comp[B.src_off + B.lit_src], l0);
     else lsrc = J.lit + B.lit_base;
     if (B.n_seq == 0) {
-        if (B.lit_type == LT_RLE) for (uint32_t i = tid; i < B.lit_regen; i += nt) out[i] = rle;
-        else copy_g2g(out, lsrc, B.lit_regen, tid, nt);
+        if (B.lit_type == LT_RLE) fill_run(out, rle, B.lit_regen << sc, tid, nt);
+        else put_run<1, D>(out, 0, lsrc, B.lit_regen, tid, nt, l0);
         return;
     }
     const int lane = tid % LZLIT_G, ng = nt / LZLIT_G, grp = U > 1 ? (int)(threadIdx.x / LZLIT_G) * (int)gridDim.y + (int)blockIdx.y : tid / LZLIT_G;
@@ -1893,12 +1935,56 @@
         }
         if (ll > LZLIT_LONG && B.lit_type != LT_RLE) {
             if (lane == 0) { const uint32_t q = atomicAdd(&lq_n, 1u); lq_lp[q] = lp; lq_op[q] = op; lq_ll[q] = ll; }
-        } else if (B.lit_type == LT_RLE) for (uint32_t k = lane; k < ll; k += LZLIT_G) out[op + k] = rle;
-        else copy_g2g(out + op, lsrc + lp, ll, lane, LZLIT_G);
+        } else if (B.lit_type == LT_RLE) rle_run<D>(out, op, rle, ll, lane, LZLIT_G);
+        else put_run<1, D>(out, op, lsrc + lp, ll, lane, LZLIT_G, l0);
         lp = nlp; op = nop; ll = nll; ml = nml;
     }
     __syncthreads();
-    for (uint32_t q = 0; q < lq_n; q++) copy_g2g<U>(out + lq_op[q], lsrc + lq_lp[q], lq_ll[q], (int)threadIdx.x, (int)blockDim.x);
+    for (uint32_t q = 0; q < lq_n; q++) put_run<U, D>(out, lq_op[q], lsrc + lq_lp[q], lq_ll[q], (int)threadIdx.x, (int)blockDim.x, l0);
+}
+
+template <int U>
+__global__ void __launch_bounds__(256, U == 1 ? 6 : 1) k_lz_literals(JobDev J) {
+    const uint32_t bi = J.tiny_blocks ? J.lit_big_list[blockIdx.x] : blockIdx.x;
+    const BlockDesc& B = J.blocks[bi];
+    if (J.frame_bad[B.frame]) return;
+    const BlockState& S = J.bstate[bi];
+    const FrameDesc& F = J.frames[B.frame];
+    if (F.direct_lut) lz_literals_block<U, true>(J, B, S, J.out + F.ascii_off + 2 * (S.out_off - F.dst_off), F.direct_lut);
+    else lz_literals_block<U, false>(J, B, S, J.out + S.out_off, 0);
+}
+
+template <bool D>
+__device__ __forceinline__ void lz_literals_tiny_block(const JobDev& J, const BlockDesc& B, const BlockState& S, uint8_t* out, uint32_t l0, int lane) {
+    constexpr uint32_t sc = D ? 1 : 0;
+    if (B.btype == BT_RAW) { put_run<1, D>(out, 0, J.comp + B.src_off, B.src_size, lane, 32, l0); return; }
+    if (B.btype == BT_RLE) { fill_run(out, rle_word<D>(J.comp[B.src_off], l0), B.src_size << sc, lane, 32); return; }
+    const uint8_t* lsrc = nullptr;
+    uint32_t rle = 0;
+    if (B.lit_type == LT_RAW) lsrc = J.comp + B.src_off + B.lit_src;
+    else if (B.lit_type == LT_RLE) rle = rle_word<D>(J.comp[B.src_off + B.lit_src], l0);
+    else lsrc = J.lit + B.lit_base;
+    const uint32_t n = B.n_seq, base = B.seq_base;
+    uint32_t lp = 0, op = 0, ll = 0, ml = 0;
+    if ((uint32_t)lane < n) {
+        const uint4 r = *(const uint4*)&J.seq[base + lane];
+        ll = r.x; ml = r.y; lp = r.w; op = J.seq[base + lane].outpos;
+        J.seq[base + lane].match_pos = S.out_off + op + ll;
+    }
+    uint32_t t_lp = 0, t_op = 0;
+    if (n) {
+        const uint32_t e_lp = __shfl_sync(0xFFFFFFFFu, lp + ll, (int)n - 1), e_op = __shfl_sync(0xFFFFFFFFu, op + ll + ml, (int)n - 1);
+        t_lp = e_lp; t_op = e_op;
+    }
+    for (uint32_t i = 0; i <= n; i++) {
+        uint32_t rl, rp, ro;
+        if (i < n) { rl = __shfl_sync(0xFFFFFFFFu, ll, (int)i); rp = __shfl_sync(0xFFFFFFFFu, lp, (int)i); ro = __shfl_sync(0xFFFFFFFFu, op, (int)i); }
+        else { rp = t_lp; ro = t_op; rl = B.lit_regen > t_lp ? B.lit_regen - t_lp : 0u; }
+        if (rl == 0) continue;
+        if (rp + rl > B.lit_regen) break;
+        if (B.lit_type == LT_RLE) rle_run<D>(out, ro, rle, rl, lane, 32);
+        else put_run<1, D>(out, ro, lsrc + rp, rl, lane, 32, l0);
+    }
 }
 
 __global__ void __launch_bounds__(256) k_lz_literals_tiny(JobDev J) {
@@ -1909,39 +1995,9 @@
     if (!tiny_lit_block(B)) return;
     if (J.frame_bad[B.frame]) return;
     const BlockState& S = J.bstate[bi];
-    uint8_t* out = J.out + S.out_off;
-    if (B.btype == BT_RAW) { copy_g2g(out, J.comp + B.src_off, B.src_size, lane, 32); return; }
-    if (B.btype == BT_RLE) {
-        const uint8_t v = J.comp[B.src_off];
-        for (uint32_t i = lane; i < B.src_size; i += 32) out[i] = v;
-        return;
-    }
-    const uint8_t* lsrc = nullptr;
-    uint8_t rle = 0;
-    if (B.lit_type == LT_RAW) lsrc = J.comp + B.src_off + B.lit_src;
-    else if (B.lit_type == LT_RLE) rle = J.comp[B.src_off + B.lit_src];
-    else lsrc = J.lit + B.lit_base;
-    const uint32_t n = B.n_seq, base = B.seq_base;
-    uint32_t lp = 0, op = 0, ll = 0, ml = 0;
-    if ((uint32_t)lane < n) {
-        const uint4 r = *(const uint4*)&J.seq[base + lane];
-        ll = r.x; ml = r.y; lp = r.w; op = J.seq[base + lane].outpos;
-        J.seq[base + lane].match_pos = S.out_off + op + ll;
-    }
-    uint32_t t_lp = 0, t_op = 0;
-    if (n) {
-        const uint32_t e_lp = __shfl_sync(0xFFFFFFFFu, lp + ll, (int)n - 1), e_op = __shfl_sync(0xFFFFFFFFu, op + ll + ml, (int)n - 1);
-        t_lp = e_lp; t_op = e_op;
-    }
-    for (uint32_t i = 0; i <= n; i++) {
-        uint32_t rl, rp, ro;
-        if (i < n) { rl = __shfl_sync(0xFFFFFFFFu, ll, (int)i); rp = __shfl_sync(0xFFFFFFFFu, lp, (int)i); ro = __shfl_sync(0xFFFFFFFFu, op, (int)i); }
-        else { rp = t_lp; ro = t_op; rl = B.lit_regen > t_lp ? B.lit_regen - t_lp : 0u; }
-        if (rl == 0) continue;
-        if (rp + rl > B.lit_regen) break;
-        if (B.lit_type == LT_RLE) for (uint32_t k = lane; k < rl; k += 32) out[ro + k] = rle;
-        else copy_g2g(out + ro, lsrc + rp, rl, lane, 32);
-    }
+    const FrameDesc& F = J.frames[B.frame];
+    if (F.direct_lut) lz_literals_tiny_block<true>(J, B, S, J.out + F.ascii_off + 2 * (S.out_off - F.dst_off), F.direct_lut, lane);
+    else lz_literals_tiny_block<false>(J, B, S, J.out + S.out_off, 0, lane);
 }
 
 __device__ __forceinline__ uint32_t resolve_offset(const JobDev& J, uint32_t v, uint32_t block) {
@@ -1951,39 +2007,41 @@
     return in > d ? in - d : 0;
 }
 
+__device__ __forceinline__ bool pair_match(uint64_t d, uint32_t off, uint32_t ml) { return ((d | off | ml) & 1u) == 0; }
 __device__ __forceinline__ void copy_match(uint8_t* out, uint64_t d, uint32_t off, uint32_t ml, int lane, int nlanes) {
     const uint8_t* s = out + d - off;
     uint8_t* o = out + d;
+    const uint32_t us = pair_match(d, off, ml) ? 1u : 0u;
+    const uint32_t n = ml >> us, p = off >> us;
     const bool periodic = off < ml;
-    for (uint32_t k0 = 0; k0 < ml; k0 += 8u * (uint32_t)nlanes) {
-        uint8_t t[8];
+    for (uint32_t k0 = 0; k0 < n; k0 += 8u * (uint32_t)nlanes) {
+        uint32_t t[8];
 #pragma unroll
         for (uint32_t j = 0; j < 8; j++) {
             const uint32_t k = k0 + j * (uint32_t)nlanes + (uint32_t)lane;
-            if (k < ml) t[j] = s[periodic ? k % off : k];
+            const uint32_t x = (periodic ? k % p : k) << us;
+            if (k < n) t[j] = us ? (uint32_t)*(const uint16_t*)(s + x) : (uint32_t)s[x];
         }
 #pragma unroll
         for (uint32_t j = 0; j < 8; j++) {
             const uint32_t k = k0 + j * (uint32_t)nlanes + (uint32_t)lane;
-            if (k < ml) o[k] = t[j];
-        }
-    }
-}
-
-__device__ __forceinline__ void fill_run(uint8_t* dst, uint32_t v, uint32_t n, int lane, int nlanes) {
-    const uint32_t h = (uint32_t)(-(intptr_t)dst) & 15u;
-    if (n < 32u + h) { for (uint32_t k = lane; k < n; k += nlanes) dst[k] = (uint8_t)v; return; }
-    if ((uint32_t)lane < h) dst[lane] = (uint8_t)v;
-    const uint32_t body = (n - h) >> 4, w = v * 0x01010101u;
-    uint4* d4 = (uint4*)(dst + h);
-    for (uint32_t c = lane; c < body; c += nlanes) d4[c] = make_uint4(w, w, w, w);
-    for (uint32_t k = h + (body << 4) + lane; k < n; k += nlanes) dst[k] = (uint8_t)v;
+            if (k < n) { if (us) *(uint16_t*)(o + (k << 1)) = (uint16_t)t[j]; else o[k] = (uint8_t)t[j]; }
+        }
+    }
 }
 
 __device__ __forceinline__ void copy_long_match(uint8_t* out, uint64_t d, uint32_t off, uint32_t ml, int lane, int nlanes) {
     if (off >= ml) copy_g2g(out + d, out + d - off, ml, lane, nlanes);
-    else if (off == 1) fill_run(out + d, out[d - 1], ml, lane, nlanes);
+    else if (off == 1) fill_run(out + d, out[d - 1] * 0x01010101u, ml, lane, nlanes);
+    else if (off == 2) {
+        const uint32_t p = (d & 1) ? out[d - 1] | ((uint32_t)out[d - 2] << 8) : out[d - 2] | ((uint32_t)out[d - 1] << 8);
+        fill_run(out + d, p * 0x00010001u, ml, lane, nlanes);
+    }
     else copy_match(out, d, off, ml, lane, nlanes);
+}
+
+__device__ __forceinline__ void to_letters(const FrameDesc& F, uint64_t& d, uint32_t& off, uint32_t& ml) {
+    if (F.direct_lut) { d = F.ascii_off + 2 * (d - F.dst_off); off *= 2; ml *= 2; }
 }
 
 constexpr uint32_t LZ_IDX_SHIFT = 12, LZ_IDX_PER_CHUNK = 65536u >> LZ_IDX_SHIFT;
@@ -2054,6 +2112,7 @@
         off += resolve_offset(J, Q.off, Q.block);
     }
     if (off != off0) R.off = off;
+    if (verdict == 1) to_letters(F, d, off, ml);
     return verdict;
 }
 
@@ -2091,7 +2150,7 @@
                 const int v = lz_try(J, idx[u], round, d, off, ml);
                 if (v == 0) pend[u] = true;
                 else if (v == 1) {
-                    if (ml <= LZ_SHORT) { copy_match(J.out, d, off, ml, 0, 1); J.seq_done[idx[u]] = round; }
+                    if (ml <= (pair_match(d, off, ml) ? 2 * LZ_SHORT : LZ_SHORT)) { copy_match(J.out, d, off, ml, 0, 1); J.seq_done[idx[u]] = round; }
                     else {
                         const uint32_t slot = atomicAdd(q_n, 1u);
                         if (slot < (uint32_t)LZ_CTA) { q_d[slot] = d; q_off[slot] = off; q_ml[slot] = ml; q_i[slot] = idx[u]; }
@@ -2220,6 +2279,7 @@
             if (active) {
                 while (j < i && J.seq[j].match_pos < e && done[j] != 0) j++;
                 ready = !(j < i && J.seq[j].match_pos < e);
+                if (ready) to_letters(J.frames[frame], d, off, ml);
             }
             const uint32_t rb = __ballot_sync(0xFFFFFFFFu, ready);
             if (rb) {
@@ -2278,9 +2338,12 @@
         done[i] = J.frame_bad[B.frame] ? 1 : 0;
     }
     if (tid == 0) { s_pending[0] = s_pending[1] = s_pending[2] = 0; }
-    __shared__ uint32_t fr_first[64], fr_off[64];
+    __shared__ uint32_t fr_first[64], fr_off[64], fr_asc[64];
     const bool fr_cached = J.n_frames <= 64u;
-    if (fr_cached && (uint32_t)tid < J.n_frames) { fr_first[tid] = J.frames[tid].first_seq; fr_off[tid] = (uint32_t)J.frames[tid].dst_off; }
+    if (fr_cached && (uint32_t)tid < J.n_frames) {
+        const FrameDesc& F = J.frames[tid];
+        fr_first[tid] = F.first_seq; fr_off[tid] = (uint32_t)F.dst_off; fr_asc[tid] = F.direct_lut ? (uint32_t)F.ascii_off : 0u;
+    }
     __syncthreads();
     long long t_probe = 0, t_copy = 0, t0 = 0, t_begin = 0;
     SEQ_CLK(t_begin);
@@ -2326,13 +2389,21 @@
         const uint32_t nq = q_n, nbig = q_big;
         {
             const uint32_t warp = (uint32_t)tid >> 5, NW = LZS_T / 32;
+            auto letters = [&](uint32_t i, uint32_t& d, uint32_t& off, uint32_t& ml) {
+                const uint32_t f = frm[i], asc = fr_cached ? fr_asc[f] : (J.frames[f].direct_lut ? (uint32_t)J.frames[f].ascii_off : 0u);
+                if (asc) { d = asc + 2 * (d - (fr_cached ? fr_off[f] : (uint32_t)J.frames[f].dst_off)); off *= 2; ml *= 2; }
+            };
             for (uint32_t t = warp; t < nq; t += NW) {
-                const uint32_t i = q_i[t], ml = mlen[i], off = q_off[t];
-                if (off >= ml) copy_g2g<4>(J.out + pos[i], J.out + pos[i] - off, ml, lane, 32);
-                else copy_long_match(J.out, pos[i], off, ml, lane, 32);
+                const uint32_t i = q_i[t];
+                uint32_t d = pos[i], ml = mlen[i], off = q_off[t];
+                letters(i, d, off, ml);
+                if (off >= ml) copy_g2g<4>(J.out + d, J.out + d - off, ml, lane, 32);
+                else copy_long_match(J.out, d, off, ml, lane, 32);
             }
             for (uint32_t t = 0; t < nbig; t++) {
-                const uint32_t i = q_i[np - 1u - t], ml = mlen[i], off = q_off[np - 1u - t], d = pos[i];
+                const uint32_t i = q_i[np - 1u - t];
+                uint32_t ml = mlen[i], off = q_off[np - 1u - t], d = pos[i];
+                letters(i, d, off, ml);
                 for (uint32_t pc = (warp + NW - (t & (NW - 1))) & (NW - 1); pc * 2048u < ml; pc += NW) {
                     const uint32_t b = pc * 2048u, len = ml - b < 2048u ? ml - b : 2048u;
                     copy_g2g<4>(J.out + d + b, J.out + d - off + b, len, lane, 32);
@@ -2378,6 +2449,19 @@
     return lo;
 }
 
+__device__ __forceinline__ void fin_pack(const JobDev& J, const FrameDesc& F, uint64_t c0, uint32_t cn, uint32_t tid, uint32_t nt) {
+    const uint8_t* a = J.out + F.ascii_off + 2 * (c0 - F.dst_off);
+    for (uint32_t e = tid * 8; e < cn; e += nt * 8) *(uint64_t*)(J.out + c0 + e) = nk::iupac_pack16(__ldcg((const uint4*)(a + 2 * e)));
+}
+__device__ __forceinline__ void fin_expand(const JobDev& J, const FrameDesc& F, uint64_t c0, uint32_t cn, uint32_t tid, uint32_t nt) {
+    uint8_t* a = J.out + F.ascii_off + 2 * (c0 - F.dst_off);
+    const uint32_t l0 = F.direct_lut;
+    for (uint32_t e = tid * 8; e < cn; e += nt * 8) {
+        const uint2 w = __ldcg((const uint2*)(J.out + c0 + e));
+        *(uint4*)(a + 2 * e) = make_uint4(nk::iupac4(w.x & 0xFFFFu, l0), nk::iupac4(w.x >> 16, l0), nk::iupac4(w.y & 0xFFFFu, l0), nk::iupac4(w.y >> 16, l0));
+    }
+}
+
 __global__ void __launch_bounds__(FIN_T) k_lz_finish(JobDev J) {
     if (*J.lz_handover == 0) return;
     NAF_DYN_SMEM(unsigned char, fin_smem);
@@ -2415,6 +2499,8 @@
         const uint32_t cn = (uint32_t)(c1 - c0);
         uint8_t* out_c0 = J.out + c0;
         uint32_t* g = J.fin_g + J.fin_g_base[f] + (size_t)(c - J.fin_chunk_first[f]) * FIN_C;
+        const bool direct = J.frames[f].direct_lut != 0;
+        if (direct) fin_pack(J, J.frames[f], c0, cn, tid, FIN_T);
         bool mine = false;
         for (uint32_t base = mi;; base += FIN_T) {
             const uint32_t i = base + tid;
@@ -2516,6 +2602,7 @@
             for (uint32_t e = tid; e < FIN_C / 32; e += FIN_T) xb[e] = extbit[e];
         }
         if (tid == 0 && s_unres) { J.fin_chunk_flag[c] = 1; atomicAdd(J.fin_unresolved, s_unres); }
+        if (direct && !s_unres) { __syncthreads(); fin_expand(J, J.frames[f], c0, cn, tid, FIN_T); }
     }
 }
 
@@ -2624,6 +2711,7 @@
             for (uint32_t k = 0; k < 4; k++)
                 if (dd[k] != 0 && e0 + k < cn && dd[k] <= e0 + k) o[e0 + k] = __ldcg(o + e0 + k - dd[k]);
         }
+        if (J.frames[f].direct_lut) { __syncthreads(); fin_expand(J, J.frames[f], f0 + crel, cn, tid, FIN2_T); }
     }
 }
 
@@ -2632,6 +2720,10 @@
                    XXP5 = 0x27D4EB2F165667C5ull;
 __device__ __forceinline__ uint64_t xxh_round(uint64_t acc, uint64_t in) { return xxh_rotl(acc + in * XXP2, 31) * XXP1; }
 __device__ __forceinline__ uint64_t xxh_merge(uint64_t h, uint64_t v) { return (h ^ xxh_round(0, v)) * XXP1 + XXP4; }
+
+__device__ __forceinline__ uint64_t ck_load8(const FrameDesc& F, const uint8_t* p, const uint8_t* a, uint64_t i) {
+    return F.direct_lut ? nk::iupac_pack16(*(const uint4*)(a + 2 * i)) : *(const uint64_t*)(p + i);
+}
 
 __global__ void __launch_bounds__(32) k_frame_checksum(JobDev J) {
     const uint32_t f = blockIdx.x;
@@ -2639,21 +2731,21 @@
     if (!F.has_checksum || J.frame_bad[f]) return;
     const int lane = threadIdx.x;
     const uint8_t* p = J.out + F.dst_off;
+    const uint8_t* a = J.out + F.ascii_off;
     const uint64_t len = F.dst_size, stripes = len >> 5;
     uint64_t h;
     if (stripes) {
         uint64_t v = lane == 0 ? XXP1 + XXP2 : (lane == 1 ? XXP2 : (lane == 2 ? 0ull : 0ull - XXP1));
         if (lane < 4) {
-            const uint64_t* q = (const uint64_t*)p + lane;
             uint64_t s = 0;
             for (; s + 8 <= stripes; s += 8) {
                 uint64_t in[8];
 #pragma unroll
-                for (int k = 0; k < 8; k++) in[k] = q[4 * (s + k)];
+                for (int k = 0; k < 8; k++) in[k] = ck_load8(F, p, a, 32 * (s + k) + 8 * lane);
 #pragma unroll
                 for (int k = 0; k < 8; k++) v = xxh_round(v, in[k]);
             }
-            for (; s < stripes; s++) v = xxh_round(v, q[4 * s]);
+            for (; s < stripes; s++) v = xxh_round(v, ck_load8(F, p, a, 32 * s + 8 * lane));
         }
         const uint64_t v1 = __shfl_sync(0xFFFFFFFFu, v, 0), v2 = __shfl_sync(0xFFFFFFFFu, v, 1), v3 = __shfl_sync(0xFFFFFFFFu, v, 2),
                        v4 = __shfl_sync(0xFFFFFFFFu, v, 3);
@@ -2663,9 +2755,11 @@
     if (lane != 0) return;
     h += len;
     uint64_t i = stripes << 5;
-    for (; i + 8 <= len; i += 8) { h ^= xxh_round(0, *(const uint64_t*)(p + i)); h = xxh_rotl(h, 27) * XXP1 + XXP4; }
-    if (i + 4 <= len) { h ^= (uint64_t)(*(const uint32_t*)(p + i)) * XXP1; h = xxh_rotl(h, 23) * XXP2 + XXP3; i += 4; }
-    for (; i < len; i++) { h ^= (uint64_t)p[i] * XXP5; h = xxh_rotl(h, 11) * XXP1; }
+    for (; i + 8 <= len; i += 8) { h ^= xxh_round(0, ck_load8(F, p, a, i)); h = xxh_rotl(h, 27) * XXP1 + XXP4; }
+    const uint64_t t = i < len ? ck_load8(F, p, a, i) : 0;
+    uint32_t k = 0;
+    if (i + 4 <= len) { h ^= (t & 0xFFFFFFFFull) * XXP1; h = xxh_rotl(h, 23) * XXP2 + XXP3; i += 4; k = 4; }
+    for (; i < len; i++, k++) { h ^= ((t >> (8 * k)) & 0xFF) * XXP5; h = xxh_rotl(h, 11) * XXP1; }
     h ^= h >> 33; h *= XXP2; h ^= h >> 29; h *= XXP3; h ^= h >> 32;
     if ((uint32_t)h != F.checksum) flag_error(J, f, zc::E_CHECKSUM);
 }
```

After: 447.9 (median of 6 runs). 1.02x the previous value.
